# Nightmare-n/GD-MAE

Measured on AMD Instinct MI355X. Metric: MAE pre-train frames/sec (Waymo-shape, 180k pts, 75% mask), higher is better.
Workload: dtype bf16

## Files before the change

gd-mae_amd/csrc/plan.hip:

```cpp
#include "../../include/gdmae_hip.h"
#include "common.h"
#include <string.h>

int gd_voxelize_impl(const float* points, long long n_points, int n_cols, const float* lo, const float* vs, const int* grid_xyz,
                     int batch_size, float* points_out, long long* point_coords, long long* inverse, int* inverse32,
                     long long* voxel_coords, int* pillar_cell, int* pillar_pt_off, int* pillar_pts, int* point_rank,
                     int* sample_pillar_off, float* pillar_mean, int* cell2pillar_out, int* counts, void* workspace, size_t workspace_bytes,
                     void* lb_state, float* points_pm, int* row_pillar, hipStream_t st);
size_t gd_voxelize_lb_state_bytes(long long n_points, long long cells);
size_t gd_plan_scan_state_bytes(long long n);
size_t gd_plan_win_state_bytes(long long n);
int gd_plan_visible_tokens(const float* mask, const int* cell2pillar, long long n_cells, int* tok_pillar, int* tok_cell, int* map,
                           int* n_tok, void* lb_state, hipStream_t st);
int gd_plan_downsample(const int* map_in, int B, int Yi, int Xi, int* tok_cell_out, int* map_out, int* n_out, void* lb_state,
                       hipStream_t st);
struct Dims {
  int B, Y, X;
};
struct PlanJob {
  const int* n_tok;
  const int* tok_cell;
  Dims dt, dm;
  const int* map;
  int mode, s;
  int* nbr;
  int* nbr_rev;
};
constexpr int kPlanMaxJobs = 16;
struct PlanJobs {
  PlanJob j[kPlanMaxJobs];
  int count;
};
int gd_plan_jobs(const PlanJobs& J, long long cap_max, hipStream_t st);
size_t gd_plan_windows_ws_bytes(int B, int Y, int X, int wx, int wy);
long long gd_plan_n_windows(int B, int Y, int X, int wx, int wy);
struct GdWinStage {
  const int* map;
  int B, Y, X, wx, wy, nlev;
  const int *drop_lo, *drop_hi, *max_tokens;
  int* out[2][7];
  int* counts[2];
  void* workspace;
  void* lb_state;
};
int gd_plan_windows_all(const GdWinStage* stages, int n_stages, hipStream_t st);
size_t gd_decoder_tiles_lb_state_bytes(long long nt);
int gd_decoder_tiles_lb(const int* const* maps, const int* strides, int k, int B, int H, int W, int* tile_slot, int* tile_list, int* n_act,
                        int* flag, void* lb_state, hipStream_t st);
int gd_decoder_site_rulebook(const int* site, const int* n_dev, int sites_per_tok, long long cap_sites, const int* tile_slot, int H, int W,
                             int* nbr, hipStream_t st);

namespace {

struct StageGeo {
  int Y, X;
  long long cap;
  long long cap_in;
  int up_s;
  long long n_win;
};

struct Layout {
  gdmae_plan_buffer* table;
  int max_entries, n;
  size_t off;
  bool ok;
  long long add(const char* name, size_t bytes) {
    const size_t o = off;
    if (table) {
      if (n >= max_entries) {
        ok = false;
        return -1;
      }
      strncpy(table[n].name, name, sizeof(table[n].name) - 1);
      table[n].name[sizeof(table[n].name) - 1] = 0;
      table[n].offset = (long long)o;
      table[n].bytes = (long long)bytes;
    }
    ++n;
    off += gd_align(bytes);
    return (long long)o;
  }
};

struct Offsets {
  long long lb_state, counts, points, point_coords, inverse, inverse32, voxel_coords, pillar_cell, pt_off, pillar_pts, point_rank,
      sample_off, pillar_mean, cell2pillar, points_pm, row_pillar, vox_ws, mask, len_keep, tok_pillar;
  long long vis_tok_cell, vis_map;
  struct {
    long long tok_cell, map, nbr_subm, nbr_subm_t, nbr_down, nbr_down_t, up_sites, win_ws;
    long long w[2][7];
  } s[GDMAE_PLAN_MAX_STAGES];
  long long dec_slot, dec_list, dec_flag, dec_nbr[3];
  size_t lb_bytes, vox_ws_bytes;
  int n_counts;
  bool dec;
  StageGeo geo[GDMAE_PLAN_MAX_STAGES];
  long long cap_pts, m_cap, cells;
};

int check(const gdmae_plan_params* p) {
  GD_REQUIRE(p != nullptr, "geometry plan: null parameters");
  GD_REQUIRE(p->n_points >= 0 && p->n_points < (1ll << 31) && p->n_cols >= 4 && p->n_cols <= 65 && p->batch_size >= 1,
             "geometry plan: bad point buffer");
  GD_REQUIRE(p->grid[0] >= 1 && p->grid[1] >= 1 && p->grid[2] == 1, "geometry plan: single-layer pillar grids (spt_backbone_mae.py:94)");
  GD_REQUIRE(p->n_stages >= 1 && p->n_stages <= GDMAE_PLAN_MAX_STAGES, "geometry plan: 1..4 stages");
  for (int i = 0; i < p->n_stages; ++i) {
    GD_REQUIRE(p->stride[i] == 1 || p->stride[i] == 2, "geometry plan: conv_down stride 1 or 2 (k3 s2 p1)");
    GD_REQUIRE(i == 0 || p->stride[i] == 2, "geometry plan: only the first stage may keep the resolution");
    GD_REQUIRE(p->win_x[i] >= 1 && p->win_y[i] >= 1 && p->win_x[i] * p->win_y[i] <= 64, "geometry plan: window must fit one wavefront");
    GD_REQUIRE(p->n_levels[i] >= 1 && p->n_levels[i] <= 3, "geometry plan: 1..3 drop levels");
  }
  GD_REQUIRE(p->n_dec >= 0 && p->n_dec <= 3, "geometry plan: at most 3 decoder source stages");
  for (int g = 0; g < p->n_dec; ++g) GD_REQUIRE(p->dec_sources[g] >= 0 && p->dec_sources[g] < p->n_stages, "geometry plan: decoder source");
  return 0;
}

int layout(const gdmae_plan_params* p, gdmae_plan_buffer* table, int max_entries, Offsets& O, size_t* total, int* n_entries) {
  if (int rc = check(p)) return rc;
  Layout L{table, max_entries, 0, 0, true};
  const int B = p->batch_size, gx = p->grid[0], gy = p->grid[1], F = p->n_cols - 1;
  const long long n0 = p->cap_points > p->n_points ? p->cap_points : p->n_points;
  O.cells = (long long)B * gx * gy;
  GD_REQUIRE(O.cells < (1ll << 31), "geometry plan: B*Y*X must fit int32");
  O.cap_pts = n0 > 0 ? n0 : 1;
  O.m_cap = n0 < O.cells ? n0 : O.cells;
  if (O.m_cap < 1) O.m_cap = 1;
  const long long cap = O.cap_pts;
  int Y = gy, X = gx;
  long long c = O.m_cap;
  for (int i = 0; i < p->n_stages; ++i) {
    StageGeo& g = O.geo[i];
    g.cap_in = c;
    if (p->stride[i] == 2) {
      Y = (Y - 1) / 2 + 1;
      X = (X - 1) / 2 + 1;
      c = 4 * c < (long long)B * Y * X ? 4 * c : (long long)B * Y * X;
    }
    g.Y = Y; g.X = X; g.cap = c;
    const int us = gy / Y;
    g.up_s = (us >= 1 && us * Y == gy && us * X == gx) ? us : 0;
    g.n_win = gd_plan_n_windows(B, Y, X, p->win_x[i], p->win_y[i]);
    GD_REQUIRE(g.n_win < (1 << 21), "geometry plan: window grid too large for the packed scan");
  }
  O.dec = p->n_dec > 0;
  for (int g = 0; g < p->n_dec; ++g) {
    const int us = O.geo[p->dec_sources[g]].up_s;
    O.dec = O.dec && (us == 1 || us == 2 || us == 4 || us == 8);
  }
  const long long nt = (long long)B * ((gy + 7) / 8) * ((gx + 7) / 8);
  size_t lb = gd_voxelize_lb_state_bytes(n0, O.cells) + gd_plan_scan_state_bytes(O.cells);
  for (int i = 0; i < p->n_stages; ++i) {
    if (p->stride[i] == 2) lb += gd_plan_scan_state_bytes((long long)B * O.geo[i].Y * O.geo[i].X);
    lb += 2 * gd_plan_win_state_bytes(O.geo[i].n_win);
  }
  if (O.dec) lb += gd_decoder_tiles_lb_state_bytes(nt);
  O.lb_bytes = lb;
  O.lb_state = L.add("lb_state", lb);
  O.n_counts = 2 + p->n_stages + 16 * p->n_stages + 1 + 1;
  O.counts = L.add("counts", sizeof(int) * O.n_counts);
  O.points = L.add("points", sizeof(float) * cap * p->n_cols);
  O.point_coords = L.add("point_coords", sizeof(long long) * cap * 4);
  O.inverse = L.add("inverse", sizeof(long long) * cap);
  O.inverse32 = L.add("inverse32", sizeof(int) * cap);
  O.voxel_coords = L.add("voxel_coords", sizeof(long long) * cap * 4);
  O.pillar_cell = L.add("pillar_cell", sizeof(int) * cap);
  O.pt_off = L.add("pt_off", sizeof(int) * (cap + 1));
  O.pillar_pts = L.add("pillar_pts", sizeof(int) * cap);
  O.point_rank = L.add("point_rank", sizeof(int) * cap);
  O.sample_off = L.add("sample_off", sizeof(int) * (B + 1));
  O.pillar_mean = L.add("pillar_mean", sizeof(float) * cap * F);
  O.cell2pillar = L.add("cell2pillar", sizeof(int) * O.cells);
  O.points_pm = L.add("points_pm", sizeof(float) * cap * p->n_cols);
  O.row_pillar = L.add("row_pillar", sizeof(int) * cap);
  O.vox_ws_bytes = gdmae_voxelize_workspace_bytes(n0, B, gx, gy, 1);
  O.vox_ws = L.add("vox_ws", O.vox_ws_bytes);
  O.mask = L.add("mask", sizeof(float) * O.m_cap);
  O.len_keep = L.add("len_keep", sizeof(int) * B);
  O.tok_pillar = L.add("tok_pillar", sizeof(int) * O.m_cap);
  O.vis_tok_cell = O.vis_map = -1;
  if (p->stride[0] == 2) {
    O.vis_tok_cell = L.add("vis.tok_cell", sizeof(int) * O.m_cap);
    O.vis_map = L.add("vis.map", sizeof(int) * O.cells);
  }
  char nm[40];
  static const char* const kWin[7] = {"tok_win", "tok_level", "tok_slot", "tok_pos", "csr_tok", "win_start", "win_len"};
  for (int i = 0; i < p->n_stages; ++i) {
    const StageGeo& g = O.geo[i];
    auto name = [&](const char* s) { snprintf(nm, sizeof(nm), "s%d.%s", i, s); return (const char*)nm; };
    O.s[i].tok_cell = L.add(name("tok_cell"), sizeof(int) * g.cap);
    O.s[i].map = L.add(name("map"), sizeof(int) * (long long)B * g.Y * g.X);
    O.s[i].nbr_subm = L.add(name("nbr_subm"), sizeof(int) * g.cap * 9);
    O.s[i].nbr_subm_t = L.add(name("nbr_subm_t"), sizeof(int) * g.cap * 9);
    O.s[i].nbr_down = O.s[i].nbr_down_t = O.s[i].up_sites = -1;
    if (p->stride[i] == 2) {
      O.s[i].nbr_down = L.add(name("nbr_down"), sizeof(int) * g.cap * 9);
      O.s[i].nbr_down_t = L.add(name("nbr_down_t"), sizeof(int) * g.cap_in * 9);
    }
    if (g.up_s > 1) O.s[i].up_sites = L.add(name("up_sites"), sizeof(int) * g.cap * g.up_s * g.up_s);
    O.s[i].win_ws = L.add(name("win_ws"), gd_plan_windows_ws_bytes(B, g.Y, g.X, p->win_x[i], p->win_y[i]));
    const long long wcap = g.n_win < g.cap ? g.n_win : g.cap;
    for (int sh = 0; sh < 2; ++sh)
      for (int k = 0; k < 7; ++k) {
        snprintf(nm, sizeof(nm), "s%d.w%d.%s", i, sh, kWin[k]);
        O.s[i].w[sh][k] = L.add(nm, sizeof(int) * (k < 5 ? g.cap : wcap));
      }
  }
  O.dec_slot = O.dec_list = O.dec_flag = -1;
  if (O.dec) {
    O.dec_slot = L.add("dec.tile_slot", sizeof(int) * nt);
    O.dec_list = L.add("dec.tile_list", sizeof(int) * nt);
    O.dec_flag = L.add("dec.flag", sizeof(int) * nt);
    for (int g = 0; g < p->n_dec; ++g) {
      const StageGeo& sg = O.geo[p->dec_sources[g]];
      snprintf(nm, sizeof(nm), "dec.nbr%d", g);
      O.dec_nbr[g] = L.add(nm, sizeof(int) * sg.cap * sg.up_s * sg.up_s * 9);
    }
  }
  GD_REQUIRE(L.ok, "geometry plan: buffer table too small");
  if (total) *total = L.off;
  if (n_entries) *n_entries = L.n;
  return 0;
}

}

extern "C" int gdmae_geometry_plan_layout(const gdmae_plan_params* p, gdmae_plan_buffer* table, int max_entries, int* n_entries,
                                          size_t* total_bytes) {
  Offsets O;
  return layout(p, table, max_entries, O, total_bytes, n_entries);
}

extern "C" int gdmae_geometry_plan(const gdmae_plan_params* p, const float* points, const float* noise, void* arena, size_t arena_bytes,
                                   void* stream) {
  Offsets O;
  size_t total = 0;
  if (int rc = layout(p, nullptr, 0, O, &total, nullptr)) return rc;
  GD_REQUIRE(arena != nullptr && arena_bytes >= total, "geometry plan: arena too small (gdmae_geometry_plan_layout)");
  GD_REQUIRE(!p->masked || noise != nullptr, "geometry plan: masking needs one noise value per pillar (capacity min(points, cells))");
  hipStream_t st = (hipStream_t)stream;
  char* A = (char*)arena;
  auto I = [&](long long off) { return off < 0 ? (int*)nullptr : (int*)(A + off); };
  const int B = p->batch_size, gx = p->grid[0], gy = p->grid[1], ns = p->n_stages;
  int* counts = I(O.counts);
  int* n_tok = counts + 2;
  int* win_counts = counts + 2 + ns;
  int* n_act = counts + 2 + ns + 16 * ns;
  int* n_vis = n_act + 1;
  GD_CHECK(hipMemsetAsync(A + O.lb_state, 0, (size_t)(O.counts - O.lb_state) + gd_align(sizeof(int) * O.n_counts), st));
  char* lb = A + O.lb_state;
  {
    int rc = gd_voxelize_impl(points, p->n_points, p->n_cols, p->lo, p->vs, p->grid, B, (float*)(A + O.points), (long long*)(A + O.point_coords),
                              (long long*)(A + O.inverse), I(O.inverse32), (long long*)(A + O.voxel_coords), I(O.pillar_cell), I(O.pt_off),
                              I(O.pillar_pts), I(O.point_rank), I(O.sample_off), (float*)(A + O.pillar_mean), I(O.cell2pillar), counts,
                              A + O.vox_ws, O.vox_ws_bytes, lb, p->want_pm ? (float*)(A + O.points_pm) : nullptr,
                              p->want_pm ? I(O.row_pillar) : nullptr, st);
    if (rc) return rc;
    lb += gd_voxelize_lb_state_bytes(p->n_points, O.cells);
  }
  float* mask = (float*)(A + O.mask);
  if (p->masked) {
    int rc = gdmae_random_mask(noise, I(O.sample_off), B, p->keep_frac, mask, I(O.len_keep), stream);
    if (rc) return rc;
  } else {
    GD_CHECK(hipMemsetAsync(mask, 0, sizeof(float) * O.m_cap, st));
  }
  const bool first_strided = p->stride[0] == 2;
  int* cur_cell = first_strided ? I(O.vis_tok_cell) : I(O.s[0].tok_cell);
  int* cur_map = first_strided ? I(O.vis_map) : I(O.s[0].map);
  int* cur_n = first_strided ? n_vis : n_tok;
  {
    int rc = gd_plan_visible_tokens(mask, I(O.cell2pillar), O.cells, I(O.tok_pillar), cur_cell, cur_map, cur_n, lb, st);
    if (rc) return rc;
    lb += gd_plan_scan_state_bytes(O.cells);
  }
  int Yp = gy, Xp = gx;
  PlanJobs J;
  J.count = 0;
  long long cap_max = 1;
  GdWinStage W[4];
  GD_REQUIRE(ns <= 4, "geometry plan: at most four stages");
  for (int i = 0; i < ns; ++i) {
    const StageGeo& g = O.geo[i];
    GD_REQUIRE(J.count + 4 <= kPlanMaxJobs, "geometry plan: job table full");
    if (g.cap > cap_max) cap_max = g.cap;
    if (p->stride[i] == 2) {
      int rc = gd_plan_downsample(cur_map, B, Yp, Xp, I(O.s[i].tok_cell), I(O.s[i].map), n_tok + i, lb, st);
      if (rc) return rc;
      lb += gd_plan_scan_state_bytes((long long)B * g.Y * g.X);
      J.j[J.count++] = PlanJob{n_tok + i, I(O.s[i].tok_cell), Dims{B, g.Y, g.X}, Dims{B, Yp, Xp}, cur_map, 1, 0, I(O.s[i].nbr_down), nullptr};
      J.j[J.count++] = PlanJob{cur_n, cur_cell, Dims{B, Yp, Xp}, Dims{B, g.Y, g.X}, I(O.s[i].map), 2, 0, I(O.s[i].nbr_down_t), nullptr};
      if (g.cap_in > cap_max) cap_max = g.cap_in;
      cur_cell = I(O.s[i].tok_cell);
      cur_map = I(O.s[i].map);
      cur_n = n_tok + i;
      Yp = g.Y;
      Xp = g.X;
    }
    J.j[J.count++] = PlanJob{cur_n, cur_cell, Dims{B, g.Y, g.X}, Dims{B, g.Y, g.X}, cur_map, 0, 0, I(O.s[i].nbr_subm), I(O.s[i].nbr_subm_t)};
    if (g.up_s > 1) {
      J.j[J.count++] = PlanJob{cur_n, cur_cell, Dims{B, g.Y, g.X}, Dims{B, g.Y, g.X}, nullptr, 3, g.up_s, I(O.s[i].up_sites), nullptr};
      if (g.cap * g.up_s * g.up_s / 9 + 1 > cap_max) cap_max = g.cap * g.up_s * g.up_s / 9 + 1;
    }
    GdWinStage& w = W[i];
    w.map = cur_map;
    w.B = B; w.Y = g.Y; w.X = g.X; w.wx = p->win_x[i]; w.wy = p->win_y[i]; w.nlev = p->n_levels[i];
    w.drop_lo = p->drop_lo[i]; w.drop_hi = p->drop_hi[i]; w.max_tokens = p->max_tokens[i];
    w.counts[0] = win_counts + 16 * i;
    w.counts[1] = win_counts + 16 * i + 8;
    for (int sh = 0; sh < 2; ++sh)
      for (int k = 0; k < 7; ++k) w.out[sh][k] = I(O.s[i].w[sh][k]);
    w.workspace = A + O.s[i].win_ws;
    w.lb_state = lb;
    lb += 2 * gd_plan_win_state_bytes(g.n_win);
  }
  {
    int rc = gd_plan_jobs(J, cap_max, st);
    if (rc) return rc;
    rc = gd_plan_windows_all(W, ns, st);
    if (rc) return rc;
  }
  if (O.dec) {
    const int* maps[3];
    int ups[3];
    for (int g = 0; g < p->n_dec; ++g) {
      maps[g] = I(O.s[p->dec_sources[g]].map);
      ups[g] = O.geo[p->dec_sources[g]].up_s;
    }
    int rc = gd_decoder_tiles_lb(maps, ups, p->n_dec, B, gy, gx, I(O.dec_slot), I(O.dec_list), n_act, I(O.dec_flag), lb, st);
    if (rc) return rc;
    for (int g = 0; g < p->n_dec; ++g) {
      const int si = p->dec_sources[g];
      const StageGeo& sg = O.geo[si];
      const int* sites = sg.up_s > 1 ? I(O.s[si].up_sites) : I(O.s[si].tok_cell);
      rc = gd_decoder_site_rulebook(sites, n_tok + si, sg.up_s * sg.up_s, sg.cap * sg.up_s * sg.up_s, I(O.dec_slot), gy, gx, I(O.dec_nbr[g]), st);
      if (rc) return rc;
    }
  }
  return 0;
}
```

gd-mae_amd/csrc/segment.hip:

```cpp
#include "common.h"

__global__ __launch_bounds__(256) void k_gather_rows(const uint4* __restrict__ src, const int* __restrict__ idx,
                                                     long long n_slots, int row_vec, int tab_stride, int tab_off,
                                                     uint4* __restrict__ out) {
  const long long total = n_slots * row_vec;
  for (long long i = blockIdx.x * (long long)blockDim.x + threadIdx.x; i < total; i += (long long)gridDim.x * blockDim.x) {
    const long long s = i / row_vec;
    const int v = (int)(i % row_vec);
    const int j = idx[s];
    uint4 val = make_uint4(0, 0, 0, 0);
    if (j >= 0) val = src[(long long)j * tab_stride + tab_off + v];
    out[i] = val;
  }
}

__global__ __launch_bounds__(256) void k_scatter_rows(const uint4* __restrict__ src, const int* __restrict__ idx,
                                                      long long n_rows, int row_vec, int tab_stride, int tab_off,
                                                      uint4* __restrict__ dst) {
  const long long total = n_rows * row_vec;
  for (long long i = blockIdx.x * (long long)blockDim.x + threadIdx.x; i < total; i += (long long)gridDim.x * blockDim.x) {
    const long long s = i / row_vec;
    const int v = (int)(i % row_vec);
    const int j = idx[s];
    if (j >= 0) dst[(long long)j * tab_stride + tab_off + v] = src[i];
  }
}

static inline int gd_grid_for(long long total, int block = 256, int cap = 16384) {
  int g = gd_div_up(total > 0 ? total : 1, block);
  return g > cap ? cap : g;
}

extern "C" int gdmae_gather_rows(const void* src, const int* idx, long long n_slots, int row_bytes, void* out,
                                 void* stream) {
  GD_REQUIRE(row_bytes % 16 == 0, "row_bytes must be a multiple of 16");
  if (n_slots <= 0) return 0;
  const int rv = row_bytes / 16;
  hipLaunchKernelGGL(k_gather_rows, dim3(gd_grid_for(n_slots * rv)), dim3(256), 0, (hipStream_t)stream,
                     (const uint4*)src, idx, n_slots, rv, rv, 0, (uint4*)out);
  GD_LAUNCH_CHECK();
  return 0;
}

extern "C" int gdmae_gather_rows_strided(const void* src, const int* idx, long long n_slots, int row_bytes,
                                         int table_row_bytes, int table_col_bytes, void* out, void* stream) {
  GD_REQUIRE(row_bytes % 16 == 0 && table_row_bytes % 16 == 0 && table_col_bytes % 16 == 0, "16-byte granularity");
  GD_REQUIRE(table_col_bytes + row_bytes <= table_row_bytes, "slice exceeds the table row");
  if (n_slots <= 0) return 0;
  const int rv = row_bytes / 16;
  hipLaunchKernelGGL(k_gather_rows, dim3(gd_grid_for(n_slots * rv)), dim3(256), 0, (hipStream_t)stream,
                     (const uint4*)src, idx, n_slots, rv, table_row_bytes / 16, table_col_bytes / 16, (uint4*)out);
  GD_LAUNCH_CHECK();
  return 0;
}

extern "C" int gdmae_scatter_rows_strided(const void* src, const int* idx, long long n_rows, int row_bytes,
                                          int table_row_bytes, int table_col_bytes, void* dst, void* stream) {
  GD_REQUIRE(row_bytes % 16 == 0 && table_row_bytes % 16 == 0 && table_col_bytes % 16 == 0, "16-byte granularity");
  GD_REQUIRE(table_col_bytes + row_bytes <= table_row_bytes, "slice exceeds the table row");
  if (n_rows <= 0) return 0;
  const int rv = row_bytes / 16;
  hipLaunchKernelGGL(k_scatter_rows, dim3(gd_grid_for(n_rows * rv)), dim3(256), 0, (hipStream_t)stream,
                     (const uint4*)src, idx, n_rows, rv, table_row_bytes / 16, table_col_bytes / 16, (uint4*)dst);
  GD_LAUNCH_CHECK();
  return 0;
}

extern "C" int gdmae_scatter_rows(const void* src, const int* idx, long long n_rows, int row_bytes, void* dst,
                                  void* stream) {
  GD_REQUIRE(row_bytes % 16 == 0, "row_bytes must be a multiple of 16");
  if (n_rows <= 0) return 0;
  const int rv = row_bytes / 16;
  hipLaunchKernelGGL(k_scatter_rows, dim3(gd_grid_for(n_rows * rv)), dim3(256), 0, (hipStream_t)stream,
                     (const uint4*)src, idx, n_rows, rv, rv, 0, (uint4*)dst);
  GD_LAUNCH_CHECK();
  return 0;
}

template <int LPP>
__global__ __launch_bounds__(256) void k_segment_max(const float* __restrict__ x, const int* __restrict__ pt_off,
                                                     const int* __restrict__ csr, int M, float* __restrict__ out,
                                                     int* __restrict__ arg) {
  constexpr int C = LPP * 4;
  constexpr int G = GD_WAVE / LPP;
  const int lane = threadIdx.x & (GD_WAVE - 1);
  const int wib = threadIdx.x / GD_WAVE;
  const int grp = lane / LPP, cl = lane % LPP;
  for (int p = blockIdx.x * 4 + wib; p < M; p += gridDim.x * 4) {
    const int off = pt_off[p];
    const int cnt = pt_off[p + 1] - off;
    float best[4] = {-INFINITY, -INFINITY, -INFINITY, -INFINITY};
    int bi[4] = {0x7fffffff, 0x7fffffff, 0x7fffffff, 0x7fffffff};
#pragma unroll 4
    for (int j = grp; j < cnt; j += G) {
      const int i = csr[off + j];
      const float4 v = *reinterpret_cast<const float4*>(x + (long long)i * C + cl * 4);
      const float vv[4] = {v.x, v.y, v.z, v.w};
#pragma unroll
      for (int e = 0; e < 4; ++e) {
        if (vv[e] > best[e] || bi[e] == 0x7fffffff) {
          best[e] = vv[e];
          bi[e] = i;
        }
      }
    }
#pragma unroll
    for (int d = LPP; d < GD_WAVE; d <<= 1) {
#pragma unroll
      for (int e = 0; e < 4; ++e) {
        const float ob = __shfl_xor(best[e], d, GD_WAVE);
        const int oi = __shfl_xor(bi[e], d, GD_WAVE);
        const bool take = (oi != 0x7fffffff) && (bi[e] == 0x7fffffff || ob > best[e] || (ob == best[e] && oi < bi[e]));
        if (take) {
          best[e] = ob;
          bi[e] = oi;
        }
      }
    }
    if (grp == 0) {
      *reinterpret_cast<float4*>(out + (long long)p * C + cl * 4) = make_float4(best[0], best[1], best[2], best[3]);
      *reinterpret_cast<int4*>(arg + (long long)p * C + cl * 4) = make_int4(bi[0], bi[1], bi[2], bi[3]);
    }
  }
}

__global__ __launch_bounds__(256) void k_segment_max_bwd(const float* __restrict__ dout, const int* __restrict__ arg,
                                                         const int* __restrict__ inv, long long N, int C,
                                                         float* __restrict__ dx) {
  const long long total = N * C;
  for (long long e = blockIdx.x * (long long)blockDim.x + threadIdx.x; e < total; e += (long long)gridDim.x * blockDim.x) {
    const long long i = e / C;
    const int c = (int)(e % C);
    const long long q = (long long)inv[i] * C + c;
    dx[e] = (arg[q] == (int)i) ? dout[q] : 0.f;
  }
}

extern "C" int gdmae_segment_max(const float* x, const int* pt_off, const int* csr, int M, int C, float* out, int* arg,
                                 void* stream) {
  if (M <= 0) return 0;
  const dim3 grid(gd_grid_for(M, 4, 16384)), block(256);
  hipStream_t st = (hipStream_t)stream;
  switch (C) {
    case 16: hipLaunchKernelGGL((k_segment_max<4>), grid, block, 0, st, x, pt_off, csr, M, out, arg); break;
    case 32: hipLaunchKernelGGL((k_segment_max<8>), grid, block, 0, st, x, pt_off, csr, M, out, arg); break;
    case 64: hipLaunchKernelGGL((k_segment_max<16>), grid, block, 0, st, x, pt_off, csr, M, out, arg); break;
    case 128: hipLaunchKernelGGL((k_segment_max<32>), grid, block, 0, st, x, pt_off, csr, M, out, arg); break;
    case 256: hipLaunchKernelGGL((k_segment_max<64>), grid, block, 0, st, x, pt_off, csr, M, out, arg); break;
    default: GD_REQUIRE(false, "segment_max supports C in {16, 32, 64, 128, 256}");
  }
  GD_LAUNCH_CHECK();
  return 0;
}

extern "C" int gdmae_segment_max_bwd(const float* dout, const int* arg, const int* inv, long long N, int C, float* dx,
                                     void* stream) {
  if (N <= 0) return 0;
  hipLaunchKernelGGL(k_segment_max_bwd, dim3(gd_grid_for(N * C)), dim3(256), 0, (hipStream_t)stream, dout, arg, inv, N, C,
                     dx);
  GD_LAUNCH_CHECK();
  return 0;
}

struct DecoParams {
  float lo[3], vs[3];
  int ncols;
};
__global__ __launch_bounds__(256) void k_decorate(const float* __restrict__ pts, const long long* __restrict__ coords,
                                                  const int* __restrict__ inv, const float* __restrict__ mean, long long N,
                                                  DecoParams P, float* __restrict__ out) {
  const int F = P.ncols - 1;
  const int D = F + 6;
  for (long long i = blockIdx.x * (long long)blockDim.x + threadIdx.x; i < N; i += (long long)gridDim.x * blockDim.x) {
    const float* r = pts + i * P.ncols;
    const long long* c = coords + 4 * i;
    const float* m = mean + (long long)inv[i] * F;
    float* o = out + i * D;
    const float x = r[1], y = r[2], z = r[3];
    o[0] = __fsub_rn(x, __fadd_rn(__fmul_rn(__fadd_rn((float)c[3], 0.5f), P.vs[0]), P.lo[0]));
    o[1] = __fsub_rn(y, __fadd_rn(__fmul_rn(__fadd_rn((float)c[2], 0.5f), P.vs[1]), P.lo[1]));
    o[2] = __fsub_rn(z, __fadd_rn(__fmul_rn(__fadd_rn((float)c[1], 0.5f), P.vs[2]), P.lo[2]));
    for (int k = 0; k < F; ++k) o[3 + k] = r[1 + k];
    o[3 + F] = __fsub_rn(x, m[0]);
    o[4 + F] = __fsub_rn(y, m[1]);
    o[5 + F] = __fsub_rn(z, m[2]);
  }
}

extern "C" int gdmae_decorate_points(const float* points, const long long* point_coords, const int* inverse32,
                                     const float* pillar_mean, long long N, int n_cols, const float* lo, const float* vs,
                                     float* out, void* stream) {
  if (N <= 0) return 0;
  DecoParams P;
  for (int i = 0; i < 3; ++i) {
    P.lo[i] = lo[i];
    P.vs[i] = vs[i];
  }
  P.ncols = n_cols;
  hipLaunchKernelGGL(k_decorate, dim3(gd_grid_for(N)), dim3(256), 0, (hipStream_t)stream, points, point_coords, inverse32,
                     pillar_mean, N, P, out);
  GD_LAUNCH_CHECK();
  return 0;
}

__device__ inline void unpack8(const uint4& u, float (&f)[8]) {
  const unsigned w[4] = {u.x, u.y, u.z, u.w};
#pragma unroll
  for (int k = 0; k < 4; ++k) {
    f[2 * k] = __uint_as_float(w[k] << 16);
    f[2 * k + 1] = __uint_as_float(w[k] & 0xFFFF0000u);
  }
}

template <bool BF16>
__global__ __launch_bounds__(256) void k_colstats_partial(const uint4* __restrict__ x, long long R, int C,
                                                          float* __restrict__ part ) {
  constexpr int EPV = BF16 ? 8 : 4;
  const int vec_per_row = C / EPV;
  const int rows_per_iter = 256 / vec_per_row;
  const int vr = threadIdx.x / vec_per_row;
  const int vc = threadIdx.x % vec_per_row;
  const bool live = vr < rows_per_iter;
  const long long chunk = (R + gridDim.x - 1) / gridDim.x;
  const long long r0 = blockIdx.x * chunk;
  const long long r1 = r0 + chunk < R ? r0 + chunk : R;
  float s[EPV], q[EPV];
#pragma unroll
  for (int e = 0; e < EPV; ++e) s[e] = q[e] = 0.f;
  for (long long r = r0 + vr; live && r < r1; r += rows_per_iter) {
    const uint4 u = x[r * vec_per_row + vc];
    float f[8];
    if (BF16) {
      unpack8(u, f);
    } else {
      f[0] = __uint_as_float(u.x);
      f[1] = __uint_as_float(u.y);
      f[2] = __uint_as_float(u.z);
      f[3] = __uint_as_float(u.w);
    }
#pragma unroll
    for (int e = 0; e < EPV; ++e) {
      s[e] += f[e];
      q[e] = fmaf(f[e], f[e], q[e]);
    }
  }
  extern __shared__ float sh[];
  if (live) {
#pragma unroll
    for (int e = 0; e < EPV; ++e) {
      sh[(vr * 2 + 0) * C + vc * EPV + e] = s[e];
      sh[(vr * 2 + 1) * C + vc * EPV + e] = q[e];
    }
  }
  __syncthreads();
  for (int c = threadIdx.x; c < 2 * C; c += 256) {
    float acc = 0.f;
    for (int rr = 0; rr < rows_per_iter; ++rr) acc += sh[rr * 2 * C + c];
    part[(long long)blockIdx.x * 2 * C + c] = acc;
  }
}

__global__ __launch_bounds__(256) void k_colstats_final(const float* __restrict__ part, int nblk, int C2,
                                                        double* __restrict__ out) {
  __shared__ double sh[16][17];
  const int cl = threadIdx.x & 15, ps = threadIdx.x >> 4;
  const int c = blockIdx.x * 16 + cl;
  double acc = 0.0;
  if (c < C2) {
#pragma unroll 8
    for (int b = ps; b < nblk; b += 16) acc += (double)part[(long long)b * C2 + c];
  }
  sh[ps][cl] = acc;
  __syncthreads();
  if (ps == 0 && c < C2) {
    double s = 0.0;
    for (int k = 0; k < 16; ++k) s += sh[k][cl];
    out[c] = s;
  }
}

extern "C" size_t gdmae_colstats_workspace_bytes(int C) { return (size_t)1024 * 2 * C * sizeof(float); }

extern "C" int gdmae_colstats(const void* x, long long R, int C, int is_bf16, double* out, void* workspace, void* stream) {
  hipStream_t st = (hipStream_t)stream;
  const int epv = is_bf16 ? 8 : 4;
  GD_REQUIRE(C % epv == 0 && (C / epv) <= 256, "C must be a multiple of 8 (bf16) / 4 (fp32) and <= 2048 / 1024");
  int nblk = (int)(R / 64 > 512 ? 512 : (R / 64 > 0 ? R / 64 : 1));
  if (R >= (1ll << 20)) nblk = 1024;
  const int rows_per_iter = 256 / (C / epv);
  const size_t lds = (size_t)rows_per_iter * 2 * C * sizeof(float);
  GD_REQUIRE(lds <= 64 * 1024, "colstats LDS");
  if (is_bf16)
    hipLaunchKernelGGL((k_colstats_partial<true>), dim3(nblk), dim3(256), lds, st, (const uint4*)x, R, C, (float*)workspace);
  else
    hipLaunchKernelGGL((k_colstats_partial<false>), dim3(nblk), dim3(256), lds, st, (const uint4*)x, R, C, (float*)workspace);
  GD_LAUNCH_CHECK();
  hipLaunchKernelGGL(k_colstats_final, dim3(gd_div_up(2 * C, 16)), dim3(256), 0, st, (const float*)workspace, nblk, 2 * C, out);
  GD_LAUNCH_CHECK();
  return 0;
}

__global__ __launch_bounds__(256) void k_bn_fold_final(const float* __restrict__ part, int nblk, int C, double count,
                                                       const float* __restrict__ gamma, const float* __restrict__ beta,
                                                       double eps, double momentum, float* __restrict__ running_mean,
                                                       float* __restrict__ running_var, long long* __restrict__ num_batches,
                                                       double* __restrict__ stats, float* __restrict__ ab,
                                                       float* __restrict__ mv) {
  __shared__ double sh[2][16][17];
  const int cl = threadIdx.x & 15, ps = threadIdx.x >> 4;
  const int c = blockIdx.x * 16 + cl;
  double a1 = 0.0, a2 = 0.0;
  {
    const int cc = c < C ? c : C - 1;
    const float* p = part + cc;
    for (int b0 = ps; b0 < nblk; b0 += 128) {
      float v1[8], v2[8];
#pragma unroll
      for (int u = 0; u < 8; ++u) {
        const int b = b0 + 16 * u < nblk ? b0 + 16 * u : nblk - 1;
        v1[u] = p[(long long)b * 2 * C];
        v2[u] = p[(long long)b * 2 * C + C];
      }
#pragma unroll
      for (int u = 0; u < 8; ++u) {
        const bool ok = b0 + 16 * u < nblk;
        a1 += ok ? (double)v1[u] : 0.0;
        a2 += ok ? (double)v2[u] : 0.0;
      }
    }
  }
  sh[0][ps][cl] = a1;
  sh[1][ps][cl] = a2;
  __syncthreads();
  if (ps == 0 && c < C) {
    double s1 = 0.0, s2 = 0.0;
    for (int k = 0; k < 16; ++k) { s1 += sh[0][k][cl]; s2 += sh[1][k][cl]; }
    const double mean = s1 / count;
    double var = s2 / count - mean * mean;
    if (var < 0.0) var = 0.0;
    const double r = 1.0 / sqrt(var + eps);
    const double a = (double)gamma[c] * r;
    stats[c] = mean;
    stats[C + c] = r;
    ab[c] = (float)a;
    ab[C + c] = (float)((double)beta[c] - a * mean);
    mv[c] = (float)mean;
    mv[C + c] = (float)var;
    if (running_mean) {
      const float m = (float)momentum;
      const float unb = (float)(var * (count / (count > 1.0 ? count - 1.0 : 1.0)));
      running_mean[c] = running_mean[c] * (1.f - m) + m * (float)mean;
      running_var[c] = running_var[c] * (1.f - m) + m * unb;
      if (c == 0 && num_batches) *num_batches += 1;
    }
  }
}

extern "C" int gdmae_bn_fold(const void* x, long long R, int C, int is_bf16, double count, const float* gamma,
                             const float* beta, double eps, double momentum, float* running_mean, float* running_var,
                             long long* num_batches, double* stats, float* ab, float* mv, void* workspace, void* stream) {
  hipStream_t st = (hipStream_t)stream;
  const int epv = is_bf16 ? 8 : 4;
  GD_REQUIRE(C % epv == 0 && (C / epv) <= 256, "C must be a multiple of 8 (bf16) / 4 (fp32) and <= 2048 / 1024");
  int nblk = (int)(R / 64 > 512 ? 512 : (R / 64 > 0 ? R / 64 : 1));
  if (R >= (1ll << 20)) nblk = 1024;
  const int rows_per_iter = 256 / (C / epv);
  const size_t lds = (size_t)rows_per_iter * 2 * C * sizeof(float);
  GD_REQUIRE(lds <= 64 * 1024, "colstats LDS");
  if (is_bf16)
    hipLaunchKernelGGL((k_colstats_partial<true>), dim3(nblk), dim3(256), lds, st, (const uint4*)x, R, C, (float*)workspace);
  else
    hipLaunchKernelGGL((k_colstats_partial<false>), dim3(nblk), dim3(256), lds, st, (const uint4*)x, R, C, (float*)workspace);
  GD_LAUNCH_CHECK();
  hipLaunchKernelGGL(k_bn_fold_final, dim3(gd_div_up(C, 16)), dim3(256), 0, st, (const float*)workspace, nblk, C, count, gamma,
                     beta, eps, momentum, running_mean, running_var, num_batches, stats, ab, mv);
  GD_LAUNCH_CHECK();
  return 0;
}

int gd_bn_fold_from_partials(hipStream_t st, const float* part, int nblk, int C, double count, const float* gamma,
                             const float* beta, double eps, double momentum, float* running_mean, float* running_var,
                             long long* num_batches, double* stats, float* ab, float* mv) {
  hipLaunchKernelGGL(k_bn_fold_final, dim3(gd_div_up(C, 16)), dim3(256), 0, st, part, nblk, C, count, gamma, beta, eps, momentum,
                     running_mean, running_var, num_batches, stats, ab, mv);
  GD_LAUNCH_CHECK();
  return 0;
}
extern "C" int gdmae_bn_fold_partials(const float* part, int nblk, int C, double count, const float* gamma, const float* beta, double eps,
                                      double momentum, float* running_mean, float* running_var, long long* num_batches, double* stats,
                                      float* ab, float* mv, void* stream) {
  GD_REQUIRE(part != nullptr && nblk >= 1 && C >= 1, "bn_fold_partials: partial rows");
  return gd_bn_fold_from_partials((hipStream_t)stream, part, nblk, C, count, gamma, beta, eps, momentum, running_mean, running_var,
                                  num_batches, stats, ab, mv);
}
int gd_partials_to_f64(hipStream_t st, const float* part, int nblk, int C2, double* out) {
  hipLaunchKernelGGL(k_colstats_final, dim3(gd_div_up(C2, 16)), dim3(256), 0, st, part, nblk, C2, out);
  GD_LAUNCH_CHECK();
  return 0;
}

__global__ __launch_bounds__(256) void k_bn_bwd_coeffs(const double* __restrict__ st, int n_st, const double* __restrict__ stats,
                                                       const float* __restrict__ ab, const float* __restrict__ gamma, int C,
                                                       double count, const double* __restrict__ tot,
                                                       float* __restrict__ dgamma, float* __restrict__ dbeta, int accumulate,
                                                       float* __restrict__ c01) {
  const int c = blockIdx.x * blockDim.x + threadIdx.x;
  if (c >= C) return;
  const double mean = stats[c], r = stats[C + c];
  const double a = (double)ab[c], b = (double)ab[C + c];
  double db = st[c];
  if (tot && n_st >= 3 && b > 0.0) db += tot[c] - st[2 * C + c];
  const double da = st[C + c] - db * mean;
  const double dv = -0.5 * (da * (double)gamma[c]) * r * r * r;
  const double dmu = -db * a - 2.0 * mean * dv;
  c01[c] = (float)(dmu / count);
  c01[C + c] = (float)(2.0 * dv / count);
  const float dg = (float)(da * r), dbf = (float)db;
  if (accumulate) { dgamma[c] += dg; dbeta[c] += dbf; }
  else { dgamma[c] = dg; dbeta[c] = dbf; }
}

__global__ __launch_bounds__(256) void k_bn_bwd_coeffs_rows(const float* __restrict__ part, int nblk, int n_st,
                                                            const double* __restrict__ stats, const float* __restrict__ ab,
                                                            const float* __restrict__ gamma, int C, double count,
                                                            const double* __restrict__ tot, float* __restrict__ dgamma,
                                                            float* __restrict__ dbeta, int accumulate, float* __restrict__ c01) {
  __shared__ double sh[3][32][9];
  const int cl = threadIdx.x & 7, ps = threadIdx.x >> 3;
  const int c = blockIdx.x * 8 + cl;
  const long long stride = (long long)n_st * C;
  {
    const int cc = c < C ? c : C - 1;
    double acc[3] = {0.0, 0.0, 0.0};
    for (int b0 = ps; b0 < nblk; b0 += 256) {
      float x[3][8];
#pragma unroll
      for (int v = 0; v < 3; ++v)
#pragma unroll
        for (int u = 0; u < 8; ++u) {
          const int b = b0 + 32 * u < nblk ? b0 + 32 * u : nblk - 1;
          x[v][u] = part[(long long)b * stride + (long long)(v < n_st ? v : 0) * C + cc];
        }
#pragma unroll
      for (int v = 0; v < 3; ++v)
#pragma unroll
        for (int u = 0; u < 8; ++u) acc[v] += b0 + 32 * u < nblk ? (double)x[v][u] : 0.0;
    }
#pragma unroll
    for (int v = 0; v < 3; ++v) sh[v][ps][cl] = acc[v];
  }
  __syncthreads();
  if (ps != 0 || c >= C) return;
  double s[3] = {0.0, 0.0, 0.0};
  for (int v = 0; v < n_st; ++v)
    for (int k = 0; k < 32; ++k) s[v] += sh[v][k][cl];
  const double mean = stats[c], r = stats[C + c];
  const double a = (double)ab[c], bb = (double)ab[C + c];
  double db = s[0];
  if (tot && n_st >= 3 && bb > 0.0) db += tot[c] - s[2];
  const double da = s[1] - db * mean;
  const double dv = -0.5 * (da * (double)gamma[c]) * r * r * r;
  const double dmu = -db * a - 2.0 * mean * dv;
  c01[c] = (float)(dmu / count);
  c01[C + c] = (float)(2.0 * dv / count);
  const float dg = (float)(da * r), dbf = (float)db;
  if (accumulate) { dgamma[c] += dg; dbeta[c] += dbf; }
  else { dgamma[c] = dg; dbeta[c] = dbf; }
}
extern "C" int gdmae_bn_bwd_coeffs_rows(const float* part, int nblk, int n_st, const double* stats, const float* ab, const float* gamma,
                                        int C, double count, const double* tot, float* dgamma, float* dbeta, int accumulate, float* c01,
                                        void* stream) {
  GD_REQUIRE((n_st == 2 || n_st == 3) && nblk >= 1, "n_st must be 2 or 3");
  hipLaunchKernelGGL(k_bn_bwd_coeffs_rows, dim3(gd_div_up(C, 8)), dim3(256), 0, (hipStream_t)stream, part, nblk, n_st, stats, ab, gamma, C,
                     count, tot, dgamma, dbeta, accumulate, c01);
  GD_LAUNCH_CHECK();
  return 0;
}

extern "C" int gdmae_bn_bwd_coeffs(const double* st, int n_st, const double* stats, const float* ab, const float* gamma, int C,
                                   double count, const double* tot, float* dgamma, float* dbeta, int accumulate, float* c01,
                                   void* stream) {
  GD_REQUIRE(n_st == 2 || n_st == 3, "n_st must be 2 or 3");
  hipLaunchKernelGGL(k_bn_bwd_coeffs, dim3(gd_div_up(C, 256)), dim3(256), 0, (hipStream_t)stream, st, n_st, stats, ab, gamma, C,
                     count, tot, dgamma, dbeta, accumulate, c01);
  GD_LAUNCH_CHECK();
  return 0;
}
```

gd-mae_amd/csrc/vfe_fused.hip:

```cpp
#include "common.h"
#include "gemm.h"

int gd_bn_fold_from_partials(hipStream_t st, const float* part, int nblk, int C, double count, const float* gamma,
                             const float* beta, double eps, double momentum, float* running_mean, float* running_var,
                             long long* num_batches, double* stats, float* ab, float* mv);
int gd_partials_to_f64(hipStream_t st, const float* part, int nblk, int C2, double* out);
extern "C" int gdmae_bn_bwd_coeffs(const double* st, int n_st, const double* stats, const float* ab, const float* gamma, int C,
                                   double count, const double* tot, float* dgamma, float* dbeta, int accumulate, float* c01,
                                   void* stream);

namespace {

typedef float f32x16 __attribute__((ext_vector_type(16)));

constexpr int VF_C = 64;
constexpr int VF_WAVES = 4;
constexpr int VF_MAX_GRID = 1024;

struct VfeGeom {
  float lo[3], vs[3];
  int out_f16 = 0;
};

enum { VF_STATS = 0, VF_APPLY = 1, VF_BSTATS = 2, VF_DW = 3 };

__device__ inline unsigned short vf_f2bf(float f) { return gd_to_bf16(f); }

template <int F>
struct VfA {
  float r[F + 1];
  int pil;
};
struct VfB {
  long long c1, c2, c3;
  float m[3];
};
template <int F>
__device__ __forceinline__ void vf_load_a(const float* __restrict__ pts, const int* __restrict__ inv, long long i, long long N, VfA<F>& A) {
  const long long ic = i < N ? i : N - 1;
  const float* r = pts + ic * (F + 1);
#pragma unroll
  for (int k = 0; k < F + 1; ++k) A.r[k] = r[k];
  A.pil = inv[ic];
}
template <int F>
__device__ __forceinline__ void vf_load_b(const long long* __restrict__ coords, const float* __restrict__ mean, int cpp, long long i,
                                          long long N, int pil, VfB& B) {
  const long long ic = i < N ? i : N - 1;
  const long long* c = coords + 4 * (cpp ? (long long)pil : ic);
  const float* m = mean + (long long)pil * F;
  B.c1 = c[1]; B.c2 = c[2]; B.c3 = c[3];
  B.m[0] = m[0]; B.m[1] = m[1]; B.m[2] = m[2];
}
template <int F>
__device__ __forceinline__ void vf_features(const VfA<F>& A, const VfB& B, bool live, const VfeGeom& G, float (&f)[F + 6]) {
  const float x = A.r[1], y = A.r[2], z = A.r[3];
  f[0] = __fsub_rn(x, __fadd_rn(__fmul_rn(__fadd_rn((float)B.c3, 0.5f), G.vs[0]), G.lo[0]));
  f[1] = __fsub_rn(y, __fadd_rn(__fmul_rn(__fadd_rn((float)B.c2, 0.5f), G.vs[1]), G.lo[1]));
  f[2] = __fsub_rn(z, __fadd_rn(__fmul_rn(__fadd_rn((float)B.c1, 0.5f), G.vs[2]), G.lo[2]));
#pragma unroll
  for (int k = 0; k < F; ++k) f[3 + k] = A.r[1 + k];
  f[3 + F] = __fsub_rn(x, B.m[0]);
  f[4 + F] = __fsub_rn(y, B.m[1]);
  f[5 + F] = __fsub_rn(z, B.m[2]);
#pragma unroll
  for (int k = 0; k < F + 6; ++k) f[k] = live ? f[k] : 0.f;
}
template <bool BF>
struct VfG {
  unsigned u[BF ? 16 : 1];
  float2 v[BF ? 1 : 16];
};
template <bool BF>
__device__ __forceinline__ void vf_load_g(const void* __restrict__ g, long long base, long long N, int n, int half, VfG<BF>& Gr) {
#pragma unroll
  for (int r = 0; r < 16; ++r) {
    const long long row = base + 8 * (r / 4) + 4 * half + (r % 4);
    const long long rc = row < N ? row : N - 1;
    if (BF) Gr.u[r] = ((const unsigned*)g)[rc * (VF_C / 2) + n];
    else Gr.v[r] = ((const float2*)g)[rc * (VF_C / 2) + n];
  }
}

template <int F, int MODE, bool BF>
__global__ __launch_bounds__(VF_WAVES * 64) void k_vfe1(const float* __restrict__ pts, const long long* __restrict__ coords,
                                                        const int* __restrict__ inv, const float* __restrict__ mean,
                                                        int cpp, long long N, VfeGeom G, const float* __restrict__ W,
                                                        const float* __restrict__ ab, const float* __restrict__ c01,
                                                        const void* __restrict__ g, void* __restrict__ out,
                                                        float* __restrict__ part) {
  constexpr int D = F + 6;
  constexpr int KS = (D + 1) / 2;
  constexpr int DP = 2 * KS;
  const int lane = threadIdx.x & 63, wave = threadIdx.x >> 6;
  const int n = lane & 31, half = lane >> 5;
  __shared__ float sh[VF_WAVES * (MODE == VF_DW ? VF_C * D : 4 * VF_C)];
  __shared__ float shf[MODE == VF_DW ? VF_WAVES * 32 * DP : 1];

  float wb[2][KS];
#pragma unroll
  for (int blk = 0; blk < 2; ++blk)
#pragma unroll
    for (int s = 0; s < KS; ++s) {
      const int d = 2 * s + half;
      wb[blk][s] = d < D ? W[(2 * n + blk) * D + d] : 0.f;
    }
  float ca[2] = {0.f, 0.f}, cb[2] = {0.f, 0.f}, c0[2] = {0.f, 0.f}, c1[2] = {0.f, 0.f};
  if (MODE != VF_STATS) {
#pragma unroll
    for (int blk = 0; blk < 2; ++blk) {
      ca[blk] = ab[2 * n + blk];
      cb[blk] = ab[VF_C + 2 * n + blk];
      if (MODE == VF_DW) {
        c0[blk] = c01[2 * n + blk];
        c1[blk] = c01[VF_C + 2 * n + blk];
      }
    }
  }
  float s1[2] = {0.f, 0.f}, s2[2] = {0.f, 0.f};
  f32x16 accw[2];
#pragma unroll
  for (int r = 0; r < 16; ++r) accw[0][r] = accw[1][r] = 0.f;

  const long long ntiles = (N + 31) / 32;
  const long long tstride = (long long)gridDim.x * VF_WAVES;
  constexpr bool HAS_G = MODE == VF_BSTATS || MODE == VF_DW;
  constexpr bool PIPE = !HAS_G;
  VfA<F> A1, A2, A3;
  VfB B1, B2;
  VfG<BF> G1;
  if (PIPE) {
    const long long t = (long long)blockIdx.x * VF_WAVES + wave;
    vf_load_a<F>(pts, inv, t * 32 + n, N, A1);
    vf_load_a<F>(pts, inv, (t + tstride) * 32 + n, N, A2);
    vf_load_b<F>(coords, mean, cpp, t * 32 + n, N, A1.pil, B1);
  }
  for (long long t0 = (long long)blockIdx.x * VF_WAVES; t0 < ntiles; t0 += tstride) {
    const long long base = (t0 + wave) * 32;
    if (PIPE) {
      vf_load_a<F>(pts, inv, base + 2 * tstride * 32 + n, N, A3);
      vf_load_b<F>(coords, mean, cpp, base + tstride * 32 + n, N, A2.pil, B2);
      __builtin_amdgcn_sched_barrier(0);
    } else {
      vf_load_g<BF>(g, base, N, n, half, G1);
      vf_load_a<F>(pts, inv, base + n, N, A1);
      vf_load_b<F>(coords, mean, cpp, base + n, N, A1.pil, B1);
    }
    float g0[16], g1[16];
    if (HAS_G) {
#pragma unroll
      for (int r = 0; r < 16; ++r) {
        const long long row = base + 8 * (r / 4) + 4 * half + (r % 4);
        if (BF) {
          g0[r] = row < N ? __uint_as_float(G1.u[r] << 16) : 0.f;
          g1[r] = row < N ? __uint_as_float(G1.u[r] & 0xFFFF0000u) : 0.f;
        } else {
          g0[r] = row < N ? G1.v[r].x : 0.f;
          g1[r] = row < N ? G1.v[r].y : 0.f;
        }
      }
    }
    float f[D];
    vf_features<F>(A1, B1, base + n < N, G, f);
    f32x16 h[2];
#pragma unroll
    for (int r = 0; r < 16; ++r) h[0][r] = h[1][r] = 0.f;
#pragma unroll
    for (int s = 0; s < KS; ++s) {
      const float f0 = f[2 * s], f1 = (2 * s + 1 < D) ? f[2 * s + 1] : 0.f;
      const float a = half ? f1 : f0;
      h[0] = __builtin_amdgcn_mfma_f32_32x32x2f32(a, wb[0][s], h[0], 0, 0, 0);
      h[1] = __builtin_amdgcn_mfma_f32_32x32x2f32(a, wb[1][s], h[1], 0, 0, 0);
    }
    if (MODE == VF_STATS) {
#pragma unroll
      for (int r = 0; r < 16; ++r)
#pragma unroll
        for (int blk = 0; blk < 2; ++blk) {
          const float v = h[blk][r];
          s1[blk] += v;
          s2[blk] = fmaf(v, v, s2[blk]);
        }
    } else if (MODE == VF_APPLY) {
#pragma unroll
      for (int k = 0; k < F + 1; ++k) asm volatile("" : "+v"(A3.r[k]));
      asm volatile("" : "+v"(A3.pil));
      asm volatile("" : "+v"(B2.c1), "+v"(B2.c2), "+v"(B2.c3), "+v"(B2.m[0]), "+v"(B2.m[1]), "+v"(B2.m[2]));
#pragma unroll
      for (int r = 0; r < 16; ++r) {
        const long long row = base + 8 * (r / 4) + 4 * half + (r % 4);
        if (row < N) {
          const float y0 = fmaxf(fmaf(ca[0], h[0][r], cb[0]), 0.f), y1 = fmaxf(fmaf(ca[1], h[1][r], cb[1]), 0.f);
          if (BF) ((unsigned*)out)[row * (VF_C / 2) + n] = G.out_f16 ? gd_pack_f16(y0, y1) : ((unsigned)vf_f2bf(y0) | ((unsigned)vf_f2bf(y1) << 16));
          else ((float2*)out)[row * (VF_C / 2) + n] = make_float2(y0, y1);
        }
      }
    } else {
      if (MODE == VF_DW) {
        if (half == 0) {
#pragma unroll
          for (int d = 0; d < DP; ++d) shf[(wave * 32 + n) * DP + d] = d < D ? f[d] : 0.f;
        }
        __builtin_amdgcn_fence(__ATOMIC_RELEASE, "wavefront");
        __builtin_amdgcn_wave_barrier();
        __builtin_amdgcn_fence(__ATOMIC_ACQUIRE, "wavefront");
      }
#pragma unroll
      for (int r = 0; r < 16; ++r) {
        const int pr = 8 * (r / 4) + 4 * half + (r % 4);
        const float dh0 = fmaf(ca[0], h[0][r], cb[0]) > 0.f ? g0[r] : 0.f;
        const float dh1 = fmaf(ca[1], h[1][r], cb[1]) > 0.f ? g1[r] : 0.f;
        if (MODE == VF_BSTATS) {
          s1[0] += dh0;
          s1[1] += dh1;
          s2[0] = fmaf(dh0, h[0][r], s2[0]);
          s2[1] = fmaf(dh1, h[1][r], s2[1]);
        } else {
          const float dx0 = fmaf(c1[0], h[0][r], fmaf(ca[0], dh0, c0[0]));
          const float dx1 = fmaf(c1[1], h[1][r], fmaf(ca[1], dh1, c0[1]));
          const float bv = n < DP ? shf[(wave * 32 + pr) * DP + n] : 0.f;
          accw[0] = __builtin_amdgcn_mfma_f32_32x32x2f32(dx0, bv, accw[0], 0, 0, 0);
          accw[1] = __builtin_amdgcn_mfma_f32_32x32x2f32(dx1, bv, accw[1], 0, 0, 0);
        }
      }
      if (MODE == VF_DW) {
        __builtin_amdgcn_fence(__ATOMIC_RELEASE, "wavefront");
        __builtin_amdgcn_wave_barrier();
      }
    }
    if (PIPE) {
      A1 = A2;
      A2 = A3;
      B1 = B2;
    }
  }

  if (MODE == VF_STATS || MODE == VF_BSTATS) {
#pragma unroll
    for (int blk = 0; blk < 2; ++blk) {
      s1[blk] += __shfl_xor(s1[blk], 32, 64);
      s2[blk] += __shfl_xor(s2[blk], 32, 64);
    }
    if (half == 0) {
#pragma unroll
      for (int blk = 0; blk < 2; ++blk) {
        sh[wave * 2 * VF_C + 2 * n + blk] = s1[blk];
        sh[wave * 2 * VF_C + VF_C + 2 * n + blk] = s2[blk];
      }
    }
    __syncthreads();
    if (threadIdx.x < 2 * VF_C) {
      float a = 0.f;
#pragma unroll
      for (int w = 0; w < VF_WAVES; ++w) a += sh[w * 2 * VF_C + threadIdx.x];
      part[(long long)blockIdx.x * 2 * VF_C + threadIdx.x] = a;
    }
  } else if (MODE == VF_DW) {
    if (n < D) {
#pragma unroll
      for (int blk = 0; blk < 2; ++blk)
#pragma unroll
        for (int r = 0; r < 16; ++r) {
          const int col = 2 * (8 * (r / 4) + 4 * half + (r % 4)) + blk;
          sh[wave * VF_C * D + col * D + n] = accw[blk][r];
        }
    }
    __syncthreads();
    for (int e = threadIdx.x; e < VF_C * D; e += VF_WAVES * 64) {
      float a = 0.f;
#pragma unroll
      for (int w = 0; w < VF_WAVES; ++w) a += sh[w * VF_C * D + e];
      part[(long long)blockIdx.x * VF_C * D + e] = a;
    }
  }
}

template <typename K>
int vf_resident_blocks(K kernel, int slot) {
  static int cache[32] = {0};
  if (cache[slot] == 0) {
    int per_cu = 0, dev = 0;
    hipDeviceProp_t prop;
    if (hipOccupancyMaxActiveBlocksPerMultiprocessor(&per_cu, kernel, VF_WAVES * 64, 0) != hipSuccess || per_cu < 1) per_cu = 2;
    if (hipGetDevice(&dev) != hipSuccess || hipGetDeviceProperties(&prop, dev) != hipSuccess) prop.multiProcessorCount = 256;
    const long long b = (long long)per_cu * prop.multiProcessorCount;
    cache[slot] = (int)(b > VF_MAX_GRID ? VF_MAX_GRID : b);
  }
  return cache[slot];
}

template <int MODE>
int vf_launch(hipStream_t st, int F, bool bf, const float* pts, const long long* coords, const int* inv, const float* mean,
              int cpp, long long N, const VfeGeom& G, const float* W, const float* ab, const float* c01, const void* g, void* out,
              float* part, int* grid_out = nullptr) {
  const long long tiles = (N + 31) / 32, blocks = (tiles + VF_WAVES - 1) / VF_WAVES;
  const dim3 block(VF_WAVES * 64);
#define VF_GO(FF, BB)                                                                                                   \
  do {                                                                                                                  \
    const int cap = vf_resident_blocks(k_vfe1<FF, MODE, BB>, ((FF - 3) * 4 + MODE) * 2 + (BB ? 1 : 0));                 \
    const dim3 grid((unsigned)(blocks < cap ? blocks : cap));                                                           \
    if (grid_out) *grid_out = (int)grid.x;                                                                              \
    hipLaunchKernelGGL((k_vfe1<FF, MODE, BB>), grid, block, 0, st, pts, coords, inv, mean, cpp, N, G, W, ab, c01, g, out, part); \
  } while (0)
  if (F == 5) { if (bf) VF_GO(5, true); else VF_GO(5, false); }
  else if (F == 4) { if (bf) VF_GO(4, true); else VF_GO(4, false); }
  else if (F == 3) { if (bf) VF_GO(3, true); else VF_GO(3, false); }
  else GD_REQUIRE(false, "vfe point layer: 3, 4 or 5 point features (x, y, z [, intensity [, elongation]])");
#undef VF_GO
  GD_LAUNCH_CHECK();
  return 0;
}

}

__global__ __launch_bounds__(256) void k_pillar_major_rows(const float* __restrict__ pts, int ncols, const int* __restrict__ csr,
                                                           const int* __restrict__ inv, const int* __restrict__ n_dev,
                                                           float* __restrict__ pts_pm, int* __restrict__ rowpil) {
  const long long N = *n_dev;
  for (long long q = blockIdx.x * (long long)blockDim.x + threadIdx.x; q < N; q += (long long)gridDim.x * blockDim.x) {
    const int i = csr[q];
    rowpil[q] = inv[i];
    for (int k = 0; k < ncols; ++k) pts_pm[q * ncols + k] = pts[(long long)i * ncols + k];
  }
}

extern "C" int gdmae_pillar_major_rows(const float* points, int n_cols, const int* pillar_pts, const int* inverse32,
                                       const int* n_dev, long long capacity, float* points_pm, int* row_pillar,
                                       void* stream) {
  if (capacity <= 0) return 0;
  hipLaunchKernelGGL(k_pillar_major_rows, dim3((unsigned)(capacity / 256 + 1 > 8192 ? 8192 : capacity / 256 + 1)), dim3(256), 0, (hipStream_t)stream, points, n_cols,
                     pillar_pts, inverse32, n_dev, points_pm, row_pillar);
  GD_LAUNCH_CHECK();
  return 0;
}

extern "C" size_t gdmae_vfe_point_layer_workspace_bytes(int n_cols) {
  const int D = n_cols - 1 + 6;
  return gd_align((size_t)VF_MAX_GRID * VF_C * (D > 2 ? D : 2) * sizeof(float)) + gd_align(2 * VF_C * sizeof(double)) +
         gd_align(2 * VF_C * sizeof(float));
}

extern "C" int gdmae_vfe_point_layer_fwd(const float* points, const long long* point_coords, const int* inverse32,
                                         const float* pillar_mean, int coords_per_pillar, long long N, int n_cols,
                                         const float* lo, const float* vs,
                                         const float* W, int C, const float* gamma, const float* beta, double eps,
                                         double momentum, float* running_mean, float* running_var, long long* num_batches,
                                         double* stats, float* ab, float* mv, void* out, int out_bf16, void* workspace,
                                         void* stream) {
  GD_REQUIRE(C == VF_C, "vfe point layer: 64 output channels");
  GD_REQUIRE(N > 0, "vfe point layer: no points");
  hipStream_t st = (hipStream_t)stream;
  VfeGeom G;
  for (int i = 0; i < 3; ++i) { G.lo[i] = lo[i]; G.vs[i] = vs[i]; }
  float* part = (float*)workspace;
  const int F = n_cols - 1;
  int grid = 0;
  int rc = vf_launch<VF_STATS>(st, F, false, points, point_coords, inverse32, pillar_mean, coords_per_pillar, N, G, W, nullptr, nullptr, nullptr,
                               nullptr, part, &grid);
  if (rc) return rc;
  rc = gd_bn_fold_from_partials(st, part, grid, C, (double)N, gamma, beta, eps, momentum, running_mean, running_var,
                                num_batches, stats, ab, mv);
  if (rc) return rc;
  G.out_f16 = out_bf16 == 2;
  return vf_launch<VF_APPLY>(st, F, out_bf16 != 0, points, point_coords, inverse32, pillar_mean, coords_per_pillar, N, G, W, ab, nullptr, nullptr,
                             out, nullptr);
}

extern "C" int gdmae_vfe_point_layer_bwd(const float* points, const long long* point_coords, const int* inverse32,
                                         const float* pillar_mean, int coords_per_pillar, long long N, int n_cols,
                                         const float* lo, const float* vs,
                                         const float* W, int C, const float* gamma, const double* stats, const float* ab,
                                         const void* g, int g_bf16, float* dgamma, float* dbeta, float* dW, int accumulate,
                                         void* workspace, void* stream) {
  GD_REQUIRE(C == VF_C, "vfe point layer: 64 output channels");
  GD_REQUIRE(N > 0, "vfe point layer: no points");
  hipStream_t st = (hipStream_t)stream;
  VfeGeom G;
  for (int i = 0; i < 3; ++i) { G.lo[i] = lo[i]; G.vs[i] = vs[i]; }
  const int F = n_cols - 1, D = F + 6;
  char* p = (char*)workspace;
  float* part = (float*)p;
  p += gd_align((size_t)VF_MAX_GRID * VF_C * (D > 2 ? D : 2) * sizeof(float));
  double* sums = (double*)p;
  p += gd_align(2 * VF_C * sizeof(double));
  float* c01 = (float*)p;
  int grid = 0;
  int rc = vf_launch<VF_BSTATS>(st, F, g_bf16 != 0, points, point_coords, inverse32, pillar_mean, coords_per_pillar, N, G, W, ab, nullptr, g,
                                nullptr, part, &grid);
  if (rc) return rc;
  rc = gd_partials_to_f64(st, part, grid, 2 * C, sums);
  if (rc) return rc;
  rc = gdmae_bn_bwd_coeffs(sums, 2, stats, ab, gamma, C, (double)N, nullptr, dgamma, dbeta, accumulate, c01, stream);
  if (rc) return rc;
  rc = vf_launch<VF_DW>(st, F, g_bf16 != 0, points, point_coords, inverse32, pillar_mean, coords_per_pillar, N, G, W, ab, c01, g, nullptr, part, &grid);
  if (rc) return rc;
  return gd_splitk_acc(st, part, grid, (long long)VF_C * D, dW, accumulate);
}
```

gd-mae_amd/gdmae_hip/lib.py:

```python
from __future__ import annotations

import ctypes as C
import os

import torch

_HERE = os.path.dirname(os.path.abspath(__file__))
LIB_PATH = os.path.abspath(os.path.join(_HERE, "..", "csrc", "libgdmae_hip.so"))
if os.environ.get("GDMAE_LIB"):
    LIB_PATH = os.path.abspath(os.environ["GDMAE_LIB"])


class GdmaeHipError(RuntimeError):
    pass


_P, _I, _L, _F, _D, _Z = C.c_void_p, C.c_int, C.c_longlong, C.c_float, C.c_double, C.c_size_t

SIGNATURES = {
    "gdmae_abi_version": (_I, []),
    "gdmae_target_arch": (C.c_char_p, []),
    "gdmae_last_error": (C.c_char_p, []),
    "gdmae_voxelize_workspace_bytes": (_Z, [_L, _I, _I, _I, _I]),
    "gdmae_voxelize": (_I, [_P, _L, _I, _P, _P, _P, _I, _P, _P, _P, _P, _P, _P, _P, _P, _P, _P, _P, _P, _P, _P, _Z, _P]),
    "gdmae_decorate_points": (_I, [_P, _P, _P, _P, _L, _I, _P, _P, _P, _P]),
    "gdmae_vfe_infer": (_I, [_P, _P, _P, _P, _L, _L, _I, _P, _P, _P, _P, _I, _P, _P, _I, _P, _P]),
    "gdmae_vfe_point_layer_workspace_bytes": (_Z, [_I]),
    "gdmae_pillar_major_rows": (_I, [_P, _I, _P, _P, _P, _L, _P, _P, _P]),
    "gdmae_vfe_point_layer_fwd": (_I, [_P, _P, _P, _P, _I, _L, _I, _P, _P, _P, _I, _P, _P, _D, _D, _P, _P, _P, _P, _P, _P, _P, _I, _P, _P]),
    "gdmae_vfe_point_layer_bwd": (_I, [_P, _P, _P, _P, _I, _L, _I, _P, _P, _P, _I, _P, _P, _P, _P, _I, _P, _P, _P, _I, _P, _P]),
    "gdmae_vfe_max_layer_workspace_bytes": (_Z, []),
    "gdmae_vfe_max_layer_fwd": (_I, [_P, _L, _P, _P, _P, _I, _P, _P, _D, _D, _P, _P, _P, _P, _P, _P, _P, _P, _P, _P]),
    "gdmae_vfe_max_layer_bwd": (_I, [_P, _L, _P, _P, _I, _P, _P, _P, _P, _P, _P, _P, _P, _P, _P, _P, _I, _P, _P]),
    "gdmae_vfe_max_layer_fwd_f16": (_I, [_P, _L, _P, _P, _P, _I, _P, _P, _D, _D, _P, _P, _P, _P, _P, _P, _P, _P, _P, _P]),
    "gdmae_vfe_max_layer_bwd_f16": (_I, [_P, _L, _P, _P, _I, _P, _P, _P, _P, _P, _P, _P, _P, _P, _P, _P, _I, _P, _P]),
    "gdmae_fill_rows": (_I, [_P, _L, _I, _I, _P, _P]),
    "gdmae_weighted_mean_finish": (_I, [_P, _P, _L, _P, _P]),
    "gdmae_decoder_region_workspace_bytes": (_Z, [_I, _I]),
    "gdmae_decoder_region_algebra": (_I, [_P, _P, _P, _P, _P, _P, _P, _D, _I, _I, _P, _P, _I, _P, _P, _P, _P, _P, _P]),
    "gdmae_segment_max": (_I, [_P, _P, _P, _I, _I, _P, _P, _P]),
    "gdmae_segment_max_bwd": (_I, [_P, _P, _P, _L, _I, _P, _P]),
    "gdmae_random_mask": (_I, [_P, _P, _I, _D, _P, _P, _P]),
    "gdmae_visible_tokens": (_I, [_P, _P, _P, _L, _L, _P, _P, _P, _P, _P, _P]),
    "gdmae_downsample_tokens": (_I, [_P, _P, _L, _I, _I, _I, _P, _P, _P, _P, _P, _P]),
    "gdmae_rulebook": (_I, [_P, _P, _L, _I, _I, _I, _I, _I, _P, _I, _P, _P]),
    "gdmae_window_workspace_bytes": (_Z, [_I, _I, _I, _I, _I]),
    "gdmae_window_partition": (_I, [_P, _I, _I, _I, _I, _I, _I, _I, _P, _P, _P, _P, _P, _P, _P, _P, _P, _P, _P, _P, _Z, _P]),
    "gdmae_gather_rows": (_I, [_P, _P, _L, _I, _P, _P]),
    "gdmae_scatter_rows": (_I, [_P, _P, _L, _I, _P, _P]),
    "gdmae_gather_rows_strided": (_I, [_P, _P, _L, _I, _I, _I, _P, _P]),
    "gdmae_scatter_rows_strided": (_I, [_P, _P, _L, _I, _I, _I, _P, _P]),
    "gdmae_colstats_workspace_bytes": (_Z, [_I]),
    "gdmae_colstats": (_I, [_P, _L, _I, _I, _P, _P, _P]),
    "gdmae_rows_affine_relu_scatter": (_I, [_P, _I, _P, _L, _I, _P, _P, _P, _I, _I, _I, _P]),
    "gdmae_rows_affine_relu_sub": (_I, [_P, _I, _P, _L, _I, _P, _P, _P, _P, _I, _I, _I, _P]),
    "gdmae_rows_affine_relu_add": (_I, [_P, _I, _L, _I, _P, _P, _P, _P, _I, _P]),
    "gdmae_rows_bwd_stats_workspace_bytes": (_Z, [_I]),
    "gdmae_rows_bwd_stats": (_I, [_P, _I, _P, _L, _I, _P, _P, _P, _I, _I, _I, _P, _P, _P]),
    "gdmae_bn_fold": (_I, [_P, _L, _I, _I, _D, _P, _P, _D, _D, _P, _P, _P, _P, _P, _P, _P, _P]),
    "gdmae_bn_bwd_coeffs": (_I, [_P, _I, _P, _P, _P, _I, _D, _P, _P, _P, _I, _P, _P]),
    "gdmae_rows_bwd_stats_rows": (_I, [_L]),
    "gdmae_bn_bwd_coeffs_rows": (_I, [_P, _I, _I, _P, _P, _P, _I, _D, _P, _P, _P, _I, _P, _P]),
    "gdmae_border_sums_workspace_bytes": (_Z, [_I, _I]),
    "gdmae_border_sums": (_I, [_P, _I, _P, _P, _P, _P, _I, _I, _I, _I, _I, _P, _P, _P]),
    "gdmae_conv3x3_grad_taps": (_I, [_P, _I, _P, _P, _P, _P, _P, _P, _P, _L, _I, _I, _I, _P, _P]),
    "gdmae_decoder_tiles_workspace_bytes": (_Z, [_I, _I, _I]),
    "gdmae_decoder_tiles": (_I, [_P, _P, _I, _I, _I, _I, _P, _P, _P, _P, _P]),
    "gdmae_conv3x3_tiles_packed_bytes": (_Z, [_I]),
    "gdmae_conv3x3_tiles_pack": (_I, [_P, _I, _I, _P, _I, _P, _P, _P, _P]),
    "gdmae_conv3x3_tiles_workspace_bytes": (_Z, [_I]),
    "gdmae_conv3x3_tiles_fwd": (_I, [_P, _P, _P, _P, _P, _I, _P, _P, _P, _I, _I, _I, _I, _P, _P, _P, _D, _D, _P, _P, _P, _P, _P, _P,
                                     _P, _P]),
    "gdmae_tiles_gather_rows": (_I, [_P, _P, _P, _P, _L, _I, _I, _I, _I, _P, _P]),
    "gdmae_tiles_to_dense": (_I, [_P, _P, _P, _I, _I, _I, _I, _I, _P, _P]),
    "gdmae_tiles_to_dense_affine_relu": (_I, [_P, _P, _P, _I, _I, _I, _I, _P, _P, _P, _P]),
    "gdmae_rows_bwd": (_I, [_P, _I, _P, _L, _I, _P, _P, _P, _P, _P, _I, _I, _I, _P, _I, _P]),
    "gdmae_segment_max_affine": (_I, [_P, _I, _P, _P, _I, _I, _P, _P, _P, _P, _P]),
    "gdmae_segmax_bwd_stats": (_I, [_P, _I, _P, _P, _P, _L, _I, _P, _P, _P, _P, _P]),
    "gdmae_segmax_bn_bwd": (_I, [_P, _I, _P, _P, _P, _P, _L, _I, _P, _P, _P, _P, _I, _P]),
    "gdmae_window_attention_fwd": (_I, [_P, _P, _P, _I, _P, _P, _P, _I, _I, _I, _I, _P, _F, _P]),
    "gdmae_window_attention_bwd": (_I, [_P, _P, _P, _P, _P, _I, _P, _P, _P, _P, _I, _I, _I, _I, _P, _F, _P]),
    "gdmae_window_attention_levels_writes_lse": (_I, [_I, _I, _P, _I, _I]),
    "gdmae_window_attention_levels_fwd": (_I, [_P, _P, _P, _I, _P, _P, _P, _I, _P, _P, _I, _I, _P, _F, _P, _P]),
    "gdmae_window_attention_levels_bwd": (_I, [_P, _P, _P, _P, _P, _I, _P, _P, _P, _P, _I, _P, _P, _I, _I, _P, _F, _P, _P, _P]),
    "gdmae_conv3x3_dense_packed_bytes": (_Z, [_I, _I]),
    "gdmae_conv3x3_dense_pack": (_I, [_P, _I, _I, _I, _I, _P, _P]),
    "gdmae_conv3x3_dense": (_I, [_P, _I, _I, _I, _I, _I, _I, _P, _P, _P, _P]),
    "gdmae_conv3x3_dense_add": (_I, [_P, _I, _I, _I, _I, _I, _I, _P, _P, _P, _P, _P]),
    "gdmae_conv3x3_dense_relu": (_I, [_P, _I, _I, _I, _I, _I, _I, _P, _P, _P, _P, _P]),
    "gdmae_conv3x3_dense_stats_workspace_bytes": (_Z, [_I, _I, _I, _I]),
    "gdmae_conv3x3_dense_stat_rows": (_I, []),
    "gdmae_conv3x3_dense_stats": (_I, [_P, _I, _I, _I, _I, _I, _I, _P, _P, _P, _P, _P, _P]),
    "gdmae_bn_fold_partials": (_I, [_P, _I, _I, _D, _P, _P, _D, _D, _P, _P, _P, _P, _P, _P, _P]),
    "gdmae_conv3x3_dense_f32out": (_I, [_P, _I, _I, _I, _I, _I, _I, _P, _P, _P, _I, _P]),
    "gdmae_conv3x3_dense_dw_workspace_bytes": (_Z, [_I, _I, _I, _I, _I]),
    "gdmae_conv3x3_dense_bwd_weight": (_I, [_P, _P, _I, _I, _I, _I, _I, _I, _I, _I, _P, _P, _P]),
    "gdmae_attention_timing": (_I, [_I]),
    "gdmae_attention_timing_read": (_I, [_I, _P, _P]),
    "gdmae_kernel_timing": (_I, [_I]),
    "gdmae_kernel_timing_slots": (_I, []),
    "gdmae_kernel_timing_name": (C.c_char_p, [_I]),
    "gdmae_kernel_timing_read": (_I, [_I, _P, _P, _P, _P]),
    "gdmae_kernel_timing_read_side": (_I, [_I, _P]),
    "gdmae_add_layernorm_workspace_bytes": (_Z, [_I]),
    "gdmae_add_layernorm_fwd": (_I, [_P, _P, _I, _P, _P, _L, _I, _F, _P, _P, _P, _P]),
    "gdmae_add_layernorm_bwd": (_I, [_P, _P, _I, _P, _P, _P, _P, _I, _L, _I, _P, _P, _P, _P, _P]),
    "gdmae_prep_tokens": (_I, [_P, _P, _P, _L, _I, _P, _P, _I, _P]),
    "gdmae_sum_bf16": (_I, [_P, _I, _L, _P, _P]),
    "gdmae_add3": (_I, [_P, _P, _I, _P, _I, _L, _P, _P]),
    "gdmae_add3_to": (_I, [_P, _P, _I, _P, _I, _L, _P, _I, _P]),
    "gdmae_set_attention_impl": (_I, [_I]),
    "gdmae_sum_partials": (_I, [_P, _L, _F, _P, _I, _P]),
    "gdmae_sum_partials_gated": (_I, [_P, _L, _F, _P, _P, _F, _P]),
    "gdmae_gemm_workspace_bytes": (_Z, []),
    "gdmae_gemm_stats": (_I, [_P]),
    "gdmae_gemm_tuning": (_I, [_I]),
    "gdmae_gemm": (_I, [_P, _P, _P, _L, _L, _L, _I, _I, _I, _I, _P, _P, _P]),
    "gdmae_gemm_tn_splitk_workspace_bytes": (_Z, [_L, _I, _I]),
    "gdmae_gemm_tn_splitk": (_I, [_P, _P, _P, _L, _I, _I, _I, _I, _P, _P]),
    "gdmae_conv_block_scratch_bytes": (_Z, [_L, _L, _I, _I, _I]),
    "gdmae_spconv_packed_bytes": (_Z, [_I, _I]),
    "gdmae_spconv_pack_jobs": (_I, [_P, _I, _I, _I, _P, _P]),
    "gdmae_spconv": (_I, [_P, _I, _P, _P, _L, _I, _I, _P, _I, _P]),
    "gdmae_spconv_bias_relu": (_I, [_P, _I, _P, _P, _P, _L, _I, _I, _P, _P]),
    "gdmae_spconv_stat_rows": (_I, [_I, _I, _I]),
    "gdmae_spconv_stats": (_I, [_P, _I, _P, _P, _L, _I, _I, _P, _P, _P]),
    "gdmae_decoder_dy": (_I, [_P, _P, _I, _P, _P, _P, _P, _I, _I, _I, _P, _P]),
    "gdmae_decoder_site_rulebook": (_I, [_P, _P, _I, _L, _P, _I, _I, _P, _P]),
    "gdmae_tap_dw_rows": (_L, [_L, _I, _I]),
    "gdmae_tap_dw_workspace_bytes": (_Z, [_L, _I, _I]),
    "gdmae_tap_dw": (_I, [_P, _L, _L, _I, _P, _P, _I, _P, _I, _I, _P, _P]),
    "gdmae_conv_block_fwd": (_I, [_P, _P]),
    "gdmae_conv_block_bwd": (_I, [_P, _P]),
    "gdmae_encoder_layer_bytes": (_I, [_L, _I, _I, _I, _I, _P, _P, _P]),
    "gdmae_dw_gemm_workspace_bytes": (_Z, [_L, _I, _I]),
    "gdmae_dw_gemm": (_I, [_P, _P, _L, _I, _I, _P, _P, _P, _P]),
    "gdmae_layer_packed_bytes": (_Z, [_I, _I]),
    "gdmae_layer_pack_jobs": (_I, [_P, _P, _P, _P, _I, _I, _P, _P]),
    "gdmae_layer_pack_job_count": (_I, [_I, _I]),
    "gdmae_tok_gemm_pack": (_I, [_P, _I, _P]),
    "gdmae_tok_gemm": (_I, [_P, _P, _P, _L, _L, _I, _I, _I, _P, _P, _P, _P, _P, _P, _F, _P, _P, _P, _P, _P, _P, _P]),
    "gdmae_tok_gemm_qkv": (_I, [_P, _P, _P, _P, _P, _L, _I, _P, _P, _P]),
    "gdmae_tok_gemm_ffn": (_I, [_P, _P, _P, _P, _P, _L, _L, _I, _P, _P, _P, _P, _F, _P, _P, _P, _P, _P, _P, _P, _P]),
    "gdmae_tok_gemm_ln_bwd_rows": (_I, [_I]),
    "gdmae_tok_gemm_ln_bwd": (_I, [_P, _P, _L, _L, _I, _I, _P, _P, _P, _P, _P, _P, _P, _P, _P, _P]),
    "gdmae_encoder_layer_fwd": (_I, [_P, _P]),
    "gdmae_encoder_layer_bwd": (_I, [_P, _P]),
    "gdmae_encoder_stage_fwd": (_I, [_P, _I, _P]),
    "gdmae_encoder_stage_bwd": (_I, [_P, _I, _P]),
    "gdmae_deconv_rows_packed_bytes": (_Z, [_I, _I, _I]),
    "gdmae_deconv_rows_pack": (_I, [_P, _I, _I, _I, _P, _P, _P]),
    "gdmae_deconv_rows_fwd": (_I, [_P, _L, _I, _I, _I, _P, _P, _P]),
    "gdmae_deconv_rows_bwd_input": (_I, [_P, _L, _I, _I, _I, _P, _P, _P]),
    "gdmae_deconv_rows_dw_workspace_bytes": (_Z, [_L, _I, _I, _I]),
    "gdmae_deconv_rows_bwd_weight": (_I, [_P, _P, _L, _I, _I, _I, _P, _P, _P]),
    "gdmae_pred_head_packed_bytes": (_Z, []),
    "gdmae_pred_head_pack": (_I, [_P, _P, _I, _I, _P, _P]),
    "gdmae_pred_head_fwd": (_I, [_P, _L, _I, _P, _P, _P, _P, _P]),
    "gdmae_pred_head_bwd_workspace_bytes": (_Z, [_L]),
    "gdmae_pred_head_bwd": (_I, [_P, _I, _P, _P, _P, _P, _L, _I, _P, _P, _P, _P, _P, _P]),
    "gdmae_encoder_set_layer_path": (_I, [_I]),
    "gdmae_encoder_stage_fused": (_I, [_P, _I]),
    "gdmae_group_gt_points": (_I, [_P, _I, _P, _P, _P, _I, _I, _P, _P, _P, _P, _P]),
    "gdmae_chamfer": (_I, [_P, _P, _P, _I, _I, _I, _P, _P, _P]),
    "gdmae_augment_collate_workspace_bytes": (_Z, [_L]),
    "gdmae_augment_collate": (_I, [_P, _L, _I, _P, _I, _P, _P, _P, _P, _P, _P]),
    "gdmae_group_workspace_bytes": (_Z, [_L, _L]),
    "gdmae_ingroup_inds": (_I, [_P, _L, _L, _P, _P, _Z, _P]),
    "gdmae_group_inner_inds": (_I, [_P, _L, _L, _I, _P, _P, _Z, _P]),
    "gdmae_center_head_targets_workspace_bytes": (_Z, [_I, _I]),
    "gdmae_center_head_targets": (_I, [_P, _I, _I, _I, _P, _I, _I, _P, _P, _F, _I, _I, _I, _D, _I, _P, _P, _P, _P, _P, _P]),
    "gdmae_center_head_targets_iou": (_I, [_P, _I, _I, _I, _P, _I, _I, _P, _P, _F, _I, _I, _I, _D, _I, _P, _P, _P, _P, _P, _P, _P]),
    "gdmae_focal_loss_rows": (_I, []),
    "gdmae_focal_loss_fwd": (_I, [_P, _I, _P, _P, _I, _I, _I, _I, _P, _P, _P, _P]),
    "gdmae_focal_loss_bwd": (_I, [_P, _I, _P, _P, _I, _I, _I, _I, _P, _P, _P, _I, _P]),
    "gdmae_center_head_decode": (_I, [_P, _P, _P, _P, _P, _P, _P, _P, _I, _I, _I, _I, _P, _P, _F, _P, _F, _I, _P, _P, _P, _P, _P]),
    "gdmae_anchor_targets_workspace_bytes": (_Z, [_I, _I, _I]),
    "gdmae_anchor_targets": (_I, [_P, _I, _I, _I, _I, _I, _I, _I, _I, _P, _P, _P, _P, _P, _P, _P, _P, _P, _F, _I, _P, _P, _P, _P, _P, _P, _P]),
    "gdmae_anchor_loss_rows": (_I, []),
    "gdmae_anchor_loss_fwd": (_I, [_P, _I, _I, _I, _I, _I, _I, _I, _P, _P, _P, _P, _P, _P, _P, _P, _P]),
    "gdmae_anchor_loss_bwd": (_I, [_P, _I, _I, _I, _I, _I, _I, _I, _P, _P, _P, _P, _P, _P, _P, _P, _P]),
    "gdmae_anchor_decode": (_I, [_P, _I, _I, _I, _I, _I, _I, _I, _I, _P, _P, _P, _F, _F, _P, _P, _P]),
    "gdmae_anchor_select": (_I, [_P, _I, _I, _I, _I, _F, _P, _P, _P, _P, _P]),
    "gdmae_anchor_head_infer_packed_bytes": (_Z, [_I]),
    "gdmae_anchor_head_infer_pack": (_I, [_P, _P, _P, _P, _P, _P, _I, _I, _I, _I, _P, _P]),
    "gdmae_anchor_head_infer_workspace_bytes": (_Z, [_I, _I, _I, _I]),
    "gdmae_anchor_head_infer": (_I, [_P, _I, _I, _I, _I, _I, _I, _I, _P, _P, _P, _P, _F, _F, _F, _P, _P, _P, _P, _P, _P, _P, _P]),
    "gdmae_boxes_bev_pairs": (_I, [_P, _I, _P, _I, _I, _P, _P]),
    "gdmae_nms_workspace_bytes": (_Z, [_I]),
    "gdmae_nms_bev": (_I, [_P, _I, _F, _I, _P, _P, _P, _P]),
    "gdmae_geometry_plan_layout": (_I, [_P, _P, _I, _P, _P]),
    "gdmae_geometry_plan": (_I, [_P, _P, _P, _P, _Z, _P]),
    "gdmae_grad_sq_norm": (_I, [_P, _L, _P, _P, _P]),
    "gdmae_adam_step": (_I, [_P, _P, _P, _P, _P, _I, _F, _F, _F, _F, _F, _I, _F, _F, _P, _P]),
    "gdmae_adam_step_shadow": (_I, [_P, _P, _P, _P, _P, _I, _F, _F, _F, _F, _F, _I, _F, _F, _P, _P, _P]),
}

class LayerArgs(C.Structure):
    _fields_ = ([("n", _L), ("d", _I), ("ff", _I), ("nhead", _I), ("bf16", _I), ("eps", _F), ("tau_min", _F), ("n_levels", _I),
                 ("n_win", _I * 4), ("max_tokens", _I * 4)]
                + [(k, _P) for k in ("tok_pos", "csr_tok", "win_start", "win_len", "pos_table", "Win", "bin", "Wo", "bo", "W1", "b1",
                                     "W2", "b2", "g1", "be1", "g2", "be2", "tau", "x", "y", "dy", "dx", "dWin", "dbin", "dtau", "dWo",
                                     "dbo", "dW1", "db1", "dW2", "db2", "dg1", "dbe1", "dg2", "dbe2", "saved", "scratch", "packed")]
                + [("x_bf16", _I), ("res_out", _P), ("dres", _P), ("dx_bf16", _P), ("path", _I)])


class PlanParams(C.Structure):
    _fields_ = [("n_points", _L), ("n_cols", _I), ("batch_size", _I), ("lo", _F * 3), ("vs", _F * 3), ("grid", _I * 3), ("n_stages", _I),
                ("stride", _I * 4), ("win_x", _I * 4), ("win_y", _I * 4), ("n_levels", _I * 4), ("drop_lo", (_I * 3) * 4),
                ("drop_hi", (_I * 3) * 4), ("max_tokens", (_I * 3) * 4), ("masked", _I), ("keep_frac", _D), ("n_dec", _I),
                ("dec_sources", _I * 4), ("want_pm", _I), ("cap_points", _L)]


class PlanBuffer(C.Structure):
    _fields_ = [("name", C.c_char * 40), ("offset", _L), ("bytes", _L)]


class ConvBlockArgs(C.Structure):
    _fields_ = ([("n_in", _L), ("n_out", _L), ("cin", _I), ("cout", _I), ("bf16", _I), ("x_f32", _I), ("g_f32", _I),
                 ("eps", _F), ("momentum", _F)]
                + [(k, _P) for k in ("x", "nbr", "nbr_t", "W", "gamma", "beta", "running_mean", "running_var", "num_batches", "cols",
                                     "y", "stats", "ab", "mv", "out", "g", "dx", "dW", "dgamma", "dbeta", "scratch", "packed_fwd", "packed_bwd")]
                + [("out_f32", _I)])


_lib = None


def load():
    global _lib
    if _lib is not None:
        return _lib
    if not os.path.exists(LIB_PATH):
        raise GdmaeHipError(f"{LIB_PATH} not found - build it with `python -m gdmae_hip.build` "
                            "(__graft_entry__.build()); there is no CPU fallback for the product path")
    lib = C.CDLL(LIB_PATH)
    for name, (res, args) in SIGNATURES.items():
        fn = getattr(lib, name)
        fn.restype = res
        fn.argtypes = args
    _lib = lib
    return lib


def ptr(t):
    if t is None:
        return None
    assert t.is_cuda and t.is_contiguous(), "HIP entry points need contiguous device tensors"
    return t.data_ptr()


_raw_stream = getattr(torch._C, "_cuda_getCurrentRawStream", None)


def stream():
    if _raw_stream is not None:
        return _raw_stream(torch.cuda.current_device())
    return torch.cuda.current_stream().cuda_stream


def call(name, *args):
    lib = load()
    rc = getattr(lib, name)(*args)
    if rc != 0:
        raise GdmaeHipError(f"{name} failed ({rc}): {lib.gdmae_last_error().decode()}")


def host_f32(vals):
    return (C.c_float * len(vals))(*[float(v) for v in vals])


def host_i32(vals):
    return (C.c_int * len(vals))(*[int(v) for v in vals])


def host_i64(vals):
    return (C.c_longlong * len(vals))(*[int(v) for v in vals])


def ptr_any(t):
    assert t.is_cuda
    return t.data_ptr()


def host_ptrs(tensors):
    return (C.c_void_p * len(tensors))(*[ptr(t) for t in tensors])


def host_ptrs_any(tensors):
    return (C.c_void_p * len(tensors))(*[ptr_any(t) for t in tensors])
```

gd-mae_amd/gdmae_hip/plan.py:

```python
from __future__ import annotations

from dataclasses import dataclass, field
from typing import List, Optional

import torch

from . import lib as L

I32 = torch.int32


def _empty(n, dtype, dev):
    return torch.empty(int(n), dtype=dtype, device=dev)


@dataclass
class VoxelPlan:
    batch_size: int
    grid: tuple
    lo: tuple
    vs: tuple
    n_cols: int
    N: int
    M: int
    points: torch.Tensor
    point_coords: torch.Tensor
    inverse: torch.Tensor
    inverse32: torch.Tensor
    voxel_coords: torch.Tensor
    pillar_cell: torch.Tensor
    pt_off: torch.Tensor
    pillar_pts: torch.Tensor
    point_rank: torch.Tensor
    sample_off: torch.Tensor
    pillar_mean: torch.Tensor
    cell2pillar: torch.Tensor
    counts: torch.Tensor
    points_pm: torch.Tensor = None
    row_pillar: torch.Tensor = None


def _voxelize_launch(points: torch.Tensor, point_cloud_range, voxel_size, grid_size, batch_size: int) -> dict:
    assert points.is_cuda and points.dtype == torch.float32 and points.dim() == 2
    points = points.contiguous()
    dev = points.device
    n0, ncols = points.shape
    gx, gy, gz = (int(g) for g in grid_size)
    cells = batch_size * gx * gy * gz
    lo = tuple(float(v) for v in point_cloud_range[:3])
    vs = tuple(float(v) for v in voxel_size)
    F = ncols - 1
    cap = max(n0, 1)
    r = dict(batch_size=batch_size, grid=(gx, gy, gz), lo=lo, vs=vs, ncols=ncols, n0=n0, src=points,
             pts_out=_empty(cap * ncols, torch.float32, dev), pcoords=_empty(cap * 4, torch.int64, dev),
             inverse=_empty(cap, torch.int64, dev), inverse32=_empty(cap, I32, dev), vcoords=_empty(cap * 4, torch.int64, dev),
             pillar_cell=_empty(cap, I32, dev), pt_off=_empty(cap + 1, I32, dev), pillar_pts=_empty(cap, I32, dev),
             prank=_empty(cap, I32, dev), sample_off=_empty(batch_size + 1, I32, dev), mean=_empty(cap * F, torch.float32, dev),
             cell2pillar=_empty(cells, I32, dev), counts=_empty(2, I32, dev))
    wsb = L.load().gdmae_voxelize_workspace_bytes(n0, batch_size, gx, gy, gz)
    r["ws"] = _empty(wsb, torch.uint8, dev)
    L.call("gdmae_voxelize", L.ptr(points), n0, ncols, L.host_f32(lo), L.host_f32(vs), L.host_i32((gx, gy, gz)),
           batch_size, L.ptr(r["pts_out"]), L.ptr(r["pcoords"]), L.ptr(r["inverse"]), L.ptr(r["inverse32"]), L.ptr(r["vcoords"]),
           L.ptr(r["pillar_cell"]), L.ptr(r["pt_off"]), L.ptr(r["pillar_pts"]), L.ptr(r["prank"]), L.ptr(r["sample_off"]),
           L.ptr(r["mean"]), L.ptr(r["cell2pillar"]), L.ptr(r["counts"]), L.ptr(r["ws"]), wsb, L.stream())
    r["pts_pm"] = _empty(cap * ncols, torch.float32, dev)
    r["row_pillar"] = _empty(cap, I32, dev)
    L.call("gdmae_pillar_major_rows", L.ptr(r["pts_out"]), ncols, L.ptr(r["pillar_pts"]), L.ptr(r["inverse32"]), L.ptr(r["counts"]),
           cap, L.ptr(r["pts_pm"]), L.ptr(r["row_pillar"]), L.stream())
    return r


def _voxelize_finalize(r: dict, N: int, M: int) -> VoxelPlan:
    ncols = r["ncols"]
    F = ncols - 1
    return VoxelPlan(r["batch_size"], r["grid"], r["lo"], r["vs"], ncols, N, M,
                     r["pts_out"][:N * ncols].view(N, ncols), r["pcoords"][:N * 4].view(N, 4), r["inverse"][:N],
                     r["inverse32"][:N], r["vcoords"][:M * 4].view(M, 4), r["pillar_cell"][:M], r["pt_off"][:M + 1],
                     r["pillar_pts"][:N], r["prank"][:N], r["sample_off"], r["mean"][:M * F].view(M, F), r["cell2pillar"],
                     r["counts"], r["pts_pm"][:N * ncols].view(N, ncols), r["row_pillar"][:N])


def voxelize(points: torch.Tensor, point_cloud_range, voxel_size, grid_size, batch_size: int) -> VoxelPlan:
    r = _voxelize_launch(points, point_cloud_range, voxel_size, grid_size, batch_size)
    N, M = (int(v) for v in r["counts"].tolist())
    return _voxelize_finalize(r, N, M)


@dataclass
class WindowPlan:
    tok_win: torch.Tensor
    tok_level: torch.Tensor
    tok_slot: torch.Tensor
    tok_pos: torch.Tensor
    csr_tok: torch.Tensor
    win_start: torch.Tensor
    win_len: torch.Tensor
    n_win: List[int] = field(default_factory=list)
    n_tok: List[int] = field(default_factory=list)
    max_tokens: List[int] = field(default_factory=list)


@dataclass
class StagePlan:
    B: int
    Y: int
    X: int
    n_tok: int
    tok_cell: torch.Tensor
    map: torch.Tensor
    nbr_subm: torch.Tensor
    nbr_down: Optional[torch.Tensor]
    nbr_down_t: Optional[torch.Tensor]
    windows: List[WindowPlan] = field(default_factory=list)

    def indices_byx(self) -> torch.Tensor:
        c = self.tok_cell.long()
        x = c % self.X
        r = c // self.X
        return torch.stack([r // self.Y, r % self.Y, x], dim=-1).int()


@dataclass
class DecoderTiles:
    sources: tuple
    B: int
    H: int
    W: int
    n_act: int
    tile_slot: torch.Tensor
    tile_list: torch.Tensor
    nbr: Optional[list] = None


@dataclass
class EncoderPlan:
    mask: Optional[torch.Tensor]
    tok_pillar: torch.Tensor
    stages: List[StagePlan]
    dec_tiles: Optional[DecoderTiles] = None


def upsample_cells(c: torch.Tensor, Ys: int, Xs: int, s: int) -> torch.Tensor:
    x = c % Xs
    r = torch.div(c, Xs, rounding_mode='floor')
    y = r % Ys
    b = torch.div(r, Ys, rounding_mode='floor')
    d = torch.arange(s, device=c.device, dtype=c.dtype)
    yy = (y * s).view(-1, 1, 1) + d.view(1, s, 1)
    xx = (x * s).view(-1, 1, 1) + d.view(1, 1, s)
    return ((b.view(-1, 1, 1) * (Ys * s) + yy) * (Xs * s) + xx).reshape(c.numel(), s * s)


def _drop_arrays(drop_info):
    d = {int(k): v for k, v in drop_info.items()}
    keys = sorted(d)
    assert keys == list(range(len(keys))) and len(keys) <= 3
    lo = [int(d[k]["drop_range"][0]) for k in keys]
    hi = [int(d[k]["drop_range"][1]) for k in keys]
    T = [int(d[k]["max_tokens"]) for k in keys]
    return lo, hi, T


def _decoder_tiles_launch(maps, ups, B, H, W, dev) -> dict:
    nt = B * ((H + 7) // 8) * ((W + 7) // 8)
    r = dict(tile_slot=_empty(nt, I32, dev), tile_list=_empty(nt, I32, dev), n_act=_empty(1, I32, dev), B=B, H=H, W=W)
    ws = _empty(L.load().gdmae_decoder_tiles_workspace_bytes(B, H, W), torch.uint8, dev)
    L.call("gdmae_decoder_tiles", L.host_ptrs(maps), L.host_i32(ups), len(maps), B, H, W, L.ptr(r["tile_slot"]),
           L.ptr(r["tile_list"]), L.ptr(r["n_act"]), L.ptr(ws), L.stream())
    r["_ws"] = ws
    return r


def decoder_tiles(ep: "EncoderPlan", sources, H: int, W: int) -> DecoderTiles:
    sources = tuple(int(v) for v in sources)
    dt = ep.dec_tiles
    if dt is not None and dt.sources == sources and dt.H == H and dt.W == W:
        return dt
    st = [ep.stages[i] for i in sources]
    B = st[0].B
    ups = [H // sp.Y for sp in st]
    assert all(sp.Y * u == H and sp.X * u == W for sp, u in zip(st, ups))
    r = _decoder_tiles_launch([sp.map for sp in st], ups, B, H, W, st[0].map.device)
    n = int(r["n_act"].item())
    ep.dec_tiles = DecoderTiles(sources, B, H, W, n, r["tile_slot"], r["tile_list"][:n], _site_rulebooks(st, ups, r["tile_slot"], H, W))
    return ep.dec_tiles


def decoder_site_rulebooks(dt: "DecoderTiles", sites, ups):
    out = []
    for st, u in zip(sites, ups):
        n_dev = torch.tensor([st.numel() // (u * u)], dtype=I32, device=st.device)
        nbr = _empty(st.numel() * 9, I32, st.device)
        L.call("gdmae_decoder_site_rulebook", L.ptr(st.contiguous()), L.ptr(n_dev), u * u, st.numel(), L.ptr(dt.tile_slot), dt.H, dt.W,
               L.ptr(nbr), L.stream())
        out.append(nbr.view(-1, 9))
    return out


def _site_rulebooks(stages, ups, tile_slot, H, W):
    out = []
    for sp, u in zip(stages, ups):
        sites = sp.tok_cell if u == 1 else (sp._up_sites[1] if getattr(sp, "_up_sites", None) is not None and sp._up_sites[0] == u
                                            else upsample_cells(sp.tok_cell, sp.Y, sp.X, u).reshape(-1).contiguous())
        n_dev = torch.tensor([sp.n_tok], dtype=I32, device=tile_slot.device)
        nbr = _empty(sites.numel() * 9, I32, tile_slot.device)
        L.call("gdmae_decoder_site_rulebook", L.ptr(sites.contiguous()), L.ptr(n_dev), u * u, sites.numel(), L.ptr(tile_slot), H, W, L.ptr(nbr),
               L.stream())
        out.append(nbr.view(-1, 9))
    return out


def _encoder_launch(vox, m_cap: int, strides, window_shapes, drop_infos, keep_frac, noise, dec_sources=None) -> dict:
    if isinstance(vox, dict):
        dev, grid, B = vox["src"].device, vox["grid"], vox["batch_size"]
        sample_off, pillar_cell, vcounts = vox["sample_off"], vox["pillar_cell"], vox["counts"]
    else:
        dev, grid, B = vox.points.device, vox.grid, vox.batch_size
        sample_off, pillar_cell, vcounts = vox.sample_off, vox.pillar_cell, vox.counts
    gx, gy, gz = grid
    assert gz == 1, "the SST backbone works on single-layer pillar grids (spt_backbone_mae.py:94)"
    lib = L.load()
    st = L.stream()
    M = m_cap
    scan_ws = _empty(8 * (max(B * gx * gy, M) // 4096 + 4), torch.int64, dev)

    if keep_frac is not None:
        if noise is None:
            noise = torch.rand(max(M, 1), device=dev, dtype=torch.float32)
        assert noise.numel() >= 1 and noise.dtype == torch.float32
        mask = _empty(max(M, 1), torch.float32, dev)
        len_keep = _empty(B, I32, dev)
        L.call("gdmae_random_mask", L.ptr(noise.contiguous()), L.ptr(sample_off), B, float(keep_frac), L.ptr(mask),
               L.ptr(len_keep), st)
    else:
        mask = torch.zeros(max(M, 1), dtype=torch.float32, device=dev)

    cap = max(M, 1)
    Y, X = gy, gx
    tok_pillar = _empty(cap, I32, dev)
    tok_cell = _empty(cap, I32, dev)
    smap = _empty(B * Y * X, I32, dev)
    n_tok = _empty(1, I32, dev)
    L.call("gdmae_visible_tokens", L.ptr(mask), L.ptr(pillar_cell), L.ptr(vcounts), M, B * Y * X,
           L.ptr(tok_pillar), L.ptr(tok_cell), L.ptr(smap), L.ptr(n_tok), L.ptr(scan_ws), st)

    raw = []
    for si, stride in enumerate(strides):
        if stride > 1:
            assert stride == 2, "only the k3 s2 p1 strided sparse conv of the shipped configs is implemented"
            Yi, Xi = Y, X
            Y, X = (Yi - 1) // 2 + 1, (Xi - 1) // 2 + 1
            cap_in = cap
            cap = min(4 * cap_in, B * Y * X)
            tok_cell_n = _empty(cap, I32, dev)
            smap_n = _empty(B * Y * X, I32, dev)
            n_tok_n = _empty(1, I32, dev)
            flag = _empty(B * Y * X, I32, dev)
            L.call("gdmae_downsample_tokens", L.ptr(n_tok), L.ptr(tok_cell), cap_in, B, Yi, Xi, L.ptr(tok_cell_n),
                   L.ptr(smap_n), L.ptr(n_tok_n), L.ptr(flag), L.ptr(scan_ws), st)
            nbr_down = _empty(cap * 9, I32, dev)
            L.call("gdmae_rulebook", L.ptr(n_tok_n), L.ptr(tok_cell_n), cap, B, Y, X, Yi, Xi, L.ptr(smap), 1,
                   L.ptr(nbr_down), st)
            nbr_down_t = _empty(cap_in * 9, I32, dev)
            L.call("gdmae_rulebook", L.ptr(n_tok), L.ptr(tok_cell), cap_in, B, Yi, Xi, Y, X, L.ptr(smap_n), 2,
                   L.ptr(nbr_down_t), st)
            tok_cell, smap, n_tok = tok_cell_n, smap_n, n_tok_n
        else:
            nbr_down = nbr_down_t = None
        nbr_subm = _empty(cap * 9, I32, dev)
        L.call("gdmae_rulebook", L.ptr(n_tok), L.ptr(tok_cell), cap, B, Y, X, Y, X, L.ptr(smap), 0, L.ptr(nbr_subm), st)
        wx, wy, wz = (int(v) for v in window_shapes[si])
        assert wz == 1
        dlo, dhi, dT = _drop_arrays(drop_infos[si])
        assert wx * wy <= max(dT), "token drop would not be the identity: unsupported (SURVEY header item 5)"
        wsb = lib.gdmae_window_workspace_bytes(B, Y, X, wx, wy)
        wins = []
        for shifted in (0, 1):
            nwin_cap = B * ((X + wx - 1) // wx + 1) * ((Y + wy - 1) // wy + 1)
            w = dict(tok_win=_empty(cap, I32, dev), tok_level=_empty(cap, I32, dev), tok_slot=_empty(cap, I32, dev),
                     tok_pos=_empty(cap, I32, dev), csr_tok=_empty(cap, I32, dev),
                     win_start=_empty(min(nwin_cap, cap), I32, dev), win_len=_empty(min(nwin_cap, cap), I32, dev),
                     counts=_empty(8, I32, dev), T=dT)
            ws = _empty(wsb, torch.uint8, dev)
            L.call("gdmae_window_partition", L.ptr(smap), B, Y, X, wx, wy, shifted, len(dT), L.host_i32(dlo),
                   L.host_i32(dhi), L.host_i32(dT), L.ptr(w["tok_win"]), L.ptr(w["tok_level"]), L.ptr(w["tok_slot"]),
                   L.ptr(w["tok_pos"]), L.ptr(w["csr_tok"]), L.ptr(w["win_start"]), L.ptr(w["win_len"]),
                   L.ptr(w["counts"]), L.ptr(ws), wsb, st)
            w["_ws"] = ws
            wins.append(w)
        nbr_subm_t = torch.flip(nbr_subm.view(cap, 9), dims=[1]).contiguous().view(-1)
        up_s = gy // Y
        up_sites = upsample_cells(tok_cell, Y, X, up_s) if (up_s > 1 and up_s * Y == gy and up_s * X == gx) else None
        raw.append(dict(B=B, Y=Y, X=X, cap=cap, tok_cell=tok_cell, map=smap, n_tok=n_tok, nbr_subm=nbr_subm,
                        nbr_subm_t=nbr_subm_t, up_s=up_s, up_sites=up_sites, nbr_down=nbr_down, nbr_down_t=nbr_down_t, wins=wins))
    dec = None
    if dec_sources is not None:
        srcs = [raw[int(i)] for i in dec_sources]
        if all(r["up_s"] * r["Y"] == gy and r["up_s"] * r["X"] == gx and r["up_s"] in (1, 2, 4, 8) for r in srcs):
            dec = _decoder_tiles_launch([r["map"] for r in srcs], [r["up_s"] for r in srcs], B, gy, gx, dev)
            dec["sources"] = tuple(int(i) for i in dec_sources)
    counts = torch.cat([r["n_tok"] for r in raw] + [w["counts"] for r in raw for w in r["wins"]]
                       + ([dec["n_act"]] if dec is not None else []))
    return dict(stages=raw, mask=mask, tok_pillar=tok_pillar, masked=keep_frac is not None, counts=counts,
                keep=(noise, scan_ws), dec=dec)


def _encoder_finalize(e: dict, allc, M: int) -> EncoderPlan:
    raw = e["stages"]
    ns = len(raw)
    stages = []
    for si, r in enumerate(raw):
        n = int(allc[si])
        wps = []
        for k, w in enumerate(r["wins"]):
            c = allc[ns + 8 * (2 * si + k): ns + 8 * (2 * si + k) + 8]
            assert c[7] == n, (c, n)
            nw = int(c[6])
            wps.append(WindowPlan(w["tok_win"][:n], w["tok_level"][:n], w["tok_slot"][:n], w["tok_pos"][:n],
                                  w["csr_tok"][:n], w["win_start"][:nw], w["win_len"][:nw],
                                  [int(v) for v in c[0:3]], [int(v) for v in c[3:6]], list(w["T"])))
        n_prev = int(allc[si - 1]) if r["nbr_down"] is not None else 0
        stages.append(StagePlan(r["B"], r["Y"], r["X"], n, r["tok_cell"][:n], r["map"],
                                r["nbr_subm"][:n * 9].view(n, 9),
                                None if r["nbr_down"] is None else r["nbr_down"][:n * 9].view(n, 9),
                                None if r["nbr_down_t"] is None else r["nbr_down_t"][:n_prev * 9].view(n_prev, 9),
                                wps))
        stages[-1]._nbr_subm_t = r["nbr_subm_t"][:n * 9].view(n, 9)
        stages[-1]._up_sites = None if r["up_sites"] is None else (r["up_s"], r["up_sites"][:n].reshape(-1))
    dec = e.get("dec", None)
    dt = None
    if dec is not None:
        n_act = int(allc[ns + 16 * ns])
        dt = DecoderTiles(dec["sources"], dec["B"], dec["H"], dec["W"], n_act, dec["tile_slot"], dec["tile_list"][:n_act])
    return EncoderPlan(e["mask"][:M] if e["masked"] else None, e["tok_pillar"][:stages[0].n_tok], stages, dt)


def encoder_plan(vox: VoxelPlan, strides, window_shapes, drop_infos, keep_frac: Optional[float] = None,
                 noise: Optional[torch.Tensor] = None, dec_sources=None) -> EncoderPlan:
    if noise is not None:
        assert noise.shape == (vox.M,)
    e = _encoder_launch(vox, vox.M, strides, window_shapes, drop_infos, keep_frac, noise, dec_sources)
    return _encoder_finalize(e, e["counts"].tolist(), vox.M)


import collections
import time as _time

EVENT_WAIT_S = 0.0

_PLAN_SHAPES = collections.OrderedDict()
_PLAN_SHAPES_MAX = 32
_PLAN_GRANULE = 16384
_PINNED = {}


def _plan_shape(n0, ncols, B, pcr, voxel_size, grid_size, strides, window_shapes, drop_infos, keep_frac, dec_sources):
    gx, gy, gz = (int(g) for g in grid_size)
    lo = tuple(float(v) for v in pcr[:3])
    vs = tuple(float(v) for v in voxel_size)
    drops = tuple(tuple(map(tuple, _drop_arrays(d))) for d in drop_infos)
    n_exact = n0
    n0 = max(1, (n0 + _PLAN_GRANULE - 1) // _PLAN_GRANULE) * _PLAN_GRANULE
    key = (n0, ncols, B, lo, vs, (gx, gy, gz), tuple(int(s) for s in strides), tuple(tuple(int(v) for v in w) for w in window_shapes),
           drops, None if keep_frac is None else float(keep_frac), None if dec_sources is None else tuple(int(i) for i in dec_sources))
    hit = _PLAN_SHAPES.get(key)
    if hit is not None:
        _PLAN_SHAPES.move_to_end(key)
        return hit
    del n_exact
    import ctypes as C
    ns = len(strides)
    assert gz == 1, "the SST backbone works on single-layer pillar grids (spt_backbone_mae.py:94)"
    assert 1 <= ns <= 4
    P = L.PlanParams()
    P.n_points, P.cap_points, P.n_cols, P.batch_size = n0, n0, ncols, B
    for i in range(3):
        P.lo[i], P.vs[i] = lo[i], vs[i]
        P.grid[i] = (gx, gy, gz)[i]
    P.n_stages = ns
    geo = []
    Y, X = gy, gx
    cap = max(1, min(n0, B * gx * gy))
    m_cap = cap
    for i in range(ns):
        wx, wy, wz = (int(v) for v in window_shapes[i])
        assert wz == 1
        dlo, dhi, dT = drops[i]
        assert wx * wy <= max(dT), "token drop would not be the identity: unsupported (SURVEY header item 5)"
        P.stride[i], P.win_x[i], P.win_y[i], P.n_levels[i] = int(strides[i]), wx, wy, len(dT)
        for l in range(len(dT)):
            P.drop_lo[i][l], P.drop_hi[i][l], P.max_tokens[i][l] = dlo[l], dhi[l], dT[l]
        cap_in = cap
        if int(strides[i]) > 1:
            assert int(strides[i]) == 2, "only the k3 s2 p1 strided sparse conv of the shipped configs is implemented"
            Y, X = (Y - 1) // 2 + 1, (X - 1) // 2 + 1
            cap = min(4 * cap, B * Y * X)
        us = gy // Y
        up_s = us if (us >= 1 and us * Y == gy and us * X == gx) else 0
        geo.append(dict(Y=Y, X=X, cap=cap, cap_in=cap_in, up_s=up_s, strided=int(strides[i]) > 1, T=list(dT)))
    P.masked = int(keep_frac is not None)
    P.keep_frac = float(keep_frac) if keep_frac is not None else 1.0
    P.n_dec = 0 if dec_sources is None else len(dec_sources)
    for g in range(P.n_dec):
        P.dec_sources[g] = int(dec_sources[g])
    P.want_pm = 1
    table = (L.PlanBuffer * 160)()
    n_ent, total = C.c_int(0), C.c_size_t(0)
    L.call("gdmae_geometry_plan_layout", C.byref(P), table, 160, C.byref(n_ent), C.byref(total))
    names = {table[i].name.decode(): (int(table[i].offset), int(table[i].bytes)) for i in range(n_ent.value)}
    hit = _PLAN_SHAPES[key] = (P, names, int(total.value), geo, m_cap, (lo, vs, (gx, gy, gz)))
    while len(_PLAN_SHAPES) > _PLAN_SHAPES_MAX:
        _PLAN_SHAPES.popitem(last=False)
    return hit


class _Arena:

    def __init__(self, raw, names):
        self.raw, self.names = raw, names
        self.base = {torch.int32: raw.view(torch.int32), torch.float32: raw.view(torch.float32), torch.int64: raw.view(torch.int64)}

    def has(self, name):
        return name in self.names

    def view(self, name, dtype, *shape):
        off, _ = self.names[name]
        es = 8 if dtype == torch.int64 else 4
        strides, acc = [], 1
        for d in reversed(shape):
            strides.append(acc)
            acc *= int(d)
        return self.base[dtype].as_strided(tuple(int(d) for d in shape), tuple(reversed(strides)), off // es)


class PlanPrefetch:

    _side = {}
    _arena_bytes = {}

    def __init__(self, points, point_cloud_range, voxel_size, grid_size, batch_size, strides, window_shapes, drop_infos,
                 keep_frac=None, noise=None, ready=None, dec_sources=None):
        import ctypes as C
        assert points.is_cuda and points.dtype == torch.float32 and points.dim() == 2
        points = points.contiguous()
        dev = points.device
        main = torch.cuda.current_stream(dev)
        side = PlanPrefetch._side.setdefault(dev.index, torch.cuda.Stream(device=dev))
        side.wait_stream(main)
        if ready is not None:
            side.wait_event(ready)
        points.record_stream(side)
        if noise is not None:
            noise.record_stream(side)
        n0, ncols = points.shape
        P, names, total, geo, m_cap, _ = self.shape = _plan_shape(n0, ncols, int(batch_size), point_cloud_range, voxel_size, grid_size,
                                                                    strides, window_shapes, drop_infos, keep_frac, dec_sources)
        self.masked, self.dec_sources, self.batch_size, self.ncols = keep_frac is not None, dec_sources, int(batch_size), ncols
        with torch.cuda.stream(side):
            cap = PlanPrefetch._arena_bytes.get(dev.index, 0)
            if total > cap:
                cap = PlanPrefetch._arena_bytes[dev.index] = -(-total // (64 << 20)) * (64 << 20)
            raw = torch.empty(cap, dtype=torch.uint8, device=dev)
            if self.masked and noise is None:
                noise = torch.rand(m_cap, device=dev, dtype=torch.float32)
            if noise is not None:
                assert noise.dtype == torch.float32 and noise.numel() >= 1
                noise = noise.contiguous()
            Pc = L.PlanParams.from_buffer_copy(P)
            Pc.n_points = n0
            L.call("gdmae_geometry_plan", C.byref(Pc), L.ptr(points), None if noise is None else L.ptr(noise), L.ptr(raw), total, L.stream())
            self.arena = _Arena(raw, names)
            nc = names["counts"][1] // 4
            assert nc <= 256
            free = _PINNED.setdefault(dev.index, [])
            self._pinned = free.pop() if free else torch.empty(256, dtype=torch.int32).pin_memory()
            self.host = self._pinned[:nc]
            self.host.copy_(self.arena.view("counts", torch.int32, nc), non_blocking=True)
            self.event = torch.cuda.Event()
            self.event.record(side)
        self.side, self.keep, self.points = side, noise, points
        self.serial = side == main

    def finish(self):
        assert self.serial or torch.cuda.current_stream() != self.side, "plan tensors must not be consumed on the plan stream"
        global EVENT_WAIT_S
        t_w = _time.perf_counter()
        self.event.synchronize()
        EVENT_WAIT_S += _time.perf_counter() - t_w
        torch.cuda.current_stream().wait_event(self.event)
        c = self.host.tolist()
        self.points_device = self.points.device
        self.host = None
        if self._pinned is not None:
            _PINNED.setdefault(self.points_device.index, []).append(self._pinned)
            self._pinned = None
        P, names, total, geo, m_cap, (lo, vs, grid) = self.shape
        A, V = self.arena, self.arena.view
        i32, f32, i64 = torch.int32, torch.float32, torch.int64
        B, ncols = self.batch_size, self.ncols
        F = ncols - 1
        N, M = int(c[0]), int(c[1])
        gx, gy, gz = grid
        vox = VoxelPlan(B, grid, lo, vs, ncols, N, M, V("points", f32, N, ncols), V("point_coords", i64, N, 4), V("inverse", i64, N),
                        V("inverse32", i32, N), V("voxel_coords", i64, M, 4), V("pillar_cell", i32, M), V("pt_off", i32, M + 1),
                        V("pillar_pts", i32, N), V("point_rank", i32, N), V("sample_off", i32, B + 1), V("pillar_mean", f32, M, F),
                        V("cell2pillar", i32, B * gx * gy * gz), V("counts", i32, 2), V("points_pm", f32, N, ncols), V("row_pillar", i32, N))
        vox._arena = A
        ns = len(geo)
        n_vis = int(c[2 + ns + 16 * ns + 1])
        stages = []
        for i, g in enumerate(geo):
            n = int(c[2 + i])
            pre = f"s{i}."
            wps = []
            for k in range(2):
                wc = c[2 + ns + 16 * i + 8 * k: 2 + ns + 16 * i + 8 * k + 8]
                assert wc[7] == n, (wc, n)
                nw = int(wc[6])
                wpre = f"{pre}w{k}."
                wps.append(WindowPlan(V(wpre + "tok_win", i32, n), V(wpre + "tok_level", i32, n), V(wpre + "tok_slot", i32, n),
                                      V(wpre + "tok_pos", i32, n), V(wpre + "csr_tok", i32, n), V(wpre + "win_start", i32, nw),
                                      V(wpre + "win_len", i32, nw), [int(v) for v in wc[0:3]], [int(v) for v in wc[3:6]], list(g["T"])))
            n_prev = (int(c[2 + i - 1]) if i > 0 else n_vis) if g["strided"] else 0
            sp = StagePlan(B, g["Y"], g["X"], n, V(pre + "tok_cell", i32, n), V(pre + "map", i32, B * g["Y"] * g["X"]),
                           V(pre + "nbr_subm", i32, n, 9), V(pre + "nbr_down", i32, n, 9) if g["strided"] else None,
                           V(pre + "nbr_down_t", i32, n_prev, 9) if g["strided"] else None, wps)
            sp._nbr_subm_t = V(pre + "nbr_subm_t", i32, n, 9)
            sp._up_sites = (g["up_s"], V(pre + "up_sites", i32, n * g["up_s"] * g["up_s"])) if g["up_s"] > 1 else None
            stages.append(sp)
        dt = None
        if A.has("dec.tile_slot"):
            n_act = int(c[2 + ns + 16 * ns])
            nt = B * ((gy + 7) // 8) * ((gx + 7) // 8)
            nbrs = [V(f"dec.nbr{g}", i32, stages[int(si)].n_tok * geo[int(si)]["up_s"] ** 2, 9) for g, si in enumerate(self.dec_sources)]
            dt = DecoderTiles(tuple(int(i) for i in self.dec_sources), B, gy, gx, n_act, V("dec.tile_slot", i32, nt), V("dec.tile_list", i32, n_act),
                              nbrs)
        ep = EncoderPlan(V("mask", f32, M) if self.masked else None, V("tok_pillar", i32, stages[0].n_tok if not geo[0]["strided"] else n_vis),
                         stages, dt)
        self.arena = self.points = self.keep = None
        return vox, ep


def _tensors_of(obj):
    out = []
    if isinstance(obj, torch.Tensor):
        if obj.is_cuda:
            out.append(obj)
    elif isinstance(obj, dict):
        for v in obj.values():
            out += _tensors_of(v)
    elif isinstance(obj, (list, tuple)):
        for v in obj:
            out += _tensors_of(v)
    return out
```

gd-mae_amd/gdmae_hip/vfe.py:

```python
from __future__ import annotations

import torch

from . import bn as gbn
from . import lib as L
from . import ops


def _bf(t):
    return int(t.dtype == torch.bfloat16)


class BNReLURows(torch.autograd.Function):

    @staticmethod
    def forward(ctx, x, gamma, beta, eps, bn=None, residual=None, partials=None):
        x = x.contiguous()
        n, C = x.shape
        stats, ab, mv = gbn.fold(x, n, gamma, beta, eps, bn, partials)
        out = torch.empty_like(x)
        if residual is not None:
            assert residual.shape == x.shape and residual.dtype == x.dtype and residual.is_contiguous() and C % 8 == 0
            L.call("gdmae_rows_affine_relu_add", L.ptr(x), _bf(x), n, C, L.ptr(ab), L.ptr(ab[C:]), L.ptr(residual), L.ptr(out), _bf(out),
                   L.stream())
        else:
            L.call("gdmae_rows_affine_relu_scatter", L.ptr(x), _bf(x), None, n, C, L.ptr(ab), L.ptr(ab[C:]), L.ptr(out), _bf(out), C, 0,
                   L.stream())
        ctx.has_res = residual is not None
        ctx.save_for_backward(x, ab, stats, gamma.detach())
        ctx.direct = gbn.direct_pair(gamma, beta)
        mf, vf = mv[:C], mv[C:]
        ctx.mark_non_differentiable(mf, vf)
        ctx.set_materialize_grads(False)
        return out, mf, vf

    @staticmethod
    def backward(ctx, g, _m, _v):
        if g is None:
            return None, None, None, None, None, None, None
        x, ab, stats, gamma = ctx.saved_tensors
        n, C = x.shape
        g = g.contiguous()
        st = torch.empty(3 * C, dtype=torch.float64, device=x.device)
        ws = torch.empty(L.load().gdmae_rows_bwd_stats_workspace_bytes(C), dtype=torch.uint8, device=x.device)
        L.call("gdmae_rows_bwd_stats", L.ptr(x), _bf(x), None, n, C, L.ptr(ab), L.ptr(ab[C:]), L.ptr(g), _bf(g), C, 0, L.ptr(st),
               L.ptr(ws), L.stream())
        dgamma, dbeta, c01 = gbn.bwd_coeffs(st, 3, stats, ab, gamma, n, None, ctx.direct)
        dx = torch.empty_like(x)
        L.call("gdmae_rows_bwd", L.ptr(x), _bf(x), None, n, C, L.ptr(ab), L.ptr(ab[C:]), L.ptr(c01), L.ptr(c01[C:]), L.ptr(g),
               _bf(g), C, 0, L.ptr(dx), _bf(dx), L.stream())
        return dx, dgamma, dbeta, None, None, (g if ctx.has_res else None), None


class BNReLURowsCat(torch.autograd.Function):

    @staticmethod
    def forward(ctx, bns, eps, *args):
        xs = [a.contiguous() for a in args[0::3]]
        gammas, betas = args[1::3], args[2::3]
        n, Ct = xs[0].shape[0], sum(x.shape[1] for x in xs)
        assert all(x.shape[0] == n and x.dtype == xs[0].dtype and x.shape[1] % 8 == 0 for x in xs)
        out = torch.empty(n, Ct, dtype=xs[0].dtype, device=xs[0].device)
        saved, col = [], 0
        for x, g_, b_, bn in zip(xs, gammas, betas, bns):
            C = x.shape[1]
            stats, ab, _ = gbn.fold(x, n, g_, b_, eps, bn)
            L.call("gdmae_rows_affine_relu_scatter", L.ptr(x), _bf(x), None, n, C, L.ptr(ab), L.ptr(ab[C:]), L.ptr(out), _bf(out), Ct, col,
                   L.stream())
            saved += [x, ab, stats, g_.detach()]
            col += C
        ctx.save_for_backward(*saved)
        ctx.direct = [gbn.direct_pair(g_, b_) for g_, b_ in zip(gammas, betas)]
        return out

    @staticmethod
    def backward(ctx, g):
        sv = ctx.saved_tensors
        g = g.contiguous()
        n, Ct = g.shape
        grads, col = [None, None], 0
        for i in range(len(sv) // 4):
            x, ab, stats, gamma = sv[4 * i:4 * i + 4]
            C = x.shape[1]
            st = torch.empty(3 * C, dtype=torch.float64, device=x.device)
            ws = torch.empty(L.load().gdmae_rows_bwd_stats_workspace_bytes(C), dtype=torch.uint8, device=x.device)
            L.call("gdmae_rows_bwd_stats", L.ptr(x), _bf(x), None, n, C, L.ptr(ab), L.ptr(ab[C:]), L.ptr(g), _bf(g), Ct, col, L.ptr(st),
                   L.ptr(ws), L.stream())
            dgamma, dbeta, c01 = gbn.bwd_coeffs(st, 3, stats, ab, gamma, n, None, ctx.direct[i])
            dx = torch.empty_like(x)
            L.call("gdmae_rows_bwd", L.ptr(x), _bf(x), None, n, C, L.ptr(ab), L.ptr(ab[C:]), L.ptr(c01), L.ptr(c01[C:]), L.ptr(g), _bf(g),
                   Ct, col, L.ptr(dx), _bf(dx), L.stream())
            grads += [dx, dgamma, dbeta]
            col += C
        return tuple(grads)


class _BnChannels:

    def __init__(self, bn, c0, c1, count_batch):
        self.training, self.momentum = bn.training, bn.momentum
        self.running_mean = None if bn.running_mean is None else bn.running_mean[c0:c1]
        self.running_var = None if bn.running_var is None else bn.running_var[c0:c1]
        self.num_batches_tracked = bn.num_batches_tracked if count_batch else torch.zeros_like(bn.num_batches_tracked)


def point_layer2_max(y1, row_pillar, weight, bn, pt_off):
    C = weight.shape[0]
    if C == 128:
        return PointLayer2Max.apply(y1, row_pillar, weight, bn.weight, bn.bias, bn.eps, pt_off, bn)[0]
    assert C % 128 == 0
    nb = C // 128
    ys = ops.FanOut.apply(y1, nb) if (y1.requires_grad and torch.is_grad_enabled()) else (y1,) * nb
    outs = []
    for b in range(nb):
        c0, c1 = 128 * b, 128 * (b + 1)
        outs.append(PointLayer2Max.apply(ys[b], row_pillar, weight[c0:c1], bn.weight[c0:c1], bn.bias[c0:c1], bn.eps, pt_off,
                                         _BnChannels(bn, c0, c1, b == 0))[0])
    return torch.cat(outs, dim=1)


class BNReLUSegmentMax(torch.autograd.Function):

    @staticmethod
    def forward(ctx, x, gamma, beta, eps, pt_off, pillar_pts, inverse32, bn=None):
        x = x.contiguous()
        n, C = x.shape
        M = pt_off.numel() - 1
        stats, ab, mv = gbn.fold(x, n, gamma, beta, eps, bn)
        out = torch.empty(M, C, dtype=torch.float32, device=x.device)
        arg = torch.empty(M, C, dtype=torch.int32, device=x.device)
        L.call("gdmae_segment_max_affine", L.ptr(x), _bf(x), L.ptr(pt_off), L.ptr(pillar_pts), M, C, L.ptr(ab), L.ptr(ab[C:]),
               L.ptr(out), L.ptr(arg), L.stream())
        ctx.save_for_backward(x, out, arg, inverse32, ab, stats, gamma.detach())
        ctx.direct = gbn.direct_pair(gamma, beta)
        mf, vf = mv[:C], mv[C:]
        ctx.mark_non_differentiable(mf, vf)
        ctx.set_materialize_grads(False)
        return out, mf, vf

    @staticmethod
    def backward(ctx, g, _m, _v):
        if g is None:
            return (None,) * 8
        x, out, arg, inv, ab, stats, gamma = ctx.saved_tensors
        n, C = x.shape
        M = out.shape[0]
        g = g.float().contiguous()
        st = torch.empty(2 * C, dtype=torch.float64, device=x.device)
        ws = torch.empty(L.load().gdmae_rows_bwd_stats_workspace_bytes(C), dtype=torch.uint8, device=x.device)
        L.call("gdmae_segmax_bwd_stats", L.ptr(x), _bf(x), L.ptr(out), L.ptr(arg), L.ptr(g), M, C, L.ptr(ab), L.ptr(ab[C:]),
               L.ptr(st), L.ptr(ws), L.stream())
        dgamma, dbeta, c01 = gbn.bwd_coeffs(st, 2, stats, ab, gamma, n, None, ctx.direct)
        dx = torch.empty_like(x)
        L.call("gdmae_segmax_bn_bwd", L.ptr(x), _bf(x), L.ptr(out), L.ptr(arg), L.ptr(g), L.ptr(inv), n, C, L.ptr(ab), L.ptr(c01),
               L.ptr(c01[C:]), L.ptr(dx), _bf(dx), L.stream())
        return dx, dgamma, dbeta, None, None, None, None, None


class PointLayer1(torch.autograd.Function):

    @staticmethod
    def forward(ctx, vox, weight, gamma, beta, eps, bn=None, pillar_major=False, out_f16=False):
        dev = weight.device
        C, D = weight.shape
        assert weight.dtype == torch.float32 and weight.is_contiguous() and D == vox.n_cols + 5
        odt = torch.bfloat16 if torch.is_autocast_enabled() else torch.float32
        if out_f16:
            odt = torch.float16
        n = int(vox.N)
        out = torch.empty(n, C, dtype=odt, device=dev)
        stats = torch.empty(2 * C, dtype=torch.float64, device=dev)
        ab = torch.empty(2 * C, dtype=torch.float32, device=dev)
        mv = torch.empty(2 * C, dtype=torch.float32, device=dev)
        ws = torch.empty(L.load().gdmae_vfe_point_layer_workspace_bytes(vox.n_cols), dtype=torch.uint8, device=dev)
        ctx.pm = bool(pillar_major)
        rm = rv = nb = None
        mom = 0.0
        if bn is not None and bn.training and bn.running_mean is not None:
            rm, rv, nb, mom = bn.running_mean, bn.running_var, bn.num_batches_tracked, float(bn.momentum)
        L.call("gdmae_vfe_point_layer_fwd", *PointLayer1._geometry(vox, ctx.pm), L.ptr(weight), C, L.ptr(gamma), L.ptr(beta),
               float(eps), mom, L.ptr(rm) if rm is not None else None, L.ptr(rv) if rv is not None else None,
               L.ptr(nb) if nb is not None else None, L.ptr(stats), L.ptr(ab), L.ptr(mv), L.ptr(out), 2 if out_f16 else _bf(out), L.ptr(ws),
               L.stream())
        ctx.vox, ctx.ws = vox, ws
        ctx.save_for_backward(weight, gamma.detach(), stats, ab)
        ctx.direct = (ops.direct_grad(weight), *gbn.direct_pair(gamma, beta))
        mf, vf = mv[:C], mv[C:]
        ctx.mark_non_differentiable(mf, vf)
        ctx.set_materialize_grads(False)
        return out, mf, vf

    @staticmethod
    def _geometry(vox, pm):
        if pm:
            assert vox.points_pm is not None and vox.row_pillar is not None
            return (L.ptr(vox.points_pm), L.ptr(vox.voxel_coords), L.ptr(vox.row_pillar), L.ptr(vox.pillar_mean), 1,
                    int(vox.N), vox.n_cols, L.host_f32(vox.lo), L.host_f32(vox.vs))
        return (L.ptr(vox.points), L.ptr(vox.point_coords), L.ptr(vox.inverse32), L.ptr(vox.pillar_mean), 0, int(vox.N),
                vox.n_cols, L.host_f32(vox.lo), L.host_f32(vox.vs))

    @staticmethod
    def backward(ctx, g, _m, _v):
        if g is None:
            return (None,) * 8
        weight, gamma, stats, ab = ctx.saved_tensors
        vox, C = ctx.vox, weight.shape[0]
        g = g.contiguous()
        assert g.dtype in (torch.float32, torch.bfloat16)
        dw, dg, db = ctx.direct
        acc = int(dw is not None and dg is not None and db is not None)
        if not acc:
            dw = torch.empty_like(weight)
            dgb = torch.empty(2 * C, dtype=torch.float32, device=weight.device)
            dg, db = dgb[:C], dgb[C:]
        L.call("gdmae_vfe_point_layer_bwd", *PointLayer1._geometry(vox, ctx.pm), L.ptr(weight), C, L.ptr(gamma), L.ptr(stats),
               L.ptr(ab), L.ptr(g), _bf(g), L.ptr(dg), L.ptr(db), L.ptr(dw), acc, L.ptr(ctx.ws), L.stream())
        if acc:
            return None, None, None, None, None, None, None, None
        return None, dw, dg, db, None, None, None, None


class PointLayer2Max(torch.autograd.Function):

    @staticmethod
    def forward(ctx, y1, row_pillar, weight, gamma, beta, eps, pt_off, bn=None):
        dev = y1.device
        C, K = weight.shape
        assert (C, K) == (128, 64) and y1.dtype in (torch.bfloat16, torch.float16) and y1.is_contiguous() and y1.shape[1] == K
        assert row_pillar.dtype == torch.int32 and row_pillar.numel() == y1.shape[0]
        n, M = y1.shape[0], pt_off.numel() - 1
        f16 = y1.dtype == torch.float16
        wb = weight.detach().contiguous() if f16 else ops.shadow(weight, torch.bfloat16).contiguous()
        assert not f16 or wb.dtype == torch.float32
        ctx.f16 = f16
        out = torch.empty(M, C, dtype=torch.float32, device=dev)
        arg = torch.empty(M, C, dtype=torch.int32, device=dev)
        stats = torch.empty(2 * C, dtype=torch.float64, device=dev)
        ab = torch.empty(2 * C, dtype=torch.float32, device=dev)
        mv = torch.empty(2 * C, dtype=torch.float32, device=dev)
        ws = torch.empty(L.load().gdmae_vfe_max_layer_workspace_bytes(), dtype=torch.uint8, device=dev)
        rm = rv = nb = None
        mom = 0.0
        if bn is not None and bn.training and bn.running_mean is not None:
            rm, rv, nb, mom = bn.running_mean, bn.running_var, bn.num_batches_tracked, float(bn.momentum)
        L.call("gdmae_vfe_max_layer_fwd_f16" if f16 else "gdmae_vfe_max_layer_fwd", L.ptr(y1), n, L.ptr(wb), L.ptr(pt_off), L.ptr(row_pillar), M, L.ptr(gamma),
               L.ptr(beta), float(eps), mom, L.ptr(rm) if rm is not None else None, L.ptr(rv) if rv is not None else None,
               L.ptr(nb) if nb is not None else None, L.ptr(stats), L.ptr(ab), L.ptr(mv), L.ptr(out), L.ptr(arg), L.ptr(ws),
               L.stream())
        ctx.ws = ws
        ctx.save_for_backward(y1, row_pillar, wb, gamma.detach(), stats, ab, out, arg)
        ctx.direct = (ops.direct_grad(weight), *gbn.direct_pair(gamma, beta))
        mf, vf = mv[:C], mv[C:]
        ctx.mark_non_differentiable(mf, vf)
        ctx.set_materialize_grads(False)
        return out, mf, vf

    @staticmethod
    def backward(ctx, g, _m, _v):
        if g is None:
            return (None,) * 8
        y1, row_pillar, wb, gamma, stats, ab, out, arg = ctx.saved_tensors
        n, (M, C) = y1.shape[0], out.shape
        g = g.float().contiguous()
        dw, dg, db = ctx.direct
        acc = int(dw is not None and dg is not None and db is not None)
        if not acc:
            dw = torch.empty(C, y1.shape[1], dtype=torch.float32, device=y1.device)
            dgb = torch.empty(2 * C, dtype=torch.float32, device=y1.device)
            dg, db = dgb[:C], dgb[C:]
        gm = torch.empty_like(out)
        dy1 = torch.empty(y1.shape, dtype=torch.bfloat16, device=y1.device)
        L.call("gdmae_vfe_max_layer_bwd_f16" if ctx.f16 else "gdmae_vfe_max_layer_bwd", L.ptr(y1), n, L.ptr(wb), L.ptr(row_pillar), M, L.ptr(gamma), L.ptr(stats), L.ptr(ab),
               L.ptr(out), L.ptr(arg), L.ptr(g), L.ptr(gm), L.ptr(dy1), L.ptr(dg), L.ptr(db), L.ptr(dw), acc,
               L.ptr(ctx.ws), L.stream())
        if acc:
            return dy1, None, None, None, None, None, None, None
        return dy1, None, dw, dg, db, None, None, None



class _StandInCtx:

    def __init__(self):
        self.saved_tensors = ()
        self.needs_input_grad = ()

    def save_for_backward(self, *ts):
        self.saved_tensors = ts

    def mark_non_differentiable(self, *ts):
        pass

    def set_materialize_grads(self, flag):
        pass


class PointLayers12Max(torch.autograd.Function):

    @staticmethod
    def forward(ctx, vox, w1, g1, b1, eps1, bn1, w2, g2, b2, eps2, bn2):
        c1 = _StandInCtx()
        y1, _, _ = PointLayer1.forward(c1, vox, w1, g1, b1, eps1, bn1, True, True)
        C2 = w2.shape[0]
        assert C2 % 128 == 0
        c2s, outs = [], []
        for blk in range(C2 // 128):
            lo, hi = 128 * blk, 128 * (blk + 1)
            c2 = _StandInCtx()
            if C2 == 128:
                o, _, _ = PointLayer2Max.forward(c2, y1, vox.row_pillar, w2, g2, b2, eps2, vox.pt_off, bn2)
            else:
                o, _, _ = PointLayer2Max.forward(c2, y1, vox.row_pillar, w2[lo:hi], g2[lo:hi], b2[lo:hi], eps2, vox.pt_off,
                                                 _BnChannels(bn2, lo, hi, blk == 0))
                dwf, dgf, dbf = ops.direct_grad(w2), *gbn.direct_pair(g2, b2)
                if dwf is not None and dgf is not None and dbf is not None:
                    c2.direct = (dwf[lo:hi], dgf[lo:hi], dbf[lo:hi])
            c2s.append(c2), outs.append(o)
        saved, counts = list(c1.saved_tensors), [len(c1.saved_tensors)]
        c1.saved_tensors = ()
        for c2 in c2s:
            saved += list(c2.saved_tensors)
            counts.append(len(c2.saved_tensors))
            c2.saved_tensors = ()
        ctx.save_for_backward(*saved)
        ctx.c1, ctx.c2s, ctx.counts = c1, c2s, counts
        ctx.set_materialize_grads(False)
        return outs[0] if len(outs) == 1 else torch.cat(outs, dim=1)

    @staticmethod
    def backward(ctx, g):
        if g is None:
            return (None,) * 11
        sv, pos = ctx.saved_tensors, 0
        c1, c2s = ctx.c1, ctx.c2s
        c1.saved_tensors = sv[pos:pos + ctx.counts[0]]
        pos += ctx.counts[0]
        dy1s, dw2, dg2, db2 = [], [], [], []
        acc2 = True
        for i, c2 in enumerate(c2s):
            c2.saved_tensors = sv[pos:pos + ctx.counts[i + 1]]
            pos += ctx.counts[i + 1]
            r = PointLayer2Max.backward(c2, g[:, 128 * i:128 * (i + 1)], None, None)
            c2.saved_tensors = ()
            dy1s.append(r[0])
            acc2 = acc2 and r[2] is None
            dw2.append(r[2]), dg2.append(r[3]), db2.append(r[4])
        if len(dy1s) == 1:
            dy1 = dy1s[0]
        else:
            dy1 = torch.empty_like(dy1s[0])
            L.call("gdmae_sum_bf16", L.host_ptrs(dy1s), len(dy1s), dy1.numel(), L.ptr(dy1), L.stream())
        r1 = PointLayer1.backward(c1, dy1, None, None)
        c1.saved_tensors = ()
        cat = (lambda ts: None if acc2 else torch.cat(ts, dim=0))
        return (None, r1[1], r1[2], r1[3], None, None, cat(dw2), cat(dg2), cat(db2), None, None)
```

include/gdmae_hip.h:

```cpp
#ifndef GDMAE_HIP_H
#define GDMAE_HIP_H

#include <stddef.h>
#include <stdint.h>

#ifdef __cplusplus
extern "C" {
#endif

int gdmae_abi_version(void);
const char* gdmae_target_arch(void);
const char* gdmae_last_error(void);

size_t gdmae_voxelize_workspace_bytes(long long n_points, int batch_size, int gx, int gy, int gz);
int gdmae_voxelize(const float* points, long long n_points, int n_cols, const float* lo, const float* vs,
                   const int* grid_xyz, int batch_size, float* points_out, long long* point_coords,
                   long long* inverse, int* inverse32, long long* voxel_coords, int* pillar_cell,
                   int* pillar_pt_off, int* pillar_pts, int* point_rank, int* sample_pillar_off,
                   float* pillar_mean, int* cell2pillar, int* counts, void* workspace, size_t workspace_bytes,
                   void* stream);

int gdmae_decorate_points(const float* points, const long long* point_coords, const int* inverse32,
                          const float* pillar_mean, long long N, int n_cols, const float* lo, const float* vs,
                          float* out, void* stream);
int gdmae_pillar_major_rows(const float* points, int n_cols, const int* pillar_pts, const int* inverse32, const int* n_dev,
                            long long capacity, float* points_pm, int* row_pillar, void* stream);
int gdmae_vfe_infer(const float* points_pm, const long long* voxel_coords, const int* row_pillar, const float* pillar_mean,
                    long long N, long long M, int n_cols, const float* lo, const float* vs, const float* W1, const float* b1,
                    int c1, const float* W2, const float* b2, int c2, float* out, void* stream);
size_t gdmae_vfe_point_layer_workspace_bytes(int n_cols);
int gdmae_vfe_point_layer_fwd(const float* points, const long long* point_coords, const int* inverse32,
                              const float* pillar_mean, int coords_per_pillar, long long N, int n_cols, const float* lo,
                              const float* vs,
                              const float* W, int C, const float* gamma, const float* beta, double eps, double momentum,
                              float* running_mean, float* running_var, long long* num_batches, double* stats, float* ab,
                              float* mv, void* out, int out_bf16, void* workspace, void* stream);
int gdmae_vfe_point_layer_bwd(const float* points, const long long* point_coords, const int* inverse32,
                              const float* pillar_mean, int coords_per_pillar, long long N, int n_cols, const float* lo,
                              const float* vs,
                              const float* W, int C, const float* gamma, const double* stats, const float* ab,
                              const void* g, int g_bf16, float* dgamma, float* dbeta, float* dW, int accumulate,
                              void* workspace, void* stream);
size_t gdmae_vfe_max_layer_workspace_bytes(void);
int gdmae_vfe_max_layer_fwd(const void* y1, long long N, const void* W, const int* pillar_pt_off, const int* row_pillar,
                            int M, const float* gamma, const float* beta, double eps, double momentum,
                            float* running_mean, float* running_var, long long* num_batches, double* stats, float* ab,
                            float* mv, float* out, int* arg, void* workspace, void* stream);
int gdmae_vfe_max_layer_bwd(const void* y1, long long N, const void* W, const int* row_pillar, int M, const float* gamma,
                            const double* stats, const float* ab, const float* out, const int* arg, const float* g, void* gm,
                            void* dy1, float* dgamma, float* dbeta, float* dW, int accumulate,
                            void* workspace, void* stream);
int gdmae_vfe_max_layer_fwd_f16(const void* y1, long long N, const float* W, const int* pillar_pt_off, const int* row_pillar,
                                int M, const float* gamma, const float* beta, double eps, double momentum,
                                float* running_mean, float* running_var, long long* num_batches, double* stats, float* ab,
                                float* mv, float* out, int* arg, void* workspace, void* stream);
int gdmae_vfe_max_layer_bwd_f16(const void* y1, long long N, const float* W, const int* row_pillar, int M, const float* gamma,
                                const double* stats, const float* ab, const float* out, const int* arg, const float* g, void* gm,
                                void* dy1, float* dgamma, float* dbeta, float* dW, int accumulate,
                                void* workspace, void* stream);
int gdmae_segment_max(const float* x, const int* pillar_pt_off, const int* pillar_pts, int M, int C, float* out,
                      int* arg, void* stream);
int gdmae_segment_max_bwd(const float* dout, const int* arg, const int* inverse32, long long N, int C, float* dx,
                          void* stream);

int gdmae_random_mask(const float* noise, const int* sample_pillar_off, int batch_size, double keep_frac,
                      float* mask_out, int* len_keep_out, void* stream);

int gdmae_visible_tokens(const float* mask, const int* pillar_cell, const int* vox_counts, long long m_cap,
                         long long n_cells, int* tok_pillar, int* tok_cell, int* map, int* n_tok, void* scan_ws,
                         void* stream);
int gdmae_downsample_tokens(const int* n_in, const int* tok_cell_in, long long cap_in, int B, int Yi, int Xi,
                            int* tok_cell_out, int* map_out, int* n_out, int* flag_ws, void* scan_ws, void* stream);
int gdmae_rulebook(const int* n_tok, const int* tok_cell, long long cap, int B, int Yt, int Xt, int Ym, int Xm,
                   const int* map, int mode, int* nbr, void* stream);

size_t gdmae_window_workspace_bytes(int B, int Y, int X, int wx, int wy);
int gdmae_window_partition(const int* map, int B, int Y, int X, int wx, int wy, int shifted, int nlev,
                           const int* drop_lo, const int* drop_hi, const int* max_tokens, int* tok_win,
                           int* tok_level, int* tok_slot, int* tok_pos, int* csr_tok, int* win_start, int* win_len,
                           int* counts, void* workspace, size_t workspace_bytes, void* stream);

int gdmae_gather_rows(const void* src, const int* idx, long long n_slots, int row_bytes, void* out, void* stream);
int gdmae_scatter_rows(const void* src, const int* idx, long long n_rows, int row_bytes, void* dst, void* stream);

int gdmae_gather_rows_strided(const void* src, const int* idx, long long n_slots, int row_bytes, int table_row_bytes,
                              int table_col_bytes, void* out, void* stream);
int gdmae_scatter_rows_strided(const void* src, const int* idx, long long n_rows, int row_bytes, int table_row_bytes,
                               int table_col_bytes, void* dst, void* stream);
size_t gdmae_colstats_workspace_bytes(int C);
int gdmae_colstats(const void* x, long long R, int C, int is_bf16, double* out, void* workspace, void* stream);

size_t gdmae_decoder_region_workspace_bytes(int C2, int Cin);
int gdmae_decoder_region_algebra(const double* stats2, const float* ab2, const double* st2, const float* k01,
                                 const double* reg, const double* tap_region, const double* cnt, double R, int C2, int Cin,
                                 const float* conv_w, const void* bgz, int cdt_bf16, double* S, double* tot, float* dWk,
                                 void* Wd, void* workspace, void* stream);
int gdmae_fill_rows(const void* v, long long R, int C, int elem_bytes, void* Z, void* stream);
int gdmae_rows_affine_relu_scatter(const void* P, int p_bf16, const int* site, long long n, int C, const float* a,
                                   const float* b, void* Z, int z_bf16, int z_row_elems, int col0, void* stream);
int gdmae_rows_affine_relu_sub(const void* P, int p_bf16, const int* site, long long n, int C, const float* a, const float* b,
                               const void* sub, void* Z, int z_bf16, int z_row_elems, int col0, void* stream);
int gdmae_rows_affine_relu_add(const void* P, int p_bf16, long long n, int C, const float* a, const float* b, const void* R, void* Z,
                               int z_bf16, void* stream);
size_t gdmae_rows_bwd_stats_workspace_bytes(int C);
int gdmae_rows_bwd_stats(const void* P, int p_bf16, const int* site, long long n, int C, const float* a, const float* b,
                         const void* dZ, int z_bf16, int z_row_elems, int col0, double* out, void* workspace, void* stream);
int gdmae_rows_bwd(const void* P, int p_bf16, const int* site, long long n, int C, const float* a, const float* b,
                   const float* c0, const float* c1, const void* dZ, int z_bf16, int z_row_elems, int col0, void* dP,
                   int dp_bf16, void* stream);

int gdmae_bn_fold(const void* x, long long R, int C, int is_bf16, double count, const float* gamma, const float* beta,
                  double eps, double momentum, float* running_mean, float* running_var, long long* num_batches,
                  double* stats, float* ab, float* mv, void* workspace, void* stream);
int gdmae_bn_fold_partials(const float* part, int nblk, int C, double count, const float* gamma, const float* beta, double eps,
                           double momentum, float* running_mean, float* running_var, long long* num_batches, double* stats, float* ab,
                           float* mv, void* stream);
int gdmae_bn_bwd_coeffs(const double* st, int n_st, const double* stats, const float* ab, const float* gamma, int C,
                        double count, const double* tot, float* dgamma, float* dbeta, int accumulate, float* c01,
                        void* stream);
int gdmae_rows_bwd_stats_rows(long long n);
int gdmae_bn_bwd_coeffs_rows(const float* part, int nblk, int n_st, const double* stats, const float* ab, const float* gamma, int C,
                             double count, const double* tot, float* dgamma, float* dbeta, int accumulate, float* c01,
                             void* stream);

int gdmae_conv3x3_grad_taps(const void* Y, int y_bf16, const int* tile_slot, const void* ybg, const float* k0,
                            const float* k1, const float* rows, const int* cell2pillar, const int* site, long long n, int H,
                            int W, int C, void* out, void* stream);

size_t gdmae_border_sums_workspace_bytes(int B, int C);
int gdmae_border_sums(const void* Y, int y_bf16, const int* tile_slot, const void* ybg, const float* rows,
                      const int* pillar_cell, int M, int B, int H, int W, int C, double* out, void* workspace, void* stream);

size_t gdmae_decoder_tiles_workspace_bytes(int B, int H, int W);
int gdmae_decoder_tiles(const int* const* maps, const int* strides, int k, int B, int H, int W, int* tile_slot, int* tile_list,
                        int* n_act, void* workspace, void* stream);
size_t gdmae_conv3x3_tiles_packed_bytes(int k);
int gdmae_conv3x3_tiles_pack(const float* conv_w, int C2, int Cin, const float* const* b, int k, void* Wp, void* bgz, void* ybg,
                             void* stream);
size_t gdmae_conv3x3_tiles_workspace_bytes(int n_act);
int gdmae_conv3x3_tiles_fwd(const void* const* P, const int* const* maps, const float* const* a, const float* const* b,
                            const int* strides, int k, const void* Wp, const void* ybg, const int* tile_list, int n_act, int B,
                            int H, int W, void* Yc, const float* gamma, const float* beta, double eps, double momentum,
                            float* running_mean, float* running_var, long long* num_batches, double* stats, float* ab,
                            float* mv, void* workspace, void* stream);
int gdmae_tiles_gather_rows(const void* Yc, const int* tile_slot, const void* ybg, const int* cell, long long n, int H, int W,
                            int C, int elem_bytes, void* out, void* stream);
int gdmae_tiles_to_dense(const void* Yc, const int* tile_slot, const void* ybg, int B, int H, int W, int C, int elem_bytes,
                         void* out, void* stream);
int gdmae_tiles_to_dense_affine_relu(const void* Yc, const int* tile_slot, const void* ybg, int B, int H, int W, int C, const float* a,
                                     const float* b, float* out, void* stream);

int gdmae_segment_max_affine(const void* x, int x_bf16, const int* pillar_pt_off, const int* pillar_pts, int M, int C,
                             const float* a, const float* b, float* out, int* arg, void* stream);
int gdmae_segmax_bwd_stats(const void* x, int x_bf16, const float* out, const int* arg, const float* dout, long long M,
                           int C, const float* a ,
                           const float* b, double* sums, void* workspace, void* stream);
int gdmae_segmax_bn_bwd(const void* x, int x_bf16, const float* out, const int* arg, const float* dout,
                        const int* inverse32, long long N, int C, const float* a, const float* c0, const float* c1,
                        void* dx, int dx_bf16, void* stream);

int gdmae_set_attention_impl(int impl);
int gdmae_window_attention_fwd(const void* qk, const void* v, void* out, int io_bf16, const int* csr_tok,
                               const int* win_start, const int* win_len, int n_win, int T, int d, int H,
                               const float* tau, float tau_min, void* stream);
int gdmae_window_attention_bwd(const void* qk, const void* v, const void* dout, void* dqk, void* dv, int io_bf16,
                               float* dtau_part, const int* csr_tok, const int* win_start, const int* win_len,
                               int n_win, int T, int d, int H, const float* tau, float tau_min, void* stream);
int gdmae_window_attention_levels_writes_lse(int io_bf16, int n_levels, const int* max_tokens, int d, int H);
int gdmae_window_attention_levels_fwd(const void* qk, const void* v, void* out, int io_bf16, const int* csr_tok,
                                      const int* win_start, const int* win_len, int n_levels, const int* n_win,
                                      const int* max_tokens, int d, int H, const float* tau, float tau_min, float* lse, void* stream);
int gdmae_window_attention_levels_bwd(const void* qk, const void* v, const void* dout, void* dqk, void* dv, int io_bf16,
                                      float* dtau_part, const int* csr_tok, const int* win_start, const int* win_len,
                                      int n_levels, const int* n_win, const int* max_tokens, int d, int H, const float* tau,
                                      float tau_min, const void* out, const float* lse, void* stream);
int gdmae_attention_timing(int on);
int gdmae_attention_timing_read(int which, double* total_ms, long long* calls);
int gdmae_kernel_timing(int on);
int gdmae_kernel_timing_slots(void);
const char* gdmae_kernel_timing_name(int slot);
int gdmae_kernel_timing_read(int slot, double* total_ms, long long* calls, double* bytes, double* flops);
int gdmae_kernel_timing_read_side(int slot, double* side_bytes);
int gdmae_weighted_mean_finish(const float* term, const float* weights, long long n, float* out, void* stream);
int gdmae_sum_partials(const float* part, long long n, float scale, float* out, int accumulate, void* stream);
int gdmae_sum_partials_gated(const float* part, long long n, float scale, float* out, const float* gate, float gate_min,
                             void* stream);

size_t gdmae_add_layernorm_workspace_bytes(int d);
int gdmae_add_layernorm_fwd(const float* a, const void* b, int b_is_bf16, const float* gamma, const float* beta,
                            long long n, int d, float eps, float* y, float* stats, void* y_bf16 ,
                            void* stream);
int gdmae_add_layernorm_bwd(const float* a, const void* b, int b_is_bf16, const float* gamma, const float* stats,
                            const float* dy, const void* dy2, int dy2_bf16, long long n, int d, float* dx, void* dx_bf16,
                            float* sums, void* workspace, void* stream);
int gdmae_prep_tokens(const float* x, const float* pos_table, const int* tok_pos, long long n, int d, void* x_out,
                      void* xpos_out, int out_bf16, void* stream);
int gdmae_sum_bf16(const void* const* src, int k, long long total, void* out, void* stream);
int gdmae_add3(const float* a, const void* b, int b_bf16, const void* c, int c_bf16, long long total, float* out, void* stream);
int gdmae_add3_to(const float* a, const void* b, int b_bf16, const void* c, int c_bf16, long long total, void* out, int out_bf16,
                  void* stream);

int gdmae_gemm_stats(long long* calls);
int gdmae_gemm_tuning(int mode);
size_t gdmae_gemm_workspace_bytes(void);
int gdmae_gemm(const void* A, const void* B, void* C, long long M, long long N, long long K, int trans_a, int trans_b,
               int ab_bf16, int c_f32, const void* bias, void* workspace, void* stream);
size_t gdmae_gemm_tn_splitk_workspace_bytes(long long K, int m, int n);
int gdmae_gemm_tn_splitk(const void* A, const void* B, float* C, long long K, int m, int n, int ab_bf16, int accumulate,
                         void* workspace, void* stream);

size_t gdmae_dw_gemm_workspace_bytes(long long rows, int M, int N);
int gdmae_dw_gemm(const void* G, const void* X, long long rows, int M, int N, float* dW, float* dbias, void* workspace,
                  void* stream);

typedef struct gdmae_conv_block_args {
  long long n_in, n_out;
  int cin, cout, bf16, x_f32, g_f32;
  float eps, momentum;
  const void* x;
  const int* nbr;
  const int* nbr_t;
  const void* W;
  const float *gamma, *beta;
  float *running_mean, *running_var;
  long long* num_batches;
  void* cols;
  void* y;
  double* stats;
  float* ab;
  float* mv;
  void* out;
  const void* g;
  void* dx;
  float *dW, *dgamma, *dbeta;
  void* scratch;
  const void* packed_fwd;
  const void* packed_bwd;
  int out_f32;
} gdmae_conv_block_args;
size_t gdmae_conv_block_scratch_bytes(long long n_in, long long n_out, int cin, int cout, int bf16);
size_t gdmae_spconv_packed_bytes(int cin, int cout);
int gdmae_spconv_pack_jobs(const float* W , int cin, int cout, int transposed, void* packed, long long* jobs);
int gdmae_spconv(const void* X, int x_f32, const int* nbr, const void* packed, long long n, int cin, int cout, void* Y,
                 int timing_slot , void* stream);
int gdmae_spconv_bias_relu(const void* X, int x_f32, const int* nbr, const void* packed, const float* bias, long long n, int cin, int cout,
                           void* Y, void* stream);
int gdmae_spconv_stat_rows(int cin, int cout, int x_f32);
int gdmae_spconv_stats(const void* X, int x_f32, const int* nbr, const void* packed, long long n, int cin, int cout, void* Y, float* part,
                       void* stream);
int gdmae_decoder_dy(const void* Yc, const int* tile_list, int n_act, const float* k0, const float* k1, const float* rows,
                     const int* cell2pillar, int H, int W, int C, void* dYc, void* stream);
int gdmae_decoder_site_rulebook(const int* site, const int* n_dev, int sites_per_tok, long long cap_sites, const int* tile_slot,
                                int H, int W, int* nbr, void* stream);
long long gdmae_tap_dw_rows(long long n, int M, int N);
size_t gdmae_tap_dw_workspace_bytes(long long n, int M, int N);
int gdmae_tap_dw(const void* G, long long n, long long n_pad, int M, const void* X, const int* nbr, int N, float* out, int ld_out,
                 int m_off, void* workspace, void* stream);
int gdmae_conv_block_fwd(const gdmae_conv_block_args* args , void* stream);
int gdmae_conv_block_bwd(const gdmae_conv_block_args* args , void* stream);

typedef struct gdmae_layer_args {
  long long n;
  int d, ff, nhead, bf16;
  float eps, tau_min;
  int n_levels;
  int n_win[4], max_tokens[4];
  const int* tok_pos;
  const int* csr_tok;
  const int* win_start;
  const int* win_len;
  const float* pos_table;
  const void *Win, *bin, *Wo, *bo, *W1, *b1, *W2, *b2;
  const float *g1, *be1, *g2, *be2, *tau;
  const float* x;
  float* y;
  const float* dy;
  float* dx;
  float *dWin, *dbin, *dtau, *dWo, *dbo, *dW1, *db1, *dW2, *db2, *dg1, *dbe1, *dg2, *dbe2;
  void* saved;
  void* scratch;
  const void* packed;
  int x_bf16;
  void* res_out;
  const void* dres;
  void* dx_bf16;
  int path;
} gdmae_layer_args;
size_t gdmae_layer_packed_bytes(int d, int ff);
int gdmae_layer_pack_jobs(const float* Win, const float* Wo, const float* W1, const float* W2, int d, int ff, void* packed,
                          long long* jobs_host );
int gdmae_layer_pack_job_count(int d, int ff);
int gdmae_tok_gemm_pack(const long long* jobs_dev, int n_jobs, void* stream);
int gdmae_tok_gemm(const void* X, const void* Wp, const void* bias, long long n, long long n_pad, int K, int N, int epilogue,
                   void* out0, void* out1, const void* aux, const float* res, const float* gamma, const float* beta, float eps,
                   float* y, float* stats, void* y_bf16, const float* pos_table, const int* tok_pos, void* ypos_bf16,
                   void* stream);

int gdmae_tok_gemm_qkv(const void* Xpos, const void* X, const void* Wp_qk, const void* Wp_v, const void* bias3, long long n_pad,
                       int d, void* qk, void* v, void* stream);

int gdmae_tok_gemm_ffn(const void* X, const void* W1p, const void* b1, const void* W2p, const void* b2, long long n, long long n_pad,
                       int d, void* h, const float* res, const float* gamma, const float* beta, float eps, float* y, float* stats,
                       void* y_bf16, const float* pos_table, const int* tok_pos, void* ypos_bf16, void* f_out, void* stream);

int gdmae_tok_gemm_ln_bwd_rows(int N);
int gdmae_tok_gemm_ln_bwd(const void* X, const void* Wp, long long n, long long n_pad, int K, int N, const float* dy,
                          const void* dy2_bf16, const float* ln_a, const void* ln_b_bf16, const float* stats,
                          const float* gamma, float* dx, void* dx_bf16, float* part, void* stream);
int gdmae_encoder_layer_bytes(long long n, int d, int ff, int nhead, int bf16, size_t* saved_bytes,
                              size_t* fwd_scratch_bytes, size_t* bwd_scratch_bytes);
int gdmae_encoder_layer_fwd(const gdmae_layer_args* args , void* stream);
int gdmae_encoder_layer_bwd(const gdmae_layer_args* args , void* stream);
int gdmae_encoder_stage_fwd(const gdmae_layer_args* layers , int n_layers, void* stream);
int gdmae_encoder_stage_bwd(const gdmae_layer_args* layers , int n_layers, void* stream);
int gdmae_encoder_set_layer_path(int path);
int gdmae_encoder_stage_fused(const gdmae_layer_args* layers , int n_layers);

size_t gdmae_deconv_rows_packed_bytes(int cin, int cout, int s);
int gdmae_deconv_rows_pack(const float* weight, int cin, int cout, int s, void* packed_fwd, void* packed_bwd, void* stream);
int gdmae_deconv_rows_fwd(const void* X, long long n, int cin, int cout, int s, const void* packed_fwd, void* P, void* stream);
int gdmae_deconv_rows_bwd_input(const void* dP, long long n, int cin, int cout, int s, const void* packed_bwd, void* dX, void* stream);
size_t gdmae_deconv_rows_dw_workspace_bytes(long long n, int cin, int cout, int s);
int gdmae_deconv_rows_bwd_weight(const void* X, const void* dP, long long n, int cin, int cout, int s, float* dW, void* workspace,
                                 void* stream);

size_t gdmae_pred_head_packed_bytes(void);
int gdmae_pred_head_pack(const float* weight, const float* bias, int n_in, int n_out, void* packed, void* stream);
int gdmae_pred_head_fwd(const float* X, long long n, int n_out, const void* packed, void* Y, void* X_bf16 , float* Y_f32 ,
                        void* stream);
size_t gdmae_pred_head_bwd_workspace_bytes(long long n);
int gdmae_pred_head_bwd(const void* dY, int dy_f32 ,
                        void* dY_bf16 ,
                        const float* scale_a, const float* scale_b ,
                        const void* X_bf16, long long n, int n_out,
                        const void* packed, float* dX, float* dW, float* db, void* workspace, void* stream);

size_t gdmae_conv3x3_dense_packed_bytes(int cin, int cout);
int gdmae_conv3x3_dense_pack(const float* weight, int cin, int cout, int dil, int transposed, void* packed, void* stream);
int gdmae_conv3x3_dense(const void* X, int B, int H, int W, int cin_l, int cout_l, int dil, const void* packed, const float* bias,
                        void* Y, void* stream);
int gdmae_conv3x3_dense_add(const void* X, int B, int H, int W, int cin_l, int cout_l, int dil, const void* packed, const float* bias,
                            const void* addend, void* Y, void* stream);
int gdmae_conv3x3_dense_relu(const void* X, int B, int H, int W, int cin_l, int cout_l, int dil, const void* packed, const float* bias,
                             const void* shortcut, void* Y, void* stream);
size_t gdmae_conv3x3_dense_stats_workspace_bytes(int B, int H, int W, int cout_l);
int gdmae_conv3x3_dense_stat_rows(void);
int gdmae_conv3x3_dense_stats(const void* X, int B, int H, int W, int cin_l, int cout_l, int dil, const void* packed, const float* bias,
                              void* Y, float* stat_rows, void* workspace, void* stream);
int gdmae_conv3x3_dense_f32out(const void* X, int B, int H, int W, int cin_l, int cout_l, int dil, const void* packed, const float* bias,
                               float* Y, int accumulate, void* stream);
size_t gdmae_conv3x3_dense_dw_workspace_bytes(int B, int H, int W, int cin_l, int cout_l);
int gdmae_conv3x3_dense_bwd_weight(const void* X, const void* dY, int B, int H, int W, int cin_l, int cout_l, int cin, int cout, int dil,
                                   float* dW, void* workspace, void* stream);

int gdmae_group_gt_points(const float* points, int n_cols, const int* pillar_pt_off, const int* pillar_pts,
                          const long long* voxel_coords, int M, int K, const float* lo, const float* vs,
                          float* gt_points, int* gt_index, void* stream);
int gdmae_chamfer(const float* pred, const float* gt, const float* weights, int M, int P1, int P2, float* term,
                  float* dpred, void* stream);

size_t gdmae_augment_collate_workspace_bytes(long long n_raw);
int gdmae_augment_collate(const float* raw, long long n_raw, int F, const int* frame_off, int B, const float* frame_params,
                          const float* xy_range , float* out, int* kept_off, void* workspace, void* stream);

size_t gdmae_group_workspace_bytes(long long n, long long n_groups);
int gdmae_ingroup_inds(const long long* group_inds, long long n, long long n_groups, long long* out_inds,
                       void* workspace, size_t workspace_bytes, void* stream);
int gdmae_group_inner_inds(const long long* inverse_inds, long long n, long long M, int K, long long* group_inds,
                           void* workspace, size_t workspace_bytes, void* stream);

#define GDMAE_PLAN_MAX_STAGES 4
typedef struct gdmae_plan_params {
  long long n_points;
  int n_cols, batch_size;
  float lo[3], vs[3];
  int grid[3];
  int n_stages;
  int stride[GDMAE_PLAN_MAX_STAGES];
  int win_x[GDMAE_PLAN_MAX_STAGES], win_y[GDMAE_PLAN_MAX_STAGES];
  int n_levels[GDMAE_PLAN_MAX_STAGES];
  int drop_lo[GDMAE_PLAN_MAX_STAGES][3], drop_hi[GDMAE_PLAN_MAX_STAGES][3], max_tokens[GDMAE_PLAN_MAX_STAGES][3];
  int masked;
  double keep_frac;
  int n_dec;
  int dec_sources[GDMAE_PLAN_MAX_STAGES];
  int want_pm;
  long long cap_points;
} gdmae_plan_params;
typedef struct gdmae_plan_buffer {
  char name[40];
  long long offset, bytes;
} gdmae_plan_buffer;
int gdmae_geometry_plan_layout(const gdmae_plan_params* p, gdmae_plan_buffer* table, int max_entries, int* n_entries,
                               size_t* total_bytes);
int gdmae_geometry_plan(const gdmae_plan_params* p, const float* points, const float* noise, void* arena, size_t arena_bytes,
                        void* stream);

size_t gdmae_center_head_targets_workspace_bytes(int B, int num_max_objs);
int gdmae_center_head_targets(const float* gt_boxes, int B, int n_max, int box_dim, const int* class_map, int n_class_total,
                              int n_cls, const float* pc_range , const float* voxel_size ,
                              float feature_map_stride, int fw, int fh, int num_max_objs, double gaussian_overlap, int min_radius,
                              float* heatmap, float* ret_boxes, long long* inds, long long* mask, void* workspace, void* stream);
int gdmae_focal_loss_rows(void);
int gdmae_focal_loss_fwd(const void* logits, int logits_bf16, const long long* strides_byxc, const float* gt, int B, int C, int H, int W,
                         float* prob, float* partials, float* out4, void* stream);
int gdmae_focal_loss_bwd(const void* logits, int logits_bf16, const long long* strides_byxc, const float* gt, int B, int C, int H, int W,
                         const float* out4, const float* grad_out, void* dlogits, int dlogits_bf16, void* stream);
int gdmae_center_head_targets_iou(const float* gt_boxes, int B, int n_max, int box_dim, const int* class_map, int n_class_total,
                                  int n_cls, const float* pc_range, const float* voxel_size, float feature_map_stride, int fw, int fh,
                                  int num_max_objs, double gaussian_overlap, int min_radius, float* heatmap, float* ret_boxes,
                                  float* iou_boxes, long long* inds, long long* mask, void* workspace, void* stream);
int gdmae_center_head_decode(const long long* cell, const float* score, const float* center, const float* center_z,
                             const float* dim, const float* rot, const float* vel, const float* iou, int B, int K, int H, int W,
                             const float* pc_range , const float* voxel_size ,
                             float feature_map_stride, const float* post_center_limit_range , float score_thresh,
                             int use_score_thresh, float* boxes, int* labels, float* ious, unsigned char* valid, void* stream);

int gdmae_boxes_bev_pairs(const float* boxes_a, int n, const float* boxes_b, int m, int mode, float* out, void* stream);
size_t gdmae_nms_workspace_bytes(int n);
int gdmae_nms_bev(const float* boxes, int n, float thresh, int rotated, long long* keep, int* n_keep, void* workspace,
                  void* stream);

size_t gdmae_anchor_targets_workspace_bytes(int B, int n_cls, int n_max);
int gdmae_anchor_targets(const float* gt_boxes, int B, int n_max, int box_dim, int H, int W, int K, int n_cls, int n_names,
                         const int* name_idx, const int* slot_cls, const float* xr, const float* yr, const float* xc, const float* yc,
                         const float* slot, const float* matched, const float* unmatched, float dir_offset, int num_bins,
                         int* labels, int* gt_ids, float* reg_targets, int* dir_bins, int* num_pos, void* workspace, void* stream);
int gdmae_anchor_loss_rows(void);
int gdmae_anchor_loss_fwd(const void* rows, int rows_bf16, int ld, int B, int n_loc, int K, int C, int nb, const int* labels,
                          const float* reg_targets, const int* dir_bins, const int* num_pos, const float* code_weights,
                          const float* scale, float* partials, float* out4, void* stream);
int gdmae_anchor_loss_bwd(const void* rows, int rows_bf16, int ld, int B, int n_loc, int K, int C, int nb, const int* labels,
                          const float* reg_targets, const int* dir_bins, const int* num_pos, const float* code_weights,
                          const float* scale, const float* grad3, void* drows, void* stream);
int gdmae_anchor_decode(const void* rows, int rows_bf16, int ld, int B, int H, int W, int K, int C, int nb, const float* xc,
                        const float* yc, const float* slot, float dir_offset, float dir_limit_offset, float* cls_out, float* boxes,
                        void* stream);
int gdmae_anchor_select(const float* cls, int B, int n, int C, int normalized, float thresh, int* idx, float* score, int* label,
                        int* count, void* stream);

size_t gdmae_anchor_head_infer_packed_bytes(int cin);
int gdmae_anchor_head_infer_pack(const float* w_cls, const float* b_cls, const float* w_box, const float* b_box, const float* w_dir,
                                 const float* b_dir, int cin, int K, int C, int nb, void* packed, void* stream);
size_t gdmae_anchor_head_infer_workspace_bytes(int B, int H, int W, int K);
int gdmae_anchor_head_infer(const void* X, int B, int H, int W, int cin, int K, int C, int nb, const void* packed, const float* xc,
                            const float* yc, const float* slot, float dir_offset, float dir_limit_offset, float thresh,
                            float* rows_out, int* count, int* idx, float* score, int* label, float* box, void* workspace,
                            void* stream);

int gdmae_grad_sq_norm(const float* grad, long long n, float* partials , float* sq_norm_out, void* stream);
int gdmae_adam_step(float* param, const float* grad, float* exp_avg, float* exp_avg_sq, const long long* segments,
                    int n_segments, float lr, float beta1, float beta2, float eps, float weight_decay, int step,
                    float max_norm, float grad_scale, const float* sq_norm, void* stream);
int gdmae_adam_step_shadow(float* param, const float* grad, float* exp_avg, float* exp_avg_sq, const long long* segments,
                           int n_segments, float lr, float beta1, float beta2, float eps, float weight_decay, int step,
                           float max_norm, float grad_scale, const float* sq_norm, void* param_bf16, void* stream);

#ifdef __cplusplus
}
#endif
#endif
```

Before: 1083.

## Derive VFE point-layer BN statistics from a precomputed feature Gram matrix

Adds a kernel that accumulates the first and second moments (a Gram matrix) of the per-point VFE input features in double precision during planning. For a linear layer, the BatchNorm mean and variance of each output channel then follow from W·mu and W·G·W^T, so a separate statistics pass over all points is no longer needed. In backward, a new PDW mode folds the sums of dh into the dW pass, using the Gram for the BN backward coefficients. Gram use is on by default for backward and opt-in for forward via an env var. This adds an extra pass over the points in planning and may lose precision, since variance is computed as a difference of second moments.

```diff
diff --git a/gd-mae_amd/csrc/plan.hip b/gd-mae_amd/csrc/plan.hip
--- a/gd-mae_amd/csrc/plan.hip
+++ b/gd-mae_amd/csrc/plan.hip
@@ -8,6 +8,10 @@
                      int* sample_pillar_off, float* pillar_mean, int* cell2pillar_out, int* counts, void* workspace, size_t workspace_bytes,
                      void* lb_state, float* points_pm, int* row_pillar, hipStream_t st);
 size_t gd_voxelize_lb_state_bytes(long long n_points, long long cells);
+extern "C" size_t gdmae_vfe_feature_gram_workspace_bytes(int n_cols);
+int gd_vfe_feature_gram(hipStream_t st, const float* points, const long long* point_coords, const int* inverse32, const float* pillar_mean,
+                        int coords_per_pillar, long long N, const int* n_dev, int n_cols, const float* lo, const float* vs, double* gram,
+                        void* workspace);
 size_t gd_plan_scan_state_bytes(long long n);
 size_t gd_plan_win_state_bytes(long long n);
 int gd_plan_visible_tokens(const float* mask, const int* cell2pillar, long long n_cells, int* tok_pillar, int* tok_cell, int* map,
@@ -85,7 +89,7 @@
 
 struct Offsets {
   long long lb_state, counts, points, point_coords, inverse, inverse32, voxel_coords, pillar_cell, pt_off, pillar_pts, point_rank,
-      sample_off, pillar_mean, cell2pillar, points_pm, row_pillar, vox_ws, mask, len_keep, tok_pillar;
+      sample_off, pillar_mean, cell2pillar, points_pm, row_pillar, vox_ws, feat_gram, gram_ws, mask, len_keep, tok_pillar;
   long long vis_tok_cell, vis_map;
   struct {
     long long tok_cell, map, nbr_subm, nbr_subm_t, nbr_down, nbr_down_t, up_sites, win_ws;
@@ -175,6 +179,12 @@
   O.row_pillar = L.add("row_pillar", sizeof(int) * cap);
   O.vox_ws_bytes = gdmae_voxelize_workspace_bytes(n0, B, gx, gy, 1);
   O.vox_ws = L.add("vox_ws", O.vox_ws_bytes);
+  O.feat_gram = O.gram_ws = -1;
+  if (F >= 3 && F <= 5) {
+    const int D = F + 6;
+    O.feat_gram = L.add("feat_gram", sizeof(double) * (D + D * (D + 1) / 2));
+    O.gram_ws = L.add("gram_ws", gdmae_vfe_feature_gram_workspace_bytes(p->n_cols));
+  }
   O.mask = L.add("mask", sizeof(float) * O.m_cap);
   O.len_keep = L.add("len_keep", sizeof(int) * B);
   O.tok_pillar = L.add("tok_pillar", sizeof(int) * O.m_cap);
@@ -257,6 +267,17 @@
                               p->want_pm ? I(O.row_pillar) : nullptr, st);
     if (rc) return rc;
     lb += gd_voxelize_lb_state_bytes(p->n_points, O.cells);
+    if (O.feat_gram >= 0) {
+      if (p->want_pm)
+        rc = gd_vfe_feature_gram(st, (const float*)(A + O.points_pm), (const long long*)(A + O.voxel_coords), I(O.row_pillar),
+                                 (const float*)(A + O.pillar_mean), 1, p->n_points, counts, p->n_cols, p->lo, p->vs,
+                                 (double*)(A + O.feat_gram), A + O.gram_ws);
+      else
+        rc = gd_vfe_feature_gram(st, (const float*)(A + O.points), (const long long*)(A + O.point_coords), I(O.inverse32),
+                                 (const float*)(A + O.pillar_mean), 0, p->n_points, counts, p->n_cols, p->lo, p->vs,
+                                 (double*)(A + O.feat_gram), A + O.gram_ws);
+      if (rc) return rc;
+    }
   }
   float* mask = (float*)(A + O.mask);
   if (p->masked) {
diff --git a/gd-mae_amd/csrc/segment.hip b/gd-mae_amd/csrc/segment.hip
--- a/gd-mae_amd/csrc/segment.hip
+++ b/gd-mae_amd/csrc/segment.hip
@@ -300,6 +300,30 @@
   return 0;
 }
 
+__device__ __forceinline__ void bn_fold_write(int c, int C, double s1, double s2, double count, const float* __restrict__ gamma,
+                                              const float* __restrict__ beta, double eps, double momentum,
+                                              float* __restrict__ running_mean, float* __restrict__ running_var,
+                                              long long* __restrict__ num_batches, double* __restrict__ stats,
+                                              float* __restrict__ ab, float* __restrict__ mv) {
+  const double mean = s1 / count;
+  double var = s2 / count - mean * mean;
+  if (var < 0.0) var = 0.0;
+  const double r = 1.0 / sqrt(var + eps);
+  const double a = (double)gamma[c] * r;
+  stats[c] = mean;
+  stats[C + c] = r;
+  ab[c] = (float)a;
+  ab[C + c] = (float)((double)beta[c] - a * mean);
+  mv[c] = (float)mean;
+  mv[C + c] = (float)var;
+  if (running_mean) {
+    const float m = (float)momentum;
+    const float unb = (float)(var * (count / (count > 1.0 ? count - 1.0 : 1.0)));
+    running_mean[c] = running_mean[c] * (1.f - m) + m * (float)mean;
+    running_var[c] = running_var[c] * (1.f - m) + m * unb;
+    if (c == 0 && num_batches) *num_batches += 1;
+  }
+}
 __global__ __launch_bounds__(256) void k_bn_fold_final(const float* __restrict__ part, int nblk, int C, double count,
                                                        const float* __restrict__ gamma, const float* __restrict__ beta,
                                                        double eps, double momentum, float* __restrict__ running_mean,
@@ -335,24 +359,7 @@
   if (ps == 0 && c < C) {
     double s1 = 0.0, s2 = 0.0;
     for (int k = 0; k < 16; ++k) { s1 += sh[0][k][cl]; s2 += sh[1][k][cl]; }
-    const double mean = s1 / count;
-    double var = s2 / count - mean * mean;
-    if (var < 0.0) var = 0.0;
-    const double r = 1.0 / sqrt(var + eps);
-    const double a = (double)gamma[c] * r;
-    stats[c] = mean;
-    stats[C + c] = r;
-    ab[c] = (float)a;
-    ab[C + c] = (float)((double)beta[c] - a * mean);
-    mv[c] = (float)mean;
-    mv[C + c] = (float)var;
-    if (running_mean) {
-      const float m = (float)momentum;
-      const float unb = (float)(var * (count / (count > 1.0 ? count - 1.0 : 1.0)));
-      running_mean[c] = running_mean[c] * (1.f - m) + m * (float)mean;
-      running_var[c] = running_var[c] * (1.f - m) + m * unb;
-      if (c == 0 && num_batches) *num_batches += 1;
-    }
+    bn_fold_write(c, C, s1, s2, count, gamma, beta, eps, momentum, running_mean, running_var, num_batches, stats, ab, mv);
   }
 }
 
@@ -383,6 +390,31 @@
                              long long* num_batches, double* stats, float* ab, float* mv) {
   hipLaunchKernelGGL(k_bn_fold_final, dim3(gd_div_up(C, 16)), dim3(256), 0, st, part, nblk, C, count, gamma, beta, eps, momentum,
                      running_mean, running_var, num_batches, stats, ab, mv);
+  GD_LAUNCH_CHECK();
+  return 0;
+}
+__global__ __launch_bounds__(64) void k_bn_fold_gram(const float* __restrict__ W, int D, const double* __restrict__ gram, int C,
+                                                     double count, const float* __restrict__ gamma, const float* __restrict__ beta,
+                                                     double eps, double momentum, float* __restrict__ running_mean,
+                                                     float* __restrict__ running_var, long long* __restrict__ num_batches,
+                                                     double* __restrict__ stats, float* __restrict__ ab, float* __restrict__ mv) {
+  const int c = blockIdx.x * 64 + threadIdx.x;
+  if (c >= C) return;
+  double s1 = 0.0, s2 = 0.0;
+  const double* G = gram + D;
+  int q = 0;
+  for (int i = 0; i < D; ++i) {
+    const double wi = (double)W[c * D + i];
+    s1 += wi * gram[i];
+    for (int j = i; j < D; ++j, ++q) s2 += (i == j ? 1.0 : 2.0) * wi * (double)W[c * D + j] * G[q];
+  }
+  bn_fold_write(c, C, s1, s2, count, gamma, beta, eps, momentum, running_mean, running_var, num_batches, stats, ab, mv);
+}
+int gd_bn_fold_from_gram(hipStream_t st, const float* W, int D, const double* gram, int C, double count, const float* gamma,
+                         const float* beta, double eps, double momentum, float* running_mean, float* running_var,
+                         long long* num_batches, double* stats, float* ab, float* mv) {
+  hipLaunchKernelGGL(k_bn_fold_gram, dim3(gd_div_up(C, 64)), dim3(64), 0, st, W, D, gram, C, count, gamma, beta, eps, momentum, running_mean,
+                     running_var, num_batches, stats, ab, mv);
   GD_LAUNCH_CHECK();
   return 0;
 }
diff --git a/gd-mae_amd/csrc/vfe_fused.hip b/gd-mae_amd/csrc/vfe_fused.hip
--- a/gd-mae_amd/csrc/vfe_fused.hip
+++ b/gd-mae_amd/csrc/vfe_fused.hip
@@ -4,6 +4,9 @@
 int gd_bn_fold_from_partials(hipStream_t st, const float* part, int nblk, int C, double count, const float* gamma,
                              const float* beta, double eps, double momentum, float* running_mean, float* running_var,
                              long long* num_batches, double* stats, float* ab, float* mv);
+int gd_bn_fold_from_gram(hipStream_t st, const float* W, int D, const double* gram, int C, double count, const float* gamma,
+                         const float* beta, double eps, double momentum, float* running_mean, float* running_var,
+                         long long* num_batches, double* stats, float* ab, float* mv);
 int gd_partials_to_f64(hipStream_t st, const float* part, int nblk, int C2, double* out);
 extern "C" int gdmae_bn_bwd_coeffs(const double* st, int n_st, const double* stats, const float* ab, const float* gamma, int C,
                                    double count, const double* tot, float* dgamma, float* dbeta, int accumulate, float* c01,
@@ -22,7 +25,7 @@
   int out_f16 = 0;
 };
 
-enum { VF_STATS = 0, VF_APPLY = 1, VF_BSTATS = 2, VF_DW = 3 };
+enum { VF_STATS = 0, VF_APPLY = 1, VF_BSTATS = 2, VF_DW = 3, VF_PDW = 4 };
 
 __device__ inline unsigned short vf_f2bf(float f) { return gd_to_bf16(f); }
 
@@ -88,14 +91,16 @@
                                                         int cpp, long long N, VfeGeom G, const float* __restrict__ W,
                                                         const float* __restrict__ ab, const float* __restrict__ c01,
                                                         const void* __restrict__ g, void* __restrict__ out,
-                                                        float* __restrict__ part) {
+                                                        float* __restrict__ part, float* __restrict__ part_dh) {
   constexpr int D = F + 6;
   constexpr int KS = (D + 1) / 2;
   constexpr int DP = 2 * KS;
   const int lane = threadIdx.x & 63, wave = threadIdx.x >> 6;
   const int n = lane & 31, half = lane >> 5;
-  __shared__ float sh[VF_WAVES * (MODE == VF_DW ? VF_C * D : 4 * VF_C)];
-  __shared__ float shf[MODE == VF_DW ? VF_WAVES * 32 * DP : 1];
+  constexpr bool IS_DW = MODE == VF_DW || MODE == VF_PDW;
+  __shared__ float sh[VF_WAVES * (IS_DW ? VF_C * D : 4 * VF_C)];
+  __shared__ float shf[IS_DW ? VF_WAVES * 32 * DP : 1];
+  __shared__ float shs[MODE == VF_PDW ? VF_WAVES * VF_C : 1];
 
   float wb[2][KS];
 #pragma unroll
@@ -124,7 +129,7 @@
 
   const long long ntiles = (N + 31) / 32;
   const long long tstride = (long long)gridDim.x * VF_WAVES;
-  constexpr bool HAS_G = MODE == VF_BSTATS || MODE == VF_DW;
+  constexpr bool HAS_G = MODE == VF_BSTATS || IS_DW;
   constexpr bool PIPE = !HAS_G;
   VfA<F> A1, A2, A3;
   VfB B1, B2;
@@ -196,7 +201,7 @@
         }
       }
     } else {
-      if (MODE == VF_DW) {
+      if (IS_DW) {
         if (half == 0) {
 #pragma unroll
           for (int d = 0; d < DP; ++d) shf[(wave * 32 + n) * DP + d] = d < D ? f[d] : 0.f;
@@ -216,14 +221,18 @@
           s2[0] = fmaf(dh0, h[0][r], s2[0]);
           s2[1] = fmaf(dh1, h[1][r], s2[1]);
         } else {
-          const float dx0 = fmaf(c1[0], h[0][r], fmaf(ca[0], dh0, c0[0]));
-          const float dx1 = fmaf(c1[1], h[1][r], fmaf(ca[1], dh1, c0[1]));
+          const float dx0 = MODE == VF_PDW ? dh0 : fmaf(c1[0], h[0][r], fmaf(ca[0], dh0, c0[0]));
+          const float dx1 = MODE == VF_PDW ? dh1 : fmaf(c1[1], h[1][r], fmaf(ca[1], dh1, c0[1]));
+          if (MODE == VF_PDW) {
+            s1[0] += dh0;
+            s1[1] += dh1;
+          }
           const float bv = n < DP ? shf[(wave * 32 + pr) * DP + n] : 0.f;
           accw[0] = __builtin_amdgcn_mfma_f32_32x32x2f32(dx0, bv, accw[0], 0, 0, 0);
           accw[1] = __builtin_amdgcn_mfma_f32_32x32x2f32(dx1, bv, accw[1], 0, 0, 0);
         }
       }
-      if (MODE == VF_DW) {
+      if (IS_DW) {
         __builtin_amdgcn_fence(__ATOMIC_RELEASE, "wavefront");
         __builtin_amdgcn_wave_barrier();
       }
@@ -255,7 +264,14 @@
       for (int w = 0; w < VF_WAVES; ++w) a += sh[w * 2 * VF_C + threadIdx.x];
       part[(long long)blockIdx.x * 2 * VF_C + threadIdx.x] = a;
     }
-  } else if (MODE == VF_DW) {
+  } else if (IS_DW) {
+    if (MODE == VF_PDW) {
+#pragma unroll
+      for (int blk = 0; blk < 2; ++blk) {
+        s1[blk] += __shfl_xor(s1[blk], 32, 64);
+        if (half == 0) shs[wave * VF_C + 2 * n + blk] = s1[blk];
+      }
+    }
     if (n < D) {
 #pragma unroll
       for (int blk = 0; blk < 2; ++blk)
@@ -272,12 +288,18 @@
       for (int w = 0; w < VF_WAVES; ++w) a += sh[w * VF_C * D + e];
       part[(long long)blockIdx.x * VF_C * D + e] = a;
     }
+    if (MODE == VF_PDW && threadIdx.x < VF_C) {
+      float a = 0.f;
+#pragma unroll
+      for (int w = 0; w < VF_WAVES; ++w) a += shs[w * VF_C + threadIdx.x];
+      part_dh[(long long)blockIdx.x * VF_C + threadIdx.x] = a;
+    }
   }
 }
 
 template <typename K>
 int vf_resident_blocks(K kernel, int slot) {
-  static int cache[32] = {0};
+  static int cache[30] = {0};
   if (cache[slot] == 0) {
     int per_cu = 0, dev = 0;
     hipDeviceProp_t prop;
@@ -292,15 +314,15 @@
 template <int MODE>
 int vf_launch(hipStream_t st, int F, bool bf, const float* pts, const long long* coords, const int* inv, const float* mean,
               int cpp, long long N, const VfeGeom& G, const float* W, const float* ab, const float* c01, const void* g, void* out,
-              float* part, int* grid_out = nullptr) {
+              float* part, int* grid_out = nullptr, float* part_dh = nullptr) {
   const long long tiles = (N + 31) / 32, blocks = (tiles + VF_WAVES - 1) / VF_WAVES;
   const dim3 block(VF_WAVES * 64);
 #define VF_GO(FF, BB)                                                                                                   \
   do {                                                                                                                  \
-    const int cap = vf_resident_blocks(k_vfe1<FF, MODE, BB>, ((FF - 3) * 4 + MODE) * 2 + (BB ? 1 : 0));                 \
+    const int cap = vf_resident_blocks(k_vfe1<FF, MODE, BB>, ((FF - 3) * 5 + MODE) * 2 + (BB ? 1 : 0));                 \
     const dim3 grid((unsigned)(blocks < cap ? blocks : cap));                                                           \
     if (grid_out) *grid_out = (int)grid.x;                                                                              \
-    hipLaunchKernelGGL((k_vfe1<FF, MODE, BB>), grid, block, 0, st, pts, coords, inv, mean, cpp, N, G, W, ab, c01, g, out, part); \
+    hipLaunchKernelGGL((k_vfe1<FF, MODE, BB>), grid, block, 0, st, pts, coords, inv, mean, cpp, N, G, W, ab, c01, g, out, part, part_dh); \
   } while (0)
   if (F == 5) { if (bf) VF_GO(5, true); else VF_GO(5, false); }
   else if (F == 4) { if (bf) VF_GO(4, true); else VF_GO(4, false); }
@@ -311,6 +333,157 @@
   return 0;
 }
 
+constexpr int VG_GRID = 512, VG_THREADS = 256, VG_WAVES = VG_THREADS / 64;
+__host__ __device__ constexpr int vg_np(int D) { return D + D * (D + 1) / 2; }
+__host__ __device__ constexpr int vg_idx(int a, int b, int D) { return D + a * D - a * (a - 1) / 2 + (b - a); }
+
+template <int F>
+__global__ __launch_bounds__(VG_THREADS) void k_vfe_gram(const float* __restrict__ pts, const long long* __restrict__ coords,
+                                                         const int* __restrict__ inv, const float* __restrict__ mean, int cpp,
+                                                         long long Ncap, const int* __restrict__ n_dev, VfeGeom G,
+                                                         double* __restrict__ part) {
+  constexpr int D = F + 6, NP = vg_np(D);
+  __shared__ double shg[VG_WAVES * NP];
+  long long N = Ncap;
+  if (n_dev) {
+    const long long nd = *n_dev;
+    N = nd < Ncap ? nd : Ncap;
+  }
+  double acc[NP];
+#pragma unroll
+  for (int e = 0; e < NP; ++e) acc[e] = 0.0;
+  const long long stride = (long long)gridDim.x * VG_THREADS;
+  long long i = (long long)blockIdx.x * VG_THREADS + threadIdx.x;
+  if (i < N) {
+    VfA<F> A1, A2;
+    VfB B1;
+    vf_load_a<F>(pts, inv, i, N, A1);
+    for (; i < N; i += stride) {
+      vf_load_a<F>(pts, inv, i + stride, N, A2);
+      vf_load_b<F>(coords, mean, cpp, i, N, A1.pil, B1);
+      float f[D];
+      vf_features<F>(A1, B1, true, G, f);
+      double fd[D];
+#pragma unroll
+      for (int a = 0; a < D; ++a) fd[a] = (double)f[a];
+#pragma unroll
+      for (int a = 0; a < D; ++a) {
+        acc[a] += fd[a];
+#pragma unroll
+        for (int b = a; b < D; ++b) acc[vg_idx(a, b, D)] = fma(fd[a], fd[b], acc[vg_idx(a, b, D)]);
+      }
+      A1 = A2;
+    }
+  }
+  const int lane = threadIdx.x & 63, wave = threadIdx.x >> 6;
+#pragma unroll
+  for (int e = 0; e < NP; ++e) {
+    double v = acc[e];
+#pragma unroll
+    for (int o = 32; o >= 1; o >>= 1) v += __shfl_xor(v, o, 64);
+    if (lane == 0) shg[wave * NP + e] = v;
+  }
+  __syncthreads();
+  if (threadIdx.x < NP) {
+    double a = 0.0;
+#pragma unroll
+    for (int w = 0; w < VG_WAVES; ++w) a += shg[w * NP + threadIdx.x];
+    part[(long long)blockIdx.x * NP + threadIdx.x] = a;
+  }
+}
+
+__global__ __launch_bounds__(256) void k_vfe_gram_final(const double* __restrict__ part, int nblk, int NP, double* __restrict__ gram) {
+  __shared__ double shr[2][128];
+  const int e = threadIdx.x & 127, ps = threadIdx.x >> 7;
+  const int ec = e < NP ? e : NP - 1;
+  double a = 0.0;
+  for (int b0 = ps; b0 < nblk; b0 += 16) {
+    double v[8];
+#pragma unroll
+    for (int u = 0; u < 8; ++u) {
+      const int b = b0 + 2 * u < nblk ? b0 + 2 * u : nblk - 1;
+      v[u] = part[(long long)b * NP + ec];
+    }
+#pragma unroll
+    for (int u = 0; u < 8; ++u) a += b0 + 2 * u < nblk ? v[u] : 0.0;
+  }
+  shr[ps][e] = a;
+  __syncthreads();
+  if (ps == 0 && e < NP) gram[e] = shr[0][e] + shr[1][e];
+}
+
+__global__ __launch_bounds__(256) void k_vfe1_bwd_finish(const float* __restrict__ part, const float* __restrict__ part_dh, int nblk,
+                                                         int D, const float* __restrict__ W, const double* __restrict__ gram,
+                                                         const double* __restrict__ stats, const float* __restrict__ ab,
+                                                         const float* __restrict__ gamma, double count,
+                                                         float* __restrict__ dgamma, float* __restrict__ dbeta,
+                                                         float* __restrict__ dW, int accumulate) {
+  __shared__ double shp[16][17];
+  __shared__ double P[16];
+  __shared__ double cf[2];
+  const int c = blockIdx.x, d = threadIdx.x & 15, ps = threadIdx.x >> 4;
+  {
+    const int dc = d < D ? d : 0;
+    const float* src = d < D ? part + (long long)c * D + dc : part_dh + c;
+    const long long pitch = d < D ? (long long)VF_C * D : VF_C;
+    double a = 0.0;
+    for (int b0 = ps; b0 < nblk; b0 += 128) {
+      float v[8];
+#pragma unroll
+      for (int u = 0; u < 8; ++u) {
+        const int b = b0 + 16 * u < nblk ? b0 + 16 * u : nblk - 1;
+        v[u] = src[(long long)b * pitch];
+      }
+#pragma unroll
+      for (int u = 0; u < 8; ++u) a += (b0 + 16 * u < nblk && d <= D) ? (double)v[u] : 0.0;
+    }
+    shp[ps][d] = a;
+  }
+  __syncthreads();
+  if (threadIdx.x < 16) {
+    double a = 0.0;
+    for (int k = 0; k < 16; ++k) a += shp[k][threadIdx.x];
+    P[threadIdx.x] = a;
+  }
+  __syncthreads();
+  if (threadIdx.x == 0) {
+    const double mean = stats[c], r = stats[VF_C + c];
+    const double a = (double)ab[c];
+    const double db = P[D];
+    double dhh = 0.0;
+    for (int k = 0; k < D; ++k) dhh += (double)W[c * D + k] * P[k];
+    const double da = dhh - db * mean;
+    const double dv = -0.5 * (da * (double)gamma[c]) * r * r * r;
+    const double dmu = -db * a - 2.0 * mean * dv;
+    cf[0] = dmu / count;
+    cf[1] = 2.0 * dv / count;
+    const float dg = (float)(da * r), dbf = (float)db;
+    if (accumulate) { dgamma[c] += dg; dbeta[c] += dbf; }
+    else { dgamma[c] = dg; dbeta[c] = dbf; }
+  }
+  __syncthreads();
+  if (threadIdx.x < D) {
+    const int k = threadIdx.x;
+    double wg = 0.0;
+    for (int j = 0; j < D; ++j) wg += (double)W[c * D + j] * gram[j <= k ? vg_idx(j, k, D) : vg_idx(k, j, D)];
+    const float v = (float)((double)ab[c] * P[k] + cf[0] * gram[k] + cf[1] * wg);
+    if (accumulate) dW[c * D + k] += v;
+    else dW[c * D + k] = v;
+  }
+}
+
+template <int F>
+int vg_launch(hipStream_t st, const float* pts, const long long* coords, const int* inv, const float* mean, int cpp, long long Ncap,
+              const int* n_dev, const VfeGeom& G, double* gram, double* part) {
+  const long long blocks = (Ncap + VG_THREADS - 1) / VG_THREADS;
+  const int grid = (int)(blocks < VG_GRID ? blocks : VG_GRID);
+  hipLaunchKernelGGL(k_vfe_gram<F>, dim3(grid), dim3(VG_THREADS), 0, st, pts, coords, inv, mean, cpp, Ncap, n_dev, G, part);
+  GD_LAUNCH_CHECK();
+  hipLaunchKernelGGL(k_vfe_gram_final, dim3(1), dim3(256), 0, st, (const double*)part, grid, vg_np(F + 6), gram);
+  GD_LAUNCH_CHECK();
+  return 0;
+}
+
 }
 
 __global__ __launch_bounds__(256) void k_pillar_major_rows(const float* __restrict__ pts, int ncols, const int* __restrict__ csr,
@@ -337,7 +510,33 @@
 extern "C" size_t gdmae_vfe_point_layer_workspace_bytes(int n_cols) {
   const int D = n_cols - 1 + 6;
   return gd_align((size_t)VF_MAX_GRID * VF_C * (D > 2 ? D : 2) * sizeof(float)) + gd_align(2 * VF_C * sizeof(double)) +
-         gd_align(2 * VF_C * sizeof(float));
+         gd_align(2 * VF_C * sizeof(float)) + gd_align((size_t)VF_MAX_GRID * VF_C * sizeof(float));
+}
+
+extern "C" size_t gdmae_vfe_feature_gram_workspace_bytes(int n_cols) {
+  return gd_align((size_t)VG_GRID * vg_np(n_cols - 1 + 6) * sizeof(double));
+}
+int gd_vfe_feature_gram(hipStream_t st, const float* points, const long long* point_coords, const int* inverse32, const float* pillar_mean,
+                        int coords_per_pillar, long long N, const int* n_dev, int n_cols, const float* lo, const float* vs, double* gram,
+                        void* workspace) {
+  const int F = n_cols - 1;
+  GD_REQUIRE(F >= 3 && F <= 5, "vfe feature sums: 3, 4 or 5 point features (x, y, z [, intensity [, elongation]])");
+  if (N <= 0) {
+    GD_CHECK(hipMemsetAsync(gram, 0, sizeof(double) * vg_np(F + 6), st));
+    return 0;
+  }
+  VfeGeom G;
+  for (int i = 0; i < 3; ++i) { G.lo[i] = lo[i]; G.vs[i] = vs[i]; }
+  double* part = (double*)workspace;
+  if (F == 5) return vg_launch<5>(st, points, point_coords, inverse32, pillar_mean, coords_per_pillar, N, n_dev, G, gram, part);
+  if (F == 4) return vg_launch<4>(st, points, point_coords, inverse32, pillar_mean, coords_per_pillar, N, n_dev, G, gram, part);
+  return vg_launch<3>(st, points, point_coords, inverse32, pillar_mean, coords_per_pillar, N, n_dev, G, gram, part);
+}
+extern "C" int gdmae_vfe_feature_gram(const float* points, const long long* point_coords, const int* inverse32,
+                                      const float* pillar_mean, int coords_per_pillar, long long N, const int* n_dev, int n_cols,
+                                      const float* lo, const float* vs, double* gram, void* workspace, void* stream) {
+  return gd_vfe_feature_gram((hipStream_t)stream, points, point_coords, inverse32, pillar_mean, coords_per_pillar, N, n_dev, n_cols, lo, vs,
+                             gram, workspace);
 }
 
 extern "C" int gdmae_vfe_point_layer_fwd(const float* points, const long long* point_coords, const int* inverse32,
@@ -396,3 +595,51 @@
   if (rc) return rc;
   return gd_splitk_acc(st, part, grid, (long long)VF_C * D, dW, accumulate);
 }
+
+extern "C" int gdmae_vfe_point_layer_fwd_gram(const float* points, const long long* point_coords, const int* inverse32,
+                                              const float* pillar_mean, int coords_per_pillar, long long N, int n_cols,
+                                              const float* lo, const float* vs, const double* gram,
+                                              const float* W, int C, const float* gamma, const float* beta, double eps,
+                                              double momentum, float* running_mean, float* running_var, long long* num_batches,
+                                              double* stats, float* ab, float* mv, void* out, int out_bf16, void* stream) {
+  GD_REQUIRE(C == VF_C, "vfe point layer: 64 output channels");
+  GD_REQUIRE(N > 0 && gram != nullptr, "vfe point layer: no points / no feature sums");
+  hipStream_t st = (hipStream_t)stream;
+  VfeGeom G;
+  for (int i = 0; i < 3; ++i) { G.lo[i] = lo[i]; G.vs[i] = vs[i]; }
+  const int F = n_cols - 1;
+  GD_REQUIRE(F >= 3 && F <= 5, "vfe point layer: 3, 4 or 5 point features (x, y, z [, intensity [, elongation]])");
+  int rc = gd_bn_fold_from_gram(st, W, F + 6, gram, C, (double)N, gamma, beta, eps, momentum, running_mean, running_var, num_batches,
+                                stats, ab, mv);
+  if (rc) return rc;
+  G.out_f16 = out_bf16 == 2;
+  return vf_launch<VF_APPLY>(st, F, out_bf16 != 0, points, point_coords, inverse32, pillar_mean, coords_per_pillar, N, G, W, ab, nullptr, nullptr,
+                             out, nullptr);
+}
+
+extern "C" int gdmae_vfe_point_layer_bwd_gram(const float* points, const long long* point_coords, const int* inverse32,
+                                              const float* pillar_mean, int coords_per_pillar, long long N, int n_cols,
+                                              const float* lo, const float* vs, const double* gram,
+                                              const float* W, int C, const float* gamma, const double* stats, const float* ab,
+                                              const void* g, int g_bf16, float* dgamma, float* dbeta, float* dW, int accumulate,
+                                              void* workspace, void* stream) {
+  GD_REQUIRE(C == VF_C, "vfe point layer: 64 output channels");
+  GD_REQUIRE(N > 0 && gram != nullptr, "vfe point layer: no points / no feature sums");
+  hipStream_t st = (hipStream_t)stream;
+  VfeGeom G;
+  for (int i = 0; i < 3; ++i) { G.lo[i] = lo[i]; G.vs[i] = vs[i]; }
+  const int F = n_cols - 1, D = F + 6;
+  char* p = (char*)workspace;
+  float* part = (float*)p;
+  p += gd_align((size_t)VF_MAX_GRID * VF_C * (D > 2 ? D : 2) * sizeof(float)) + gd_align(2 * VF_C * sizeof(double)) +
+       gd_align(2 * VF_C * sizeof(float));
+  float* part_dh = (float*)p;
+  int grid = 0;
+  int rc = vf_launch<VF_PDW>(st, F, g_bf16 != 0, points, point_coords, inverse32, pillar_mean, coords_per_pillar, N, G, W, ab, nullptr, g,
+                             nullptr, part, &grid, part_dh);
+  if (rc) return rc;
+  hipLaunchKernelGGL(k_vfe1_bwd_finish, dim3(VF_C), dim3(256), 0, st, (const float*)part, (const float*)part_dh, grid, D, W, gram, stats,
+                     ab, gamma, (double)N, dgamma, dbeta, dW, accumulate);
+  GD_LAUNCH_CHECK();
+  return 0;
+}
diff --git a/gd-mae_amd/gdmae_hip/lib.py b/gd-mae_amd/gdmae_hip/lib.py
--- a/gd-mae_amd/gdmae_hip/lib.py
+++ b/gd-mae_amd/gdmae_hip/lib.py
@@ -29,6 +29,10 @@
     "gdmae_pillar_major_rows": (_I, [_P, _I, _P, _P, _P, _L, _P, _P, _P]),
     "gdmae_vfe_point_layer_fwd": (_I, [_P, _P, _P, _P, _I, _L, _I, _P, _P, _P, _I, _P, _P, _D, _D, _P, _P, _P, _P, _P, _P, _P, _I, _P, _P]),
     "gdmae_vfe_point_layer_bwd": (_I, [_P, _P, _P, _P, _I, _L, _I, _P, _P, _P, _I, _P, _P, _P, _P, _I, _P, _P, _P, _I, _P, _P]),
+    "gdmae_vfe_feature_gram_workspace_bytes": (_Z, [_I]),
+    "gdmae_vfe_feature_gram": (_I, [_P, _P, _P, _P, _I, _L, _P, _I, _P, _P, _P, _P, _P]),
+    "gdmae_vfe_point_layer_fwd_gram": (_I, [_P, _P, _P, _P, _I, _L, _I, _P, _P, _P, _P, _I, _P, _P, _D, _D, _P, _P, _P, _P, _P, _P, _P, _I, _P]),
+    "gdmae_vfe_point_layer_bwd_gram": (_I, [_P, _P, _P, _P, _I, _L, _I, _P, _P, _P, _P, _I, _P, _P, _P, _P, _I, _P, _P, _P, _I, _P, _P]),
     "gdmae_vfe_max_layer_workspace_bytes": (_Z, []),
     "gdmae_vfe_max_layer_fwd": (_I, [_P, _L, _P, _P, _P, _I, _P, _P, _D, _D, _P, _P, _P, _P, _P, _P, _P, _P, _P, _P]),
     "gdmae_vfe_max_layer_bwd": (_I, [_P, _L, _P, _P, _I, _P, _P, _P, _P, _P, _P, _P, _P, _P, _P, _P, _I, _P, _P]),
diff --git a/gd-mae_amd/gdmae_hip/plan.py b/gd-mae_amd/gdmae_hip/plan.py
--- a/gd-mae_amd/gdmae_hip/plan.py
+++ b/gd-mae_amd/gdmae_hip/plan.py
@@ -38,6 +38,7 @@
     counts: torch.Tensor
     points_pm: torch.Tensor = None
     row_pillar: torch.Tensor = None
+    feat_gram: torch.Tensor = None
 
 
 def _voxelize_launch(points: torch.Tensor, point_cloud_range, voxel_size, grid_size, batch_size: int) -> dict:
@@ -418,14 +419,15 @@
 
     def __init__(self, raw, names):
         self.raw, self.names = raw, names
-        self.base = {torch.int32: raw.view(torch.int32), torch.float32: raw.view(torch.float32), torch.int64: raw.view(torch.int64)}
+        self.base = {torch.int32: raw.view(torch.int32), torch.float32: raw.view(torch.float32), torch.int64: raw.view(torch.int64),
+                     torch.float64: raw.view(torch.float64)}
 
     def has(self, name):
         return name in self.names
 
     def view(self, name, dtype, *shape):
         off, _ = self.names[name]
-        es = 8 if dtype == torch.int64 else 4
+        es = 8 if dtype in (torch.int64, torch.float64) else 4
         strides, acc = [], 1
         for d in reversed(shape):
             strides.append(acc)
@@ -506,6 +508,8 @@
                         V("pillar_pts", i32, N), V("point_rank", i32, N), V("sample_off", i32, B + 1), V("pillar_mean", f32, M, F),
                         V("cell2pillar", i32, B * gx * gy * gz), V("counts", i32, 2), V("points_pm", f32, N, ncols), V("row_pillar", i32, N))
         vox._arena = A
+        if A.has("feat_gram"):
+            vox.feat_gram = V("feat_gram", torch.float64, names["feat_gram"][1] // 8)
         ns = len(geo)
         n_vis = int(c[2 + ns + 16 * ns + 1])
         stages = []
diff --git a/gd-mae_amd/gdmae_hip/vfe.py b/gd-mae_amd/gdmae_hip/vfe.py
--- a/gd-mae_amd/gdmae_hip/vfe.py
+++ b/gd-mae_amd/gdmae_hip/vfe.py
@@ -1,4 +1,6 @@
 from __future__ import annotations
+
+import os
 
 import torch
 
@@ -7,8 +9,23 @@
 from . import ops
 
 
+VFE_GRAM = os.environ.get("GDMAE_VFE_GRAM", "1") != "0"
+VFE_GRAM_FWD = os.environ.get("GDMAE_VFE_GRAM", "1") == "2"
+
+
 def _bf(t):
     return int(t.dtype == torch.bfloat16)
+
+
+def feature_gram(vox, pm):
+    if vox.feat_gram is None:
+        D = vox.n_cols + 5
+        gram = torch.empty(D + D * (D + 1) // 2, dtype=torch.float64, device=vox.points.device)
+        ws = torch.empty(L.load().gdmae_vfe_feature_gram_workspace_bytes(vox.n_cols), dtype=torch.uint8, device=gram.device)
+        geo = PointLayer1._geometry(vox, pm)
+        L.call("gdmae_vfe_feature_gram", *geo[:6], None, *geo[6:], L.ptr(gram), L.ptr(ws), L.stream())
+        vox.feat_gram = gram
+    return vox.feat_gram
 
 
 class BNReLURows(torch.autograd.Function):
@@ -178,10 +195,14 @@
         mom = 0.0
         if bn is not None and bn.training and bn.running_mean is not None:
             rm, rv, nb, mom = bn.running_mean, bn.running_var, bn.num_batches_tracked, float(bn.momentum)
-        L.call("gdmae_vfe_point_layer_fwd", *PointLayer1._geometry(vox, ctx.pm), L.ptr(weight), C, L.ptr(gamma), L.ptr(beta),
-               float(eps), mom, L.ptr(rm) if rm is not None else None, L.ptr(rv) if rv is not None else None,
-               L.ptr(nb) if nb is not None else None, L.ptr(stats), L.ptr(ab), L.ptr(mv), L.ptr(out), 2 if out_f16 else _bf(out), L.ptr(ws),
-               L.stream())
+        ctx.gram = feature_gram(vox, ctx.pm) if VFE_GRAM_FWD else None
+        bnargs = (L.ptr(weight), C, L.ptr(gamma), L.ptr(beta), float(eps), mom, L.ptr(rm) if rm is not None else None,
+                  L.ptr(rv) if rv is not None else None, L.ptr(nb) if nb is not None else None, L.ptr(stats), L.ptr(ab), L.ptr(mv),
+                  L.ptr(out), 2 if out_f16 else _bf(out))
+        if ctx.gram is not None:
+            L.call("gdmae_vfe_point_layer_fwd_gram", *PointLayer1._geometry(vox, ctx.pm), L.ptr(ctx.gram), *bnargs, L.stream())
+        else:
+            L.call("gdmae_vfe_point_layer_fwd", *PointLayer1._geometry(vox, ctx.pm), *bnargs, L.ptr(ws), L.stream())
         ctx.vox, ctx.ws = vox, ws
         ctx.save_for_backward(weight, gamma.detach(), stats, ab)
         ctx.direct = (ops.direct_grad(weight), *gbn.direct_pair(gamma, beta))
@@ -213,8 +234,14 @@
             dw = torch.empty_like(weight)
             dgb = torch.empty(2 * C, dtype=torch.float32, device=weight.device)
             dg, db = dgb[:C], dgb[C:]
-        L.call("gdmae_vfe_point_layer_bwd", *PointLayer1._geometry(vox, ctx.pm), L.ptr(weight), C, L.ptr(gamma), L.ptr(stats),
-               L.ptr(ab), L.ptr(g), _bf(g), L.ptr(dg), L.ptr(db), L.ptr(dw), acc, L.ptr(ctx.ws), L.stream())
+        gradargs = (L.ptr(weight), C, L.ptr(gamma), L.ptr(stats), L.ptr(ab), L.ptr(g), _bf(g), L.ptr(dg), L.ptr(db), L.ptr(dw), acc,
+                    L.ptr(ctx.ws), L.stream())
+        if VFE_GRAM and ctx.gram is None:
+            ctx.gram = feature_gram(vox, ctx.pm)
+        if ctx.gram is not None:
+            L.call("gdmae_vfe_point_layer_bwd_gram", *PointLayer1._geometry(vox, ctx.pm), L.ptr(ctx.gram), *gradargs)
+        else:
+            L.call("gdmae_vfe_point_layer_bwd", *PointLayer1._geometry(vox, ctx.pm), *gradargs)
         if acc:
             return None, None, None, None, None, None, None, None
         return None, dw, dg, db, None, None, None, None
diff --git a/include/gdmae_hip.h b/include/gdmae_hip.h
--- a/include/gdmae_hip.h
+++ b/include/gdmae_hip.h
@@ -41,6 +41,22 @@
                               const float* W, int C, const float* gamma, const double* stats, const float* ab,
                               const void* g, int g_bf16, float* dgamma, float* dbeta, float* dW, int accumulate,
                               void* workspace, void* stream);
+size_t gdmae_vfe_feature_gram_workspace_bytes(int n_cols);
+int gdmae_vfe_feature_gram(const float* points, const long long* point_coords, const int* inverse32, const float* pillar_mean,
+                           int coords_per_pillar, long long N, const int* n_dev, int n_cols, const float* lo, const float* vs,
+                           double* gram, void* workspace, void* stream);
+int gdmae_vfe_point_layer_fwd_gram(const float* points, const long long* point_coords, const int* inverse32,
+                                   const float* pillar_mean, int coords_per_pillar, long long N, int n_cols, const float* lo,
+                                   const float* vs, const double* gram,
+                                   const float* W, int C, const float* gamma, const float* beta, double eps, double momentum,
+                                   float* running_mean, float* running_var, long long* num_batches, double* stats, float* ab,
+                                   float* mv, void* out, int out_bf16, void* stream);
+int gdmae_vfe_point_layer_bwd_gram(const float* points, const long long* point_coords, const int* inverse32,
+                                   const float* pillar_mean, int coords_per_pillar, long long N, int n_cols, const float* lo,
+                                   const float* vs, const double* gram,
+                                   const float* W, int C, const float* gamma, const double* stats, const float* ab,
+                                   const void* g, int g_bf16, float* dgamma, float* dbeta, float* dW, int accumulate,
+                                   void* workspace, void* stream);
 size_t gdmae_vfe_max_layer_workspace_bytes(void);
 int gdmae_vfe_max_layer_fwd(const void* y1, long long N, const void* W, const int* pillar_pt_off, const int* row_pillar,
                             int M, const float* gamma, const float* beta, double eps, double momentum,
```

Result: no change. 1092, median of 6 (+0.8%).
